# jazlab/moog.github.io

Measured on AMD Instinct MI355X. Metric: env steps/sec (whole node), 4096 envs x 32 sprites, 64x64 obs, higher is better.
Workload: dtype f64; 1 GPU; colliding_predators_32: 4096 envs/GPU x 32 sprites, K=10 substeps, 64x64 raster, random joystick actions, auto-reset on; phase=step + frames, envs_per_gpu=4096, total_envs=4096, sprites=32, parallelism=env-sharded x1, no collective, launch=step launch, then raster launch, on one stream, sub_batches=1, hw_queues=4, episodes=staggered (step_count offsets + 201 burn-in steps before the warm-up)

## Files before the change

### __graft_entry__.py

```python
import glob
import os
import time
import subprocess
import sys

REPO = os.path.dirname(os.path.abspath(__file__))
PKG = os.path.join(REPO, 'moog.github.io_amd')
CSRC = os.path.join(PKG, 'csrc')
LIB = os.path.join(PKG, 'lib', 'libmoog_hip.so')
HIPCC = os.environ.get('HIPCC', '/opt/rocm/bin/hipcc')
sys.path.insert(0, PKG)
from moog import _digest
HIP_FLAGS = _digest.HIP_FLAGS
_STEP_DEPS = ['moog_device.h', 'moog_kernels.h', 'moog_draw_record.h']
_RASTER_DEPS = ['moog_device.h', 'moog_raster.h', 'moog_raster_kernel.h', 'moog_raster_mask.h', 'moog_raster_mask_core.h', 'moog_draw_record.h']
UNITS = [('moog_engine.o', 'moog_engine.hip', [], _STEP_DEPS + _RASTER_DEPS),
         ('moog_raster.o', 'moog_raster.hip', [], _RASTER_DEPS),
         ('moog_reset_r0.o', 'moog_reset.hip', ['-DMOOG_RESET_FULL=0'], _STEP_DEPS),
         ('moog_reset_r1.o', 'moog_reset.hip', ['-DMOOG_RESET_FULL=1'], _STEP_DEPS)] + [
    ('moog_step_%s.o' % tag, 'moog_step_inst.hip',
     ['-DMOOG_STEP_DYN=%d' % dyn, '-DMOOG_STEP_WPS=%d' % wps, '-DMOOG_STEP_TAG=%s' % tag], _STEP_DEPS)
    for tag, dyn, wps in (('f3', 0, 3), ('f4', 0, 4), ('t3', 1, 3), ('t4', 1, 4), ('m3', 2, 3), ('m4', 2, 4))] + [
    ('moog_step_%sr.o' % tag, 'moog_step_inst.hip',
     ['-DMOOG_STEP_DYN=%d' % dyn, '-DMOOG_STEP_WPS=%d' % wps, '-DMOOG_STEP_TAG=%sr' % tag, '-DMOOG_STEP_REPEAT=1'], _STEP_DEPS)
    for tag, dyn, wps in (('f3', 0, 3), ('f4', 0, 4), ('t3', 1, 3), ('t4', 1, 4), ('m3', 2, 3), ('m4', 2, 4))]


SPEC_WORKLOADS = ['colliding_predators_32', 'falling_balls_64', 'functional_maze@128', 'chase_avoid_torus']


def _paths():
    for p in (PKG, os.path.join(REPO, 'tests')):
        if p not in sys.path:
            sys.path.insert(0, p)


def _stale(target, sources):
    if not os.path.exists(target):
        return True
    t = os.path.getmtime(target)
    return any(os.path.getmtime(s) > t for s in sources)


def build():
    hdr = os.path.join(REPO, 'include', 'moog_engine.h')
    os.makedirs(os.path.join(PKG, 'lib'), exist_ok=True)
    digest = _digest.source_digest()
    digest_file = os.path.join(PKG, 'lib', 'src_digest.txt')
    if not os.path.exists(digest_file) or open(digest_file).read().strip() != digest:
        with open(digest_file, 'w') as f:
            f.write(digest + '\n')
    flags_file = os.path.join(PKG, 'lib', 'hip_flags.txt')
    if not os.path.exists(flags_file) or open(flags_file).read().strip() != ' '.join(HIP_FLAGS):
        with open(flags_file, 'w') as f:
            f.write(' '.join(HIP_FLAGS) + '\n')
    for obj in glob.glob(os.path.join(PKG, 'lib', 'moog_*.o')):
        if os.path.basename(obj) not in [u[0] for u in UNITS]:
            os.remove(obj)
    objs, procs = [], []
    started = time.time()
    for obj_name, unit, extra, deps in UNITS:
        obj = os.path.join(PKG, 'lib', obj_name)
        objs.append(obj)
        own = [digest_file] if unit == 'moog_engine.hip' else []
        if unit == 'moog_engine.hip':
            extra = extra + [_digest.define_flag(digest)]
        if _stale(obj, [os.path.join(CSRC, unit), hdr, flags_file] + own + [os.path.join(CSRC, d) for d in sorted(set(deps))]):
            procs.append((obj, subprocess.Popen(
                [HIPCC] + HIP_FLAGS + extra + ['-c', os.path.join(CSRC, unit), '-o', obj])))
    for obj, p in procs:
        if p.wait() != 0:
            for _, q in procs:
                if q.poll() is None:
                    q.terminate()
            raise RuntimeError('hipcc failed: %s' % obj)
        os.utime(obj, (started, started))
    if _stale(LIB, objs):
        subprocess.check_call([HIPCC, '--offload-arch=gfx950', '-shared', '-fPIC'] + objs + ['-o', LIB])
    osrc = [os.path.join(REPO, 'oracle', 'moog_oracle.c'), hdr]
    if _stale(os.path.join(REPO, 'oracle', 'libmoog_oracle.so'), osrc):
        subprocess.check_call(['make', '-C', os.path.join(REPO, 'oracle'), '-B', 'libmoog_oracle.so'])
    _paths()
    import moog
    from moog import _engine
    _engine.load_library()
    from moog import _spec
    assert '%016x' % _engine.load_library().moog_source_digest() == digest, 'libmoog_hip.so does not carry the digest of its sources'
    _spec.main(SPEC_WORKLOADS)
    gone = _spec.remove_stale()
    if gone:
        print('removed %d specialised step kernels of another build: %s' % (len(gone), ' '.join(gone)))


def smoke():
    build()
    _paths()
    import numpy as np
    import torch
    import helpers
    from moog import environment
    from moog_demos import example_configs

    n = 16
    env = environment.BatchedEnvironment(num_envs=n, seed=3, **example_configs.load('colliding_predators'))
    o = helpers.OracleEnv(env.compiled, n_envs=n, seed=3)
    env.reset()
    o.reset()
    rs = np.random.RandomState(0)
    for _ in range(8):
        a = rs.uniform(-1, 1, size=(n, 2))
        ts = env.step(a)
        o.step(a)
    torch.cuda.synchronize()
    f, q = env.state_f64.cpu().numpy(), env.state_i32.cpu().numpy()
    assert np.array_equal(q, o.i32), 'integer state differs from the oracle'
    err = float(np.nanmax(np.abs(f - o.f64)))
    assert err <= 1e-9, 'float state differs from the oracle by %g' % err
    assert np.array_equal(ts.step_type.cpu().numpy(), o.step_type)
    o.f64[:], o.i32[:] = f, q
    assert np.array_equal(ts.observation['image'].cpu().numpy(), o.render()), 'frame mismatch'
    print('smoke ok: %d envs, max |state - oracle| = %.3g' % (n, err))


if __name__ == '__main__':
    build()
    print('build ok:', LIB)
```

### include/moog_engine.h

```cpp
#ifndef MOOG_ENGINE_H_
#define MOOG_ENGINE_H_

#include <stdint.h>

#ifdef __cplusplus
extern "C" {
#endif

#define MOOG_ABI_VERSION 31
#define MOOG_PROGRAM_VERSION 30
#define MOOG_MAX_ACTION_REPEAT 64

#define MOOG_MAX_LAYERS 16
#define MOOG_MAX_FORCES 16
#define MOOG_MAX_CORRECTIVE 4
#define MOOG_MAX_RULES 16
#define MOOG_MAX_TASKS 8
#define MOOG_MAX_OPS 256
#define MOOG_MAX_SHAPES 256
#define MOOG_MAX_SHAPE_VERTS 2048
#define MOOG_MAX_CAND 256
#define MOOG_MAX_DCODE 2048
#define MOOG_X_STACK 16
#define MOOG_MAX_SLOTS 256
// ... 307 lines not shown
  int32_t n_hdraws;
  int32_t rule_state2;
  double timeout_steps;

  moog_force_t forces[MOOG_MAX_FORCES];
  moog_corrective_t corrective[MOOG_MAX_CORRECTIVE];
  moog_rule_t rules[MOOG_MAX_RULES];
  moog_task_t tasks[MOOG_MAX_TASKS];
  moog_action_t action;
  int32_t n_actions;
  int32_t pad_actions_;
  moog_action_t more_actions[MOOG_MAX_MORE_ACTIONS];
  moog_render_t render;
  moog_maze_t maze;
  moog_genop_t ops[MOOG_MAX_OPS];
  moog_shape_t shapes[MOOG_MAX_SHAPES];
  double shape_verts[MOOG_MAX_SHAPE_VERTS][2];
  double cand[MOOG_MAX_CAND];
  int32_t n_dcode;
  int32_t xstack_depth;
  int32_t pad_x_;
  int32_t pad_y_;
  int32_t born_rule;
  moog_dinstr_t dcode[MOOG_MAX_DCODE];
  uint8_t slot_persist[MOOG_MAX_SLOTS];
} moog_program_t;

typedef struct {
  int32_t S, TOTV, T, R;
  int32_t f64_per_env, i32_per_env;
  int32_t o_pos;
  int32_t o_vel;
  int32_t o_angle;
  int32_t o_angvel;
  int32_t o_mass;
  int32_t o_color;
  int32_t o_inertia;
  int32_t o_maxr;
  int32_t o_action;
  int32_t o_task;
  int32_t o_rule;
  int32_t o_hdraw;
  int32_t o_rule2;
  int32_t o_scale;
  int32_t o_aspect;
  int32_t o_verts;
  int32_t o_flags;
  int32_t o_nverts;
  int32_t o_opacity;
  int32_t o_shape;
  int32_t o_tele;
  int32_t o_fmask;
  int32_t o_valias;
  int32_t o_step_count;
  int32_t o_reset_next;
  int32_t o_fault;
  int32_t o_rng;
  int32_t o_maze;
} moog_layout_t;

#if defined(__HIPCC__)
#define MOOG_HD __host__ __device__
#else
#define MOOG_HD
#endif
MOOG_HD static inline int32_t moog_align_(int32_t x, int32_t a) { return (x + a - 1) / a * a; }

MOOG_HD static inline void moog_layout(const moog_program_t* p, moog_layout_t* L) {
  int32_t S = p->n_slots, o = 0;
  L->S = S; L->TOTV = p->n_total_verts; L->T = p->n_tasks; L->R = p->n_rules;
  L->o_pos = o; o += 2 * S;
  L->o_vel = o; o += 2 * S;
  L->o_angle = o; o += S;
  L->o_angvel = o; o += S;
  L->o_mass = o; o += S;
  L->o_color = o; o += 3 * S;
  L->o_inertia = o; o += 2 * S;
  L->o_maxr = o; o += S;
  L->o_action = o; o += 2 * (p->n_actions > 1 ? p->n_actions : 1);
  L->o_task = o; o += p->n_tasks;
  L->o_rule = o; o += p->n_rules;
  if (p->n_hdraws > 0) { L->o_hdraw = o; o += p->n_hdraws; } else L->o_hdraw = -1;
  if (p->rule_state2) { L->o_rule2 = o; o += p->n_rules; } else L->o_rule2 = -1;
  if (p->sprite_factors) { L->o_scale = o; o += S; L->o_aspect = o; o += S; }
  else { L->o_scale = -1; L->o_aspect = -1; }
  o = moog_align_(o, 2);
  L->o_verts = o; o += 2 * p->n_total_verts;
  L->f64_per_env = moog_align_(o, 2);
  o = 0;
  L->o_flags = o; o += S;
  L->o_nverts = o; o += S;
  L->o_opacity = o; o += S;
  L->o_shape = o; o += S;
  L->o_tele = o; o += S;
  if (p->vel_alias) { L->o_valias = o; o += S; } else L->o_valias = -1;
  if (p->sprite_factors) { L->o_fmask = o; o += S; } else L->o_fmask = -1;
  L->o_step_count = o; o += 1;
  L->o_reset_next = o; o += 1;
  L->o_fault = o; o += 1;
  L->o_rng = o; o += 4;
  if (p->maze.random) { L->o_maze = o; o += MOOG_MAX_MAZE + MOOG_MAX_MAZE_POINTS; } else L->o_maze = -1;
  L->i32_per_env = moog_align_(o, 4);
}

typedef struct {
  double* f64;
  int32_t* i32;
} moog_state_view_t;

typedef struct {
  double* reward;
  double* discount;
  int32_t* step_type;
  uint8_t* image;
} moog_step_out_t;

typedef struct {
  const double* uniforms;
  int32_t per_env;
} moog_inject_t;

typedef struct moog_engine moog_engine_t;

enum { MOOG_K_STEP = 0, MOOG_K_RASTER = 1, MOOG_K_RESET = 2, MOOG_K_VIEWS = 3, MOOG_K_COUNT = 4 };

int moog_abi_version(void);
unsigned long long moog_source_digest(void);
const char* moog_last_error(void);
int64_t moog_program_sizeof(void);

int moog_engine_create(const moog_program_t* prog, int32_t n_envs, int32_t device_id,
                       uint64_t seed, int64_t env_index0, moog_engine_t** out);
int moog_engine_destroy(moog_engine_t* e);
int moog_engine_layout(const moog_engine_t* e, moog_layout_t* out);
int moog_engine_load_state(moog_engine_t* e, const moog_state_view_t* view);

int moog_engine_reset(moog_engine_t* e, const uint8_t* env_mask_dev,
                      const moog_inject_t* inject, const moog_step_out_t* out,
                      void* hip_stream);
int moog_engine_step(moog_engine_t* e, const void* actions_dev,
                     const moog_inject_t* inject, const moog_step_out_t* out,
                     void* hip_stream);
int moog_engine_set_action_dtype(moog_engine_t* e, int32_t float32);
int moog_engine_set_action_repeat(moog_engine_t* e, int32_t k, int32_t* count_dev);
int moog_engine_physics_only(moog_engine_t* e, const moog_inject_t* inject,
                             void* hip_stream);
int moog_engine_render(moog_engine_t* e, uint8_t* image_dev, void* hip_stream);

int moog_engine_add_view(moog_engine_t* e, const moog_render_t* render, int32_t* view);
int moog_engine_set_view_image(moog_engine_t* e, int32_t view, uint8_t* image_dev);
int moog_engine_view_raster_path(moog_engine_t* e, int32_t view, int32_t* path);

int moog_engine_set_schedule(moog_engine_t* e, int32_t* perm_dev, float* cost_dev);


int moog_engine_set_reset_pool(moog_engine_t* e, int32_t enabled);
int moog_engine_get_reset_pool(moog_engine_t* e, int32_t* enabled, int64_t* stats);

int moog_engine_layer_usage(moog_engine_t* e, int32_t* high_water, int32_t* dropped);

int moog_engine_set_timing(moog_engine_t* e, int32_t enabled);
int moog_engine_kernel_time(moog_engine_t* e, int32_t kernel_id, double* total_ms,
                            int64_t* launches);

int moog_engine_poll_faults(moog_engine_t* e, int32_t clear, int32_t* bits);

int moog_engine_static_prefix(moog_engine_t* e, int32_t* n_slots, uint8_t* image_dev, void* hip_stream);

int moog_engine_env_prefix(moog_engine_t* e, int32_t* n_slots);

int moog_engine_kernel_variant(moog_engine_t* e, int32_t* variant, int32_t* late_reset);

int moog_program_step_kernel(const moog_program_t* program, int32_t* variant, int32_t* wps, uint64_t* hash);
int moog_engine_step_kernel(moog_engine_t* e, int32_t* specialised);

enum { MOOG_RASTER_SPANS = 0, MOOG_RASTER_MASK = 1, MOOG_RASTER_MASK_COMPACT = 3 };
int moog_engine_raster_path(moog_engine_t* e, int32_t* path);

int moog_engine_read_draw_records(moog_engine_t* e, uint8_t* host_out, int64_t bytes, int64_t* stride, int32_t* in_step);

int moog_engine_set_color_override(moog_engine_t* e, const uint32_t* rgb_dev);

int moog_engine_set_debug(moog_engine_t* e, int32_t step_debug, int32_t raster_stop);

#define MOOG_WATCH_SECTIONS 32
int moog_engine_read_watch(moog_engine_t* e, int32_t* host_out, int32_t clear);

#ifdef __cplusplus
}
#endif
#endif
```

### moog.github.io_amd/csrc/moog_engine.hip

```cpp
#include <hip/hip_runtime.h>

#include <cmath>
#include <cstdio>
#include <cstring>
#include <string>
#include <vector>

#include "moog_kernels.h"

#include "moog_raster.h"
#include <dlfcn.h>
#include <unistd.h>

static thread_local std::string g_err;
static const char* const FRAMELESS_MSG = "this program draws no frames (no PILRenderer observer: render 0 x 0): pass no image";
static int fail(int code, const std::string& msg) { g_err = msg; return code; }
#define HIPCHK(x)                                                                        \
  do {                                                                                   \
    hipError_t err_ = (x);                                                               \
    if (err_ != hipSuccess)                                                              \
      return fail(MOOG_E_HIP, std::string(#x) + ": " + hipGetErrorString(err_));         \
  } while (0)

struct TimedKernel {
  std::vector<std::pair<hipEvent_t, hipEvent_t>> pending;
  double total_ms = 0;
  int64_t launches = 0;
  int64_t seq = 0;
};

struct RView {
  moog_render_t render{};
  const moog_program_t* P = nullptr;
  moog_program_t* d_own = nullptr;
  uint8_t* image = nullptr;
  RPlan raster_plan_{};
  RmSetup mask_setup{};
  uint8_t* draw = nullptr;
  RmDrawLayout draw_lay{};
  int raster_tile_w = 0, raster_band_h = 0, raster_tiles_x = 1, raster_bands = 1;
  int aa = 1, canvas_w = 0, canvas_h = 0, aa_chunk = 0;
  int pad_w = 0;
  uint8_t* pad_img = nullptr;
  int32_t* aa_tables = nullptr;
  RResize aa_resize{};
  int raster_chunk = 0, raster_words = 0, raster_iwords = 0, raster_hwords = 1, raster_xxcap = 4;
  size_t raster_lds = 0;
  int32_t* rows_seen = nullptr;
  int raster_rows_fixed = 0;
  int mask_free_cap = 0;
  int n_static = 0, nsv = 0, kept_n_static = 0;
  uint8_t* s_bg = nullptr;
};

struct moog_engine {
  moog_program_t prog;
  moog_layout_t L;
  moog_program_t* d_prog = nullptr;
  int16_t* d_vslot = nullptr;
  uint32_t* d_vinfo = nullptr;
  int32_t n_envs = 0;
  int device = 0;
  uint64_t seed = 0;
  int64_t env_index0 = 0;
  moog_state_view_t view{nullptr, nullptr};
  size_t step_lds = 0;
  int step_wps = 4;
  void* spec_handle = nullptr;
  void (*spec_launch)(int, size_t, hipStream_t, const KArgs*) = nullptr;
  int32_t xstack_off = 0;
  FOp* d_fops = nullptr;
  int32_t n_fops = 0;
  int32_t* watch = nullptr;
  int32_t watch_off = 0;
  bool dynamic_rules = false;
  bool maze_kernel = false;
  bool late_reset = false;
  uint8_t* late_mask = nullptr;
  RView views[MOOG_MAX_VIEWS];
  int n_views = 1;
  bool frameless = false;
  uint8_t* aa_canvas = nullptr;
  uint8_t* aa_tmp = nullptr;
  size_t aa_canvas_bytes = 0, aa_tmp_bytes = 0;
  int timing = 0;
  int32_t* perm = nullptr;
  hipStream_t sched_stream = nullptr;
  hipEvent_t ev_step_done = nullptr, ev_sched_done = nullptr;
  bool sched_pending = false;
  float* cost = nullptr;
  static constexpr int POOL_STREAMS = 8;
  int pool_streams = 2;
  bool pool_on = false, pool_ready = false;
  static constexpr int pool_depth = 2;
  int32_t* pool_state = nullptr;
  int32_t* pool_tag = nullptr;
  int32_t* pool_lock = nullptr;
  unsigned long long* pool_stats = nullptr;
  double* pool_f64[2] = {nullptr, nullptr};
  int32_t* pool_i32[2] = {nullptr, nullptr};
  hipStream_t pool_stream[POOL_STREAMS] = {};
  hipEvent_t ev_pool = nullptr;
  int64_t pool_fills = 0;
  int act_f32 = 0;
  int action_repeat = 1;
  int32_t* repeat_count = nullptr;
  int32_t* layer_hw = nullptr;
  TimedKernel timed[MOOG_K_COUNT];
  int32_t* fault_flag = nullptr;
  int step_dbg = 0, raster_stop = 0;
  double* s_f64 = nullptr;
  int32_t* s_i32 = nullptr;
  const uint32_t* rgb_override = nullptr;
  int kept_pe_ns = 0, kept_pe_nsv = 0;
  int pe_ns = 0, pe_nsv = 0;
  double* pe_f64 = nullptr;
  int32_t* pe_i32 = nullptr;
  uint8_t* pe_bg = nullptr;
  int32_t* pe_valid = nullptr;
  int32_t* pe_build = nullptr;
  int32_t* pe_min = nullptr;
};

static void free_engine(moog_engine* e) {
  if (e->d_prog) hipFree(e->d_prog);
  if (e->d_vslot) hipFree(e->d_vslot);
  if (e->d_vinfo) hipFree(e->d_vinfo);
  for (RView& v : e->views) {
    if (v.d_own) hipFree(v.d_own);
    if (v.draw) hipFree(v.draw);
    if (v.s_bg) hipFree(v.s_bg);
    if (v.pad_img) hipFree(v.pad_img);
    if (v.aa_tables) hipFree(v.aa_tables);
    if (v.rows_seen) hipHostFree(v.rows_seen);
  }
  if (e->s_f64) hipFree(e->s_f64);
  if (e->s_i32) hipFree(e->s_i32);
  if (e->aa_canvas) hipFree(e->aa_canvas);
  if (e->aa_tmp) hipFree(e->aa_tmp);
  if (e->fault_flag) hipHostFree(e->fault_flag);
  if (e->layer_hw) hipFree(e->layer_hw);
  for (int k = 0; k < moog_engine::POOL_STREAMS; ++k)
    if (e->pool_stream[k]) { hipStreamSynchronize(e->pool_stream[k]); hipStreamDestroy(e->pool_stream[k]); }
  if (e->ev_pool) hipEventDestroy(e->ev_pool);
  if (e->pe_f64) hipFree(e->pe_f64);
  if (e->pe_i32) hipFree(e->pe_i32);
  if (e->pe_bg) hipFree(e->pe_bg);
  if (e->pe_valid) hipFree(e->pe_valid);
  if (e->pe_build) hipFree(e->pe_build);
  if (e->pe_min) hipHostFree(e->pe_min);
  if (e->pool_state) hipFree(e->pool_state);
  if (e->pool_tag) hipFree(e->pool_tag);
  if (e->pool_lock) hipFree(e->pool_lock);
  if (e->late_mask) hipFree(e->late_mask);
  if (e->pool_stats) hipFree(e->pool_stats);
  for (int k = 0; k < 2; ++k) { if (e->pool_f64[k]) hipFree(e->pool_f64[k]); if (e->pool_i32[k]) hipFree(e->pool_i32[k]); }
  if (e->watch) hipFree(e->watch);
  if (e->d_fops) hipFree(e->d_fops);
  delete e;
}

static int static_prefix_slots(const moog_program_t* p, int polymod, int* nsv) {
  *nsv = 0;
  if (polymod != MOOG_POLYMOD_NONE) return 0;
  std::vector<char> ok((size_t)(p->n_slots > 0 ? p->n_slots : 1), 0);
  for (int oi = 0; oi < p->n_ops; ++oi) {
    const moog_genop_t& op = p->ops[oi];
    if (op.runtime || op.n_sampled != 0 || op.code_off >= 0 || op.count_min != op.count_max) continue;
    bool c = true;
    for (int k = 0; k < MOOG_NUM_FACTORS; ++k) c = c && op.factors[k].kind == MOOG_DIST_CONST;
    c = c && op.factors[MOOG_FAC_XVEL].a == 0 && op.factors[MOOG_FAC_YVEL].a == 0 && op.factors[MOOG_FAC_ANGVEL].a == 0;
    if (!c) continue;
    for (int sl = op.slot0; sl < op.slot0 + op.count_max && sl < p->n_slots; ++sl)
      if (sl >= 0 && !p->layer_dynamic[p->slot_layer[sl]]) ok[sl] = 1;
  }
  int ns = 0, nv = 0;
  while (ns < p->n_slots && ns < 32 && ok[ns] && p->slot_voff[ns] == nv) { nv += p->slot_vcap[ns]; ++ns; }
  *nsv = nv;
  return ns;
}

static int env_prefix_slots(const moog_program_t* p, int* nsv) {
  *nsv = 0;
  if (p->render.polymod != MOOG_POLYMOD_NONE) return 0;
  std::vector<char> ok((size_t)(p->n_slots > 0 ? p->n_slots : 1), 0);
  for (int oi = 0; oi < p->n_ops; ++oi) {
    const moog_genop_t& op = p->ops[oi];
    if (op.runtime || op.cell_sel == MOOG_CELL_STORE) continue;
    bool c = true;
    for (int k = MOOG_FAC_XVEL; k <= MOOG_FAC_ANGVEL; ++k)
      if (k == MOOG_FAC_XVEL || k == MOOG_FAC_YVEL || k == MOOG_FAC_ANGVEL) c = c && op.factors[k].kind == MOOG_DIST_CONST && op.factors[k].a == 0;
    if (!c) continue;
    for (int sl = op.slot0; sl < op.slot0 + op.count_max && sl < p->n_slots; ++sl)
      if (sl >= 0 && !p->layer_dynamic[p->slot_layer[sl]]) ok[sl] = 1;
  }
  for (int oi = 0; oi < p->n_ops; ++oi)
    if (p->ops[oi].cell_sel == MOOG_CELL_STORE && p->ops[oi].cell_arg >= 0 && p->ops[oi].cell_arg < p->n_slots) ok[p->ops[oi].cell_arg] = 0;
  int ns = 0, nv = 0;
  while (ns < p->n_slots && ok[ns] && p->slot_voff[ns] == nv) { nv += p->slot_vcap[ns]; ++ns; }
  *nsv = nv;
  return ns;
}

struct StepVariant { bool dynamic_rules = false, maze_kernel = false, late_reset = false; int wps = 4; size_t step_lds = 0; int32_t xstack_off = 0; };

static StepVariant step_variant_of(const moog_program_t* prog) {
  StepVariant v;
  moog_layout_t GL;
  moog_layout(prog, &GL);
  const moog_layout_t HL = hot_layout(GL).L;
  v.step_lds = (size_t)HL.f64_per_env * 8 + (size_t)HL.i32_per_env * 4 + (size_t)GL.S * 4 * 8 +
               (size_t)((GL.S + 3) & ~3) * 4 + CAND_CAP * 2 + 128 + 64 * 8 + 16;
  if (prog->xstack_depth > 0) {
    v.step_lds = (v.step_lds + 15) & ~(size_t)15;
    v.xstack_off = (int32_t)v.step_lds;
    v.step_lds += (size_t)prog->xstack_depth * 64 * 8;
  }
  for (int r = 0; r < prog->n_rules; ++r) {
    int k = prog->rules[r].kind;
    if (k == MOOG_RULE_VANISH_BY_FILTER || k == MOOG_RULE_CHANGE_LAYER || k == MOOG_RULE_CREATE_SPRITES ||
        k == MOOG_RULE_MODIFY_SPRITES || k == MOOG_RULE_MODIFY_ON_CONTACT || k == MOOG_RULE_DRAWS)
      v.dynamic_rules = true;
  }
  for (int t = 0; t < prog->n_tasks; ++t) {
    if (prog->tasks[t].kind == MOOG_TASK_CONTACT_REWARD && (prog->tasks[t].xcond >= 0 || prog->tasks[t].xreward >= 0))
      v.dynamic_rules = true;
    if (prog->tasks[t].kind == MOOG_TASK_RESET && (prog->tasks[t].cond >= MOOG_COND_ALL_EXPR || prog->tasks[t].xreward >= 0))
      v.dynamic_rules = true;
  }
  for (int r = 0; r < prog->n_rules; ++r)
    if ((prog->rules[r].kind == MOOG_RULE_CONDITIONAL || prog->rules[r].kind == MOOG_RULE_PHASE) &&
        prog->rules[r].cond >= MOOG_RCOND_CONTACT_COUNT)
      v.dynamic_rules = true;
  for (int l = 0; l < prog->n_layers; ++l) if (prog->layer_dynamic[l]) v.dynamic_rules = true;
  for (int f = 0; f < prog->n_forces; ++f)
    if (prog->forces[f].kind == MOOG_FORCE_DISTANCE_EXPR) v.dynamic_rules = true;
  for (int r = 0; r < prog->n_rules; ++r)
    if (prog->rules[r].kind == MOOG_RULE_FIXATION || (prog->rules[r].kind == MOOG_RULE_PHASE && prog->rules[r].op == 1))
      v.dynamic_rules = true;
  for (int k = 0; k < prog->n_dcode; ++k) {
    if (prog->dcode[k].op == MOOG_X_STORE && prog->dcode[k].a == MOOG_XA_ANGLE) v.maze_kernel = true;
    const int op = prog->dcode[k].op;
    if (op == MOOG_X_SLOT_ATTR || op == MOOG_X_HDRAW || op == MOOG_X_HDRAW_T || op == MOOG_X_STORE_VERT || op == MOOG_X_FACTOR)
      v.maze_kernel = true;
  }
  for (int o = 0; o < prog->n_ops; ++o) if (prog->ops[o].cell_sel != MOOG_CELL_NONE) v.maze_kernel = true;
  if (prog->n_hdraws > 0) v.maze_kernel = true;
  for (int o = 0; o < prog->n_ops; ++o)
    for (int k = 0; k < MOOG_NUM_FACTORS; ++k)
      if (prog->ops[o].factors[k].kind == MOOG_DIST_EXPR || prog->ops[o].factors[k].kind == MOOG_DIST_EXPR_SHAPE)
        v.maze_kernel = true;
  for (int f = 0; f < prog->n_forces; ++f)
    if (prog->forces[f].kind == MOOG_FORCE_MAZE_WALK || prog->forces[f].kind == MOOG_FORCE_MAZE_WALK_DET) v.maze_kernel = true;
  for (int c = 0; c < prog->n_corrective; ++c) if (prog->corrective[c].kind == MOOG_CORR_MAZE) v.maze_kernel = true;
  if (prog->maze.random) v.maze_kernel = true;
  if (v.maze_kernel) {
    bool stepping = false;
    for (int f = 0; f < prog->n_forces; ++f)
      stepping = stepping || prog->forces[f].kind == MOOG_FORCE_MAZE_WALK || prog->forces[f].kind == MOOG_FORCE_MAZE_WALK_DET;
    for (int c = 0; c < prog->n_corrective; ++c) stepping = stepping || prog->corrective[c].kind == MOOG_CORR_MAZE;
    for (int k = 0; k < prog->n_dcode; ++k) stepping = stepping || (prog->dcode[k].op == MOOG_X_STORE && prog->dcode[k].a == MOOG_XA_ANGLE);
    for (int o = 0; o < prog->n_ops; ++o) {
      const moog_genop_t& op = prog->ops[o];
      if (!op.runtime) continue;
      bool full = op.cell_sel != MOOG_CELL_NONE || op.code_off >= 0;
      for (int k = 0; k < MOOG_NUM_FACTORS; ++k)
        full = full || op.factors[k].kind == MOOG_DIST_EXPR || op.factors[k].kind == MOOG_DIST_EXPR_SHAPE;
      stepping = stepping || full;
    }
    const char* off = getenv("MOOG_NO_LATE_RESET");
    v.late_reset = !stepping && !(off && atoi(off));
    if (v.late_reset) v.dynamic_rules = true;
  }
  v.wps = (160 * 1024 / (v.step_lds ? v.step_lds : 1)) <= 14 ? 3 : 4;
  { const char* w = getenv("MOOG_STEP_WPS"); if (w && (atoi(w) == 3 || atoi(w) == 4)) v.wps = atoi(w); }
  return v;
}

static uint64_t program_hash(const moog_program_t* prog) {
  const unsigned char* b = reinterpret_cast<const unsigned char*>(prog);
  uint64_t h = 1469598103934665603ull;
  for (size_t i = 0; i < sizeof(moog_program_t); ++i) { h ^= b[i]; h *= 1099511628211ull; }
  return h;
}

static void load_spec_kernel(moog_engine* e, const moog_program_t* prog);

#ifndef MOOG_SRC_DIGEST
#define MOOG_SRC_DIGEST 0ull
#endif
#define MOOG_STR2(x) #x
#define MOOG_STR(x) MOOG_STR2(x)
extern "C" const char moog_src_digest_marker[] = "MOOG_SRC_DIGEST=" MOOG_STR(MOOG_SRC_DIGEST);

extern "C" {

int moog_abi_version(void) { return MOOG_ABI_VERSION; }
unsigned long long moog_source_digest(void) { return MOOG_SRC_DIGEST; }
const char* moog_last_error(void) { return g_err.c_str(); }
int64_t moog_program_sizeof(void) { return (int64_t)sizeof(moog_program_t); }

static int validate_render(const moog_program_t* p, const moog_render_t* r) {
  const int aa = r->aa > 1 ? r->aa : 1;
  const long long cw = (long long)aa * r->width, ch = (long long)aa * r->height;
  if (cw < 1 || cw > 8192 || ch < 1 || ch > 8192 || aa > 16)
    return fail(MOOG_E_UNSUPPORTED, "render size unsupported (1 <= anti_aliasing x width, height <= 8192, anti_aliasing <= 16)");
  if (r->cmap != MOOG_CMAP_IDENTITY && r->cmap != MOOG_CMAP_HSV) return fail(MOOG_E_INVALID, "render cmap out of range");
// ... 302 lines not shown
      v.mask_free_cap = (ms.ok && !v.raster_rows_fixed) ? mask_free_rows(e, v) : ms.cap_rows;
      if (ms.ok) {
        v.draw_lay = rm_draw_layout(ms.S, e->L.TOTV * ms.ncopy);
        if (hipMalloc(&v.draw, (size_t)e->n_envs * v.draw_lay.stride) != hipSuccess) {
          return fail(MOOG_E_NOMEM, "out of device memory (draw records)");
        }
      }
    }
  }
  if (hipHostMalloc(reinterpret_cast<void**>(&v.rows_seen), 2 * sizeof(int32_t), hipHostMallocMapped | hipHostMallocCoherent) == hipSuccess) { v.rows_seen[0] = 0; v.rows_seen[1] = 0; }
  else v.rows_seen = nullptr;
  return MOOG_OK;
}

int moog_engine_create(const moog_program_t* prog, int32_t n_envs, int32_t device_id, uint64_t seed,
                       int64_t env_index0, moog_engine_t** out) {
  if (!out) return fail(MOOG_E_INVALID, "null out");
  int rc = validate(prog);
  if (rc) return rc;
  if (n_envs <= 0) return fail(MOOG_E_INVALID, "n_envs <= 0");
  HIPCHK(hipSetDevice(device_id));
  moog_engine* e = new moog_engine();
  e->prog = *prog;
  e->frameless = prog->render.width == 0 && prog->render.height == 0;
  moog_layout(prog, &e->L);
  e->n_envs = n_envs;
  e->device = device_id;
  e->seed = seed;
  e->env_index0 = env_index0;
  hipError_t err = hipMalloc(&e->d_prog, sizeof(moog_program_t));
  if (err != hipSuccess) { free_engine(e); return fail(MOOG_E_NOMEM, "hipMalloc(program) failed"); }
  err = hipMemcpy(e->d_prog, prog, sizeof(moog_program_t), hipMemcpyHostToDevice);
  if (err != hipSuccess) { free_engine(e); return fail(MOOG_E_HIP, "hipMemcpy(program) failed"); }
  {
    std::vector<int16_t> vs((size_t)(prog->n_total_verts > 0 ? prog->n_total_verts : 1), 0);
    for (int sl = 0; sl < prog->n_slots; ++sl)
      for (int k = 0; k < prog->slot_vcap[sl]; ++k) vs[prog->slot_voff[sl] + k] = (int16_t)sl;
    err = hipMalloc(&e->d_vslot, vs.size() * sizeof(int16_t));
    if (err == hipSuccess)
      err = hipMemcpy(e->d_vslot, vs.data(), vs.size() * sizeof(int16_t), hipMemcpyHostToDevice);
    if (err != hipSuccess) { free_engine(e); return fail(MOOG_E_NOMEM, "vertex table"); }
    std::vector<uint32_t> vi(vs.size(), 0u);
    for (int sl = 0; sl < prog->n_slots; ++sl)
      for (int k = 0; k < prog->slot_vcap[sl]; ++k) vi[prog->slot_voff[sl] + k] = (uint32_t)sl | ((uint32_t)k << 8);
    err = hipMalloc(&e->d_vinfo, vi.size() * sizeof(uint32_t));
    if (err == hipSuccess)
      err = hipMemcpy(e->d_vinfo, vi.data(), vi.size() * sizeof(uint32_t), hipMemcpyHostToDevice);
    if (err != hipSuccess) { free_engine(e); return fail(MOOG_E_NOMEM, "vertex table"); }
  }
  {
    const std::vector<FOp> fops = moog_flatten_forces(prog);
    e->n_fops = (int32_t)fops.size();
    err = hipMalloc(&e->d_fops, (fops.size() + 1) * sizeof(FOp));
    if (err == hipSuccess && !fops.empty()) err = hipMemcpy(e->d_fops, fops.data(), fops.size() * sizeof(FOp), hipMemcpyHostToDevice);
    if (err != hipSuccess) { free_engine(e); return fail(MOOG_E_NOMEM, "force list"); }
  }
  {
    const StepVariant sv = step_variant_of(prog);
    e->step_lds = sv.step_lds; e->xstack_off = sv.xstack_off;
  }
  { const char* w = getenv("MOOG_WATCH");
    if (w && atoi(w) == 1) {
      e->step_lds = (e->step_lds + 15) & ~(size_t)15;
      e->watch_off = (int32_t)e->step_lds;
      e->step_lds += 16;
      if (hipMalloc(&e->watch, (size_t)n_envs * MOOG_WATCH_SECTIONS * sizeof(int32_t)) != hipSuccess ||
          hipMemset(e->watch, 0, (size_t)n_envs * MOOG_WATCH_SECTIONS * sizeof(int32_t)) != hipSuccess) {
        free_engine(e);
        return fail(MOOG_E_NOMEM, "hipMalloc(watch) failed");
      }
    } }
  if (e->step_lds > 160 * 1024) {
    free_engine(e);
    return fail(MOOG_E_UNSUPPORTED, "state record does not fit in 160 KB of LDS");
  }
  if (!e->frameless) {
    e->views[0].render = prog->render;
    e->views[0].P = e->d_prog;
    const int rc = setup_view(e, e->views[0], true);
    if (rc) { free_engine(e); return rc; }
  }
  {
    int (*const configure[12])(size_t) = {moog_configure_step_f3, moog_configure_step_f4, moog_configure_step_t3,
                                          moog_configure_step_t4, moog_configure_step_m3, moog_configure_step_m4,
                                          moog_configure_step_f3r, moog_configure_step_f4r, moog_configure_step_t3r,
                                          moog_configure_step_t4r, moog_configure_step_m3r, moog_configure_step_m4r};
    for (int v = 0; v < 12 && err == hipSuccess; ++v) err = (hipError_t)configure[v](e->step_lds);
  }
  {
    const StepVariant sv = step_variant_of(prog);
    e->dynamic_rules = sv.dynamic_rules; e->maze_kernel = sv.maze_kernel; e->late_reset = sv.late_reset; e->step_wps = sv.wps;
  }
  if (!e->watch) load_spec_kernel(e, prog);
  if (e->late_reset) {
    if (hipMalloc(&e->late_mask, (size_t)n_envs) != hipSuccess || hipMemset(e->late_mask, 0, (size_t)n_envs) != hipSuccess) {
      free_engine(e);
      return fail(MOOG_E_NOMEM, "hipMalloc(late reset mask) failed");
    }
  }
  if (err == hipSuccess)
    err = (hipError_t)moog_configure_reset_plain(e->step_lds);
    if (err == hipSuccess) err = (hipError_t)moog_configure_reset_full(e->step_lds);
  if (err == hipSuccess && !e->frameless)
    err = (hipError_t)moog_raster_configure(e->views[0].raster_lds);
  if (err == hipSuccess && e->views[0].mask_setup.ok) err = (hipError_t)moog_raster_configure_mask(64 * 1024);
  if (err != hipSuccess) {
    free_engine(e);
    return fail(MOOG_E_HIP, std::string("hipFuncSetAttribute: ") + hipGetErrorString(err));
  }
  { const char* ds = getenv("MOOG_STEP_DEBUG"); e->step_dbg = ds ? atoi(ds) : 0; }
  { const char* ds = getenv("MOOG_RASTER_STOP"); e->raster_stop = ds ? atoi(ds) : 0; }
  if (hipHostMalloc(reinterpret_cast<void**>(&e->fault_flag), sizeof(int32_t), hipHostMallocMapped | hipHostMallocCoherent) != hipSuccess) {
    free_engine(e);
    return fail(MOOG_E_NOMEM, "hipHostMalloc(fault flag) failed");
  }
  *e->fault_flag = 0;
  for (int l = 0; l < prog->n_layers; ++l)
    if (prog->layer_dynamic[l] && !e->layer_hw) {
      if (hipMalloc(&e->layer_hw, 2 * MOOG_MAX_LAYERS * sizeof(int32_t)) != hipSuccess ||
          hipMemset(e->layer_hw, 0, 2 * MOOG_MAX_LAYERS * sizeof(int32_t)) != hipSuccess) {
        free_engine(e);
        return fail(MOOG_E_NOMEM, "hipMalloc(layer usage) failed");
      }
    }
  int rc2 = MOOG_OK;
  if (!e->frameless) {
    RView& v = e->views[0];
    rc2 = build_static_prefix(e, v);
    if (rc2 == MOOG_OK) rc2 = setup_anti_aliasing(e, v);
    if (rc2 == MOOG_OK) rc2 = setup_env_prefix(e);
    if (rc2 == MOOG_OK && v.aa <= 1 && v.pad_w != v.canvas_w &&
        hipMalloc(&v.pad_img, (size_t)n_envs * v.canvas_h * v.pad_w * 3) != hipSuccess)
      rc2 = fail(MOOG_E_NOMEM, "hipMalloc(16-aligned frames) failed");
  }
  if (rc2) { free_engine(e); return rc2; }
  *out = e;
  return MOOG_OK;
}

static void drain(TimedKernel& t) {
  for (auto& pr : t.pending) {
    hipEventSynchronize(pr.second);
    float ms = 0;
    if (hipEventElapsedTime(&ms, pr.first, pr.second) == hipSuccess) { t.total_ms += ms; t.launches++; }
    hipEventDestroy(pr.first);
    hipEventDestroy(pr.second);
  }
  t.pending.clear();
}

int moog_engine_destroy(moog_engine_t* e) {
  if (!e) return MOOG_OK;
  for (int k = 0; k < MOOG_K_COUNT; ++k) drain(e->timed[k]);
  if (e->sched_stream) {
    hipStreamSynchronize(e->sched_stream);
    hipEventDestroy(e->ev_step_done); hipEventDestroy(e->ev_sched_done);
    hipStreamDestroy(e->sched_stream);
  }
  void* spec = e->spec_handle;
  free_engine(e);
  (void)spec;
  return MOOG_OK;
}

int moog_engine_layout(const moog_engine_t* e, moog_layout_t* out) {
  if (!e || !out) return fail(MOOG_E_INVALID, "null argument");
  *out = e->L;
  return MOOG_OK;
}

static int pool_drop(moog_engine* e, hipStream_t s);

int moog_engine_load_state(moog_engine_t* e, const moog_state_view_t* view) {
  if (!e || !view || !view->f64 || !view->i32) return fail(MOOG_E_INVALID, "null state view");
  if (((uintptr_t)view->f64 & 15) || ((uintptr_t)view->i32 & 15))
    return fail(MOOG_E_INVALID, "state buffers must be 16-byte aligned");
  e->view = *view;
  if (e->pool_on) {
    HIPCHK(hipSetDevice(e->device));
    const int rc = pool_drop(e, 0);
    if (rc) return rc;
    HIPCHK(hipStreamSynchronize(0));
  }
  return MOOG_OK;
}

static bool sampled(moog_engine* e, int id) {
  const int period = ((e->timing >> 8) & 255) + 1;
  return ((e->timing >> id) & 1) && (e->timed[id].seq++ % period) == 0;
}

struct Bracket {
  moog_engine* e; int id; hipStream_t s; hipEvent_t a = nullptr, b = nullptr;
  Bracket(moog_engine* e_, int id_, hipStream_t s_, int on = -1) : e(e_), id(id_), s(s_) {
    if (on < 0 ? sampled(e, id) : on != 0) { hipEventCreate(&a); hipEventCreate(&b); hipEventRecord(a, s); }
  }
  ~Bracket() {
    if (a) { hipEventRecord(b, s); e->timed[id].pending.emplace_back(a, b); }
  }
};

static KArgs make_args(moog_engine* e, const void* actions, const moog_inject_t* inj,
                       const moog_step_out_t* out, int mode, const uint8_t* mask) {
  KArgs a;
  a.P = e->d_prog; a.L = e->L; a.H = hot_layout(e->L); a.f64 = e->view.f64; a.i32 = e->view.i32;
  a.actions = actions;
  a.inj = (inj && inj->uniforms) ? inj->uniforms : nullptr;
  a.inj_n = (inj && inj->uniforms) ? inj->per_env : 0;
  a.n_envs = e->n_envs; a.seed = e->seed; a.env_index0 = e->env_index0;
  a.mask = mask;
  a.reward = out ? out->reward : nullptr;
  a.discount = out ? out->discount : nullptr;
  a.step_type = out ? out->step_type : nullptr;
  a.mode = mode;
  a.vslot = e->d_vslot;
  a.perm = (mode == MODE_STEP && e->perm) ? e->perm : nullptr;
  a.cost = (mode == MODE_STEP) ? e->cost : nullptr;
  a.dbg = e->step_dbg;
  a.fault_flag = e->fault_flag;
  a.layer_hw = e->layer_hw;
  a.act_f32 = e->act_f32;
  a.repeat = mode == MODE_STEP ? e->action_repeat : 1;
  a.repeat_count = mode == MODE_STEP ? e->repeat_count : nullptr;
  a.xstack_off = e->xstack_off;
  a.watch = (mode == MODE_STEP) ? e->watch : nullptr; a.watch_off = e->watch_off;
  a.fops = e->d_fops; a.n_fops = e->n_fops;
  const bool pool = e->pool_on && mode == MODE_STEP && !(inj && inj->uniforms);
  a.pool_state = pool ? e->pool_state : nullptr; a.pool_tag = e->pool_tag; a.pool_stats = e->pool_stats;
  a.pool_lock = e->pool_lock; a.pool_depth = e->pool_depth;
  for (int k = 0; k < 2; ++k) { a.pool_f64[k] = e->pool_f64[k]; a.pool_i32[k] = e->pool_i32[k]; }
  a.live_f64 = nullptr; a.live_i32 = nullptr;
  a.late_mask = (mode == MODE_STEP && e->late_reset) ? e->late_mask : nullptr;
  a.rank0 = 0;
  memset(&a.draw, 0, sizeof a.draw);
  a.draw_vinfo = e->d_vinfo;
  return a;
}

static void launch_step(moog_engine* e, hipStream_t s, const KArgs& a) {
  static const moog_step_launch_fn launch[12] = {moog_launch_step_f3, moog_launch_step_f4, moog_launch_step_t3,
                                                 moog_launch_step_t4, moog_launch_step_m3, moog_launch_step_m4,
                                                 moog_launch_step_f3r, moog_launch_step_f4r, moog_launch_step_t3r,
                                                 moog_launch_step_t4r, moog_launch_step_m3r, moog_launch_step_m4r};
  if (e->spec_launch) {
    e->spec_launch(e->n_envs, e->step_lds, s, &a);
    return;
  }
  const bool full = e->maze_kernel && !e->late_reset;
  launch[(a.repeat > 1 ? 6 : 0) + (full ? 4 : (e->dynamic_rules ? 2 : 0)) + (e->step_wps == 4 ? 1 : 0)](e->n_envs, e->step_lds, s, a);
}

static RmEmit emit_args(moog_engine* e, const RView& v) {
  RmEmit m;
  memset(&m, 0, sizeof m);
  const RmSetup& ms = v.mask_setup;
  if (!ms.ok || !v.draw) return m;
  m.out = v.draw; m.lay = v.draw_lay;
  m.S = ms.S; m.slots = ms.slots; m.ncopy = ms.ncopy; m.W = v.pad_w; m.H = v.canvas_h; m.scale_w = v.canvas_w;
  m.cmap = ms.cmap; m.first_person = ms.first_person; m.fp_slot0 = ms.fp_slot0; m.fp_nslots = ms.fp_nslots;
  m.n_static = (e->s_f64 && ms.ncopy == 1) ? v.n_static : 0;
  m.sref_v = e->s_f64 ? e->s_f64 + e->L.o_verts : nullptr;
  m.sref_col = e->s_f64 ? e->s_f64 + e->L.o_color : nullptr;
  m.sref_flags = e->s_i32 ? e->s_i32 + e->L.o_flags : nullptr;
  m.sref_nv = e->s_i32 ? e->s_i32 + e->L.o_nverts : nullptr;
  m.sref_opa = e->s_i32 ? e->s_i32 + e->L.o_opacity : nullptr;
  m.rgb_override = e->rgb_override;
  return m;
}
static bool step_emits_draw(moog_engine* e) {
  const RView& v = e->views[0];
  const bool scratch_fits = v.mask_setup.ncopy == 1 ||
      4u * (size_t)RM_EMIT_SCRATCH_WORDS(v.mask_setup.slots, v.mask_setup.S, v.mask_setup.ncopy) <= (size_t)CAND_CAP * 2 + 128 + 64 * 8;
  return v.mask_setup.ok && v.draw && e->pe_ns <= 0 && v.aa <= 1 && scratch_fits;
}

static RArgs raster_args(moog_engine* e, RView& v, uint8_t* image) {
  RArgs r;
  if (v.mask_setup.ok) mask_rows_grow(e, v);
  r.ms = v.mask_setup;
  r.rows_seen = (v.raster_rows_fixed || v.mask_setup.cap_rows >= v.mask_free_cap) ? nullptr : v.rows_seen;
  r.P = v.P; r.L = e->L; r.f64 = e->view.f64; r.i32 = e->view.i32; r.image = image;
  r.vinfo = e->d_vinfo; r.plan = v.raster_plan_;
  r.n_envs = e->n_envs; r.chunk = v.raster_chunk; r.words = v.raster_words;
  r.tile_w = v.raster_tile_w; r.band_h = v.raster_band_h; r.tiles_x = v.raster_tiles_x; r.bands = v.raster_bands;
  r.canvas_w = v.pad_w; r.scale_w = v.canvas_w; r.canvas_h = v.canvas_h; r.flip = v.aa > 1 ? 0 : 1;
  r.iwords = v.raster_iwords; r.hwords = v.raster_hwords; r.xxcap = v.raster_xxcap;
  r.debug_stop = e->raster_stop;
  r.n_static = v.n_static; r.nsv = v.nsv; r.build = 0;
  r.sref_v = e->s_f64 ? e->s_f64 + e->L.o_verts : nullptr;
  r.sref_col = e->s_f64 ? e->s_f64 + e->L.o_color : nullptr;
  r.sref_flags = e->s_i32 ? e->s_i32 + e->L.o_flags : nullptr;
  r.sref_nv = e->s_i32 ? e->s_i32 + e->L.o_nverts : nullptr;
  r.sref_opa = e->s_i32 ? e->s_i32 + e->L.o_opacity : nullptr;
  r.sbg = v.s_bg;
  r.sbg_env_stride = 0; r.env_build = nullptr; r.rgb_override = e->rgb_override;
  r.em = emit_args(e, v); r.draw_ready = 0; r.env0 = 0;
  return r;
}

static int use_env_prefix(moog_engine* e, RArgs& r, hipStream_t s) {
  if (e->pe_ns <= 0) return MOOG_OK;
  const int seen = __atomic_load_n(e->pe_min, __ATOMIC_RELAXED);
  if (seen < e->pe_ns) {
    e->pe_ns = seen < 8 ? 0 : seen;
    e->pe_nsv = e->pe_ns > 0 ? e->prog.slot_voff[e->pe_ns] : 0;
    __atomic_store_n(e->pe_min, INT32_MAX, __ATOMIC_RELAXED);
    if (e->pe_ns <= 0) return MOOG_OK;
    HIPCHK(hipMemsetAsync(e->pe_valid, 0, sizeof(int32_t) * (size_t)e->n_envs, s));
  }
  PCArgs c;
  c.P = e->d_prog; c.L = e->L; c.f64 = e->view.f64; c.i32 = e->view.i32; c.s_f64 = e->pe_f64; c.s_i32 = e->pe_i32;
  c.valid = e->pe_valid; c.build = e->pe_build; c.min_changed = e->pe_min; c.n_envs = e->n_envs; c.n_static = e->pe_ns;
  moog_prefix_check_launch(c, s);
  RArgs b = r;
  b.image = e->pe_bg; b.n_static = e->pe_ns; b.nsv = e->pe_nsv; b.build = 1; b.env_build = e->pe_build; b.debug_stop = 0;
  b.sbg = nullptr; b.sbg_env_stride = 0;
  moog_raster_launch(b, e->views[0].raster_lds, s);
  r.n_static = e->pe_ns; r.nsv = e->pe_nsv; r.sbg = e->pe_bg;
  r.sbg_env_stride = (size_t)e->views[0].canvas_h * e->views[0].pad_w * 3;
  return MOOG_OK;
}

static int launch_raster(moog_engine* e, RView& v, uint8_t* image, hipStream_t s, bool draw_ready = false) {
  RArgs r = raster_args(e, v, image);
  r.draw_ready = draw_ready ? 1 : 0;
  if (v.aa <= 1 && &v == &e->views[0]) { const int rc = use_env_prefix(e, r, s); if (rc) return rc; }
  if (v.aa <= 1 && v.pad_w != v.canvas_w) {
    r.image = v.pad_img;
    moog_raster_launch(r, v.raster_lds, s);
    moog_crop_launch(v.pad_img, image, (size_t)e->n_envs * v.canvas_h, v.pad_w * 3, v.canvas_w * 3, s);
  } else if (v.aa <= 1) {
    moog_raster_launch(r, v.raster_lds, s);
  } else {
    const size_t frame = (size_t)v.render.width * v.render.height * 3;
    for (int e0 = 0; e0 < e->n_envs; e0 += v.aa_chunk) {
      const int n = e->n_envs - e0 < v.aa_chunk ? e->n_envs - e0 : v.aa_chunk;
      RArgs c = r;
      c.f64 = r.f64 + (size_t)e0 * e->L.f64_per_env;
      c.i32 = r.i32 + (size_t)e0 * e->L.i32_per_env;
      c.image = e->aa_canvas;
      c.n_envs = n;
      c.env0 = e0; c.draw_ready = (e0 == 0 && n == e->n_envs) ? r.draw_ready : 0;
      moog_raster_launch(c, v.raster_lds, s);
      moog_resize_launch(v.aa_resize, e->aa_canvas, e->aa_tmp, image + (size_t)e0 * frame, n, s);
    }
  }
  HIPCHK(hipGetLastError());
  return MOOG_OK;
}

static bool derives_ahead(moog_engine* e, const RView& v) {
  if (!v.mask_setup.ok || !v.draw) return false;
  if (&v == &e->views[0] && e->pe_ns > 0) return false;
  return v.aa <= 1 || v.aa_chunk >= e->n_envs;
}

static int launch_frames(moog_engine* e, uint8_t* image, hipStream_t s, bool draw_ready = false, int timed = -1) {
  RView* extra[MOOG_MAX_VIEWS];
  int n_extra = 0;
  for (int k = 1; k < e->n_views; ++k) if (e->views[k].image) extra[n_extra++] = &e->views[k];
  if (n_extra == 0) {
    Bracket br(e, MOOG_K_RASTER, s, timed);
    return launch_raster(e, e->views[0], image, s, draw_ready);
  }
  RView& p = e->views[0];
  const bool join = !draw_ready && derives_ahead(e, p);
  {
    Bracket br(e, MOOG_K_VIEWS, s);
    RmEmit em[MOOG_MAX_VIEWS];
    bool ahead[MOOG_MAX_VIEWS] = {};
    int n_em = 0;
    if (join) em[n_em++] = emit_args(e, p);
    for (int k = 0; k < n_extra; ++k)
      if (derives_ahead(e, *extra[k])) { ahead[k] = true; em[n_em++] = emit_args(e, *extra[k]); }
    if (n_em > 0) moog_derive_launch(em, n_em, raster_args(e, p, image), s);
    for (int k = 0; k < n_extra; ++k) {
      const int rc = launch_raster(e, *extra[k], extra[k]->image, s, ahead[k]);
      if (rc) return rc;
    }
  }
  Bracket br(e, MOOG_K_RASTER, s, timed);
  return launch_raster(e, p, image, s, draw_ready || join);
}

static int pool_kick(moog_engine* e, hipStream_t s) {
  hipStream_t ps = e->pool_stream[e->pool_fills % e->pool_streams];
  HIPCHK(hipEventRecord(e->ev_pool, s));
  HIPCHK(hipStreamWaitEvent(ps, e->ev_pool, 0));
  KArgs a = make_args(e, nullptr, nullptr, nullptr, MODE_FILL, nullptr);
  a.live_f64 = e->view.f64; a.live_i32 = e->view.i32;
  a.f64 = e->pool_f64[1]; a.i32 = e->pool_i32[1];
  a.pool_state = e->pool_state;
  a.fault_flag = nullptr;
  a.dbg = 0;
  moog_launch_reset_full(e->n_envs * e->pool_depth, e->step_lds, ps, a);
  HIPCHK(hipGetLastError());
  ++e->pool_fills;
  return MOOG_OK;
}

static int late_reset_launch(moog_engine* e, const moog_inject_t* inject, const moog_step_out_t* out, hipStream_t s, const RmEmit* draw) {
  KArgs b = make_args(e, nullptr, inject, out, MODE_RESET_MASK, nullptr);
  if (draw) b.draw = *draw;
  b.late_mask = e->late_mask;
  b.pool_state = (e->pool_on && !(inject && inject->uniforms)) ? e->pool_state : nullptr;
  moog_launch_reset_full(e->n_envs, e->step_lds, s, b);
  HIPCHK(hipGetLastError());
  return MOOG_OK;
}

static int pool_drop(moog_engine* e, hipStream_t s) {
  for (int k = 0; k < e->pool_streams; ++k) HIPCHK(hipStreamSynchronize(e->pool_stream[k]));
  HIPCHK(hipMemsetAsync(e->pool_state, 0, sizeof(int32_t) * (size_t)e->n_envs * e->pool_depth, s));
  HIPCHK(hipMemsetAsync(e->pool_lock, 0, sizeof(int32_t) * (size_t)e->n_envs, s));
  return MOOG_OK;
}

static int ready(moog_engine* e) {
  if (!e) return fail(MOOG_E_INVALID, "null engine");
  if (!e->view.f64) return fail(MOOG_E_INVALID, "moog_engine_load_state has not been called");
  HIPCHK(hipSetDevice(e->device));
  return MOOG_OK;
}

int moog_engine_reset(moog_engine_t* e, const uint8_t* env_mask_dev, const moog_inject_t* inject,
                      const moog_step_out_t* out, void* hip_stream) {
  int rc = ready(e);
  if (rc) return rc;
  if (out && out->image && e->frameless) return fail(MOOG_E_INVALID, FRAMELESS_MSG);
  hipStream_t s = (hipStream_t)hip_stream;
  KArgs a = make_args(e, nullptr, inject, out, MODE_RESET_MASK, env_mask_dev);
  if (e->pool_on && (rc = pool_drop(e, s)) != MOOG_OK) return rc;
  {
    Bracket br(e, MOOG_K_RESET, s);
    (e->maze_kernel ? moog_launch_reset_full : moog_launch_reset_plain)(e->n_envs, e->step_lds, s, a);
  }
  HIPCHK(hipGetLastError());
  if (e->pool_on && !(inject && inject->uniforms) && (rc = pool_kick(e, s)) != MOOG_OK) return rc;
  if (out && out->image) return launch_frames(e, out->image, s);
  return MOOG_OK;
}

int moog_engine_step(moog_engine_t* e, const void* actions_dev, const moog_inject_t* inject,
                     const moog_step_out_t* out, void* hip_stream) {
  int rc = ready(e);
  if (rc) return rc;
  if (!actions_dev) return fail(MOOG_E_INVALID, "null actions");
  if (out && out->image && e->frameless) return fail(MOOG_E_INVALID, FRAMELESS_MSG);
  if (e->action_repeat > 1 && inject && inject->uniforms)
    return fail(MOOG_E_UNSUPPORTED, "injected uniforms are one call's stream: they cannot feed the several env-steps of an action repeat (moog_engine_set_action_repeat(e, 1, ...) first)");
  hipStream_t s = (hipStream_t)hip_stream;
  KArgs a = make_args(e, actions_dev, inject, out, MODE_STEP, nullptr);
  const bool emit = out && out->image && step_emits_draw(e);
  if (emit) a.draw = emit_args(e, e->views[0]);
  if (e->sched_pending) {
    HIPCHK(hipStreamWaitEvent(s, e->ev_sched_done, 0));
    e->sched_pending = false;
  }
  {
    Bracket br(e, MOOG_K_STEP, s);
    launch_step(e, s, a);
    if (e->late_reset && (rc = late_reset_launch(e, inject, out, s, emit ? &a.draw : nullptr)) != MOOG_OK) return rc;
  }
  HIPCHK(hipGetLastError());
  if (a.pool_state && (rc = pool_kick(e, s)) != MOOG_OK) return rc;
  if (e->perm && e->cost) {
    HIPCHK(hipEventRecord(e->ev_step_done, s));
    HIPCHK(hipStreamWaitEvent(e->sched_stream, e->ev_step_done, 0));
    moog_launch_sched(e->sched_stream, e->cost, e->perm, e->n_envs,
                      e->view.i32 + e->L.o_reset_next, e->L.i32_per_env);
    HIPCHK(hipEventRecord(e->ev_sched_done, e->sched_stream));
    e->sched_pending = true;
  }
  if (out && out->image) return launch_frames(e, out->image, s, emit);
  return MOOG_OK;
}

int moog_engine_physics_only(moog_engine_t* e, const moog_inject_t* inject, void* hip_stream) {
  int rc = ready(e);
  if (rc) return rc;
  hipStream_t s = (hipStream_t)hip_stream;
  KArgs a = make_args(e, nullptr, inject, nullptr, MODE_PHYSICS, nullptr);
  {
    Bracket br(e, MOOG_K_STEP, s);
    launch_step(e, s, a);
  }
  HIPCHK(hipGetLastError());
  return MOOG_OK;
}

int moog_engine_render(moog_engine_t* e, uint8_t* image_dev, void* hip_stream) {
  int rc = ready(e);
  if (rc) return rc;
  if (!image_dev) return fail(MOOG_E_INVALID, "null image");
  if (e->frameless) return fail(MOOG_E_INVALID, FRAMELESS_MSG);
  return launch_frames(e, image_dev, (hipStream_t)hip_stream);
}

int moog_engine_set_schedule(moog_engine_t* e, int32_t* perm_dev, float* cost_dev) {
  if (!e) return fail(MOOG_E_INVALID, "null engine");
  if (e->sched_pending) { hipEventSynchronize(e->ev_sched_done); e->sched_pending = false; }
  e->perm = perm_dev;
  e->cost = cost_dev;
  if (perm_dev && cost_dev) {
    HIPCHK(hipSetDevice(e->device));
    HIPCHK(hipMemset(cost_dev, 0, (size_t)e->n_envs * sizeof(float)));
  }
  if (perm_dev && cost_dev && !e->sched_stream) {
    HIPCHK(hipSetDevice(e->device));
    HIPCHK(hipStreamCreateWithFlags(&e->sched_stream, hipStreamNonBlocking));
    HIPCHK(hipEventCreateWithFlags(&e->ev_step_done, hipEventDisableTiming));
    HIPCHK(hipEventCreateWithFlags(&e->ev_sched_done, hipEventDisableTiming));
  }
  return MOOG_OK;
}

int moog_engine_set_reset_pool(moog_engine_t* e, int32_t enabled) {
  if (!e) return fail(MOOG_E_INVALID, "null engine");
  HIPCHK(hipSetDevice(e->device));
  if (!enabled) {
    if (e->pool_on) { const int rc = pool_drop(e, 0); if (rc) return rc; HIPCHK(hipStreamSynchronize(0)); }
    e->pool_on = false;
    return MOOG_OK;
  }
  if (!e->maze_kernel)
    return fail(MOOG_E_UNSUPPORTED, "the reset pool lives in the kernels that carry every component; this program runs the plain ones (its resets are cheap)");
  for (int o = 0; o < e->prog.n_ops; ++o)
    if (e->prog.ops[o].cell_sel == MOOG_CELL_PSTATE)
      return fail(MOOG_E_UNSUPPORTED, "the reset pool cannot serve a program whose initializer keeps a number across episodes (MOOG_CELL_PSTATE): its resets depend on how the previous episode went");
  {
    const char* ser = getenv("AMD_SERIALIZE_KERNEL");
    const char* blk = getenv("HIP_LAUNCH_BLOCKING");
    const char* hwq = getenv("GPU_MAX_HW_QUEUES");
    const char* cc = getenv("ROCPROF_COUNTER_COLLECTION");
    if ((ser && atoi(ser)) || (blk && atoi(blk)) || (hwq && atoi(hwq) == 1) || (cc && atoi(cc)))
      return fail(MOOG_E_UNSUPPORTED, "the reset pool needs kernels to run beside each other (AMD_SERIALIZE_KERNEL / HIP_LAUNCH_BLOCKING / GPU_MAX_HW_QUEUES=1 / counter collection serialise them)");
  }
  if (!e->pool_ready) {
    const size_t n = (size_t)e->n_envs * e->pool_depth;
    if (!e->pool_state) HIPCHK(hipMalloc(&e->pool_state, sizeof(int32_t) * n));
    if (!e->pool_tag) HIPCHK(hipMalloc(&e->pool_tag, sizeof(int32_t) * n));
    if (!e->pool_lock) HIPCHK(hipMalloc(&e->pool_lock, sizeof(int32_t) * (size_t)e->n_envs));
    if (!e->pool_stats) { HIPCHK(hipMalloc(&e->pool_stats, 4 * sizeof(unsigned long long))); HIPCHK(hipMemset(e->pool_stats, 0, 4 * sizeof(unsigned long long))); }
    for (int k = 0; k < 2; ++k) {
      if (!e->pool_f64[k]) HIPCHK(hipMalloc(&e->pool_f64[k], sizeof(double) * n * (size_t)e->L.f64_per_env));
      if (!e->pool_i32[k]) HIPCHK(hipMalloc(&e->pool_i32[k], sizeof(int32_t) * n * (size_t)e->L.i32_per_env));
    }
    {
      const char* hwq = getenv("GPU_MAX_HW_QUEUES");
      const int queues = (hwq && atoi(hwq) > 0) ? atoi(hwq) : 4;
      e->pool_streams = queues - 2 < 1 ? 1 : (queues - 2 > moog_engine::POOL_STREAMS ? moog_engine::POOL_STREAMS : queues - 2);
    }
    for (int k = 0; k < e->pool_streams; ++k)
      if (!e->pool_stream[k]) HIPCHK(hipStreamCreateWithFlags(&e->pool_stream[k], hipStreamNonBlocking));
    if (!e->ev_pool) HIPCHK(hipEventCreateWithFlags(&e->ev_pool, hipEventDisableTiming));
    e->pool_ready = true;
  }
  HIPCHK(hipMemset(e->pool_state, 0, sizeof(int32_t) * (size_t)e->n_envs * e->pool_depth));
  HIPCHK(hipMemset(e->pool_tag, 0, sizeof(int32_t) * (size_t)e->n_envs * e->pool_depth));
  HIPCHK(hipMemset(e->pool_lock, 0, sizeof(int32_t) * (size_t)e->n_envs));
  e->pool_on = true;
  return MOOG_OK;
}

int moog_engine_get_reset_pool(moog_engine_t* e, int32_t* enabled, int64_t* stats) {
  if (!e) return fail(MOOG_E_INVALID, "null engine");
  if (enabled) *enabled = e->pool_on ? 1 : 0;
  if (stats) {
    stats[0] = e->pool_fills;
    for (int k = 1; k < 5; ++k) stats[k] = 0;
    if (e->pool_stats) {
      unsigned long long h[4];
      HIPCHK(hipSetDevice(e->device));
      HIPCHK(hipDeviceSynchronize());
      HIPCHK(hipMemcpy(h, e->pool_stats, sizeof(h), hipMemcpyDeviceToHost));
      for (int k = 0; k < 4; ++k) stats[1 + k] = (int64_t)h[k];
    }
  }
  return MOOG_OK;
}

int moog_engine_set_action_dtype(moog_engine_t* e, int32_t float32) {
  if (!e) return fail(MOOG_E_INVALID, "null engine");
  e->act_f32 = float32 ? 1 : 0;
  return MOOG_OK;
}

int moog_engine_set_action_repeat(moog_engine_t* e, int32_t k, int32_t* count_dev) {
  if (!e) return fail(MOOG_E_INVALID, "null engine");
  if (k < 1 || k > MOOG_MAX_ACTION_REPEAT) return fail(MOOG_E_INVALID, "action repeat out of range (1 .. MOOG_MAX_ACTION_REPEAT)");
  e->action_repeat = k;
  e->repeat_count = count_dev;
  return MOOG_OK;
}

int moog_engine_layer_usage(moog_engine_t* e, int32_t* high_water, int32_t* dropped) {
  if (!e || !high_water || !dropped) return fail(MOOG_E_INVALID, "null argument");
  int32_t host[2 * MOOG_MAX_LAYERS] = {0};
  if (e->layer_hw) {
    HIPCHK(hipSetDevice(e->device));
    HIPCHK(hipMemcpy(host, e->layer_hw, sizeof(host), hipMemcpyDeviceToHost));
  }
  for (int l = 0; l < MOOG_MAX_LAYERS; ++l) { high_water[l] = host[l]; dropped[l] = host[MOOG_MAX_LAYERS + l]; }
  return MOOG_OK;
}

int moog_program_step_kernel(const moog_program_t* prog, int32_t* variant, int32_t* wps, uint64_t* hash) {
  if (!prog) return fail(MOOG_E_INVALID, "null program");
  const StepVariant v = step_variant_of(prog);
  if (variant) *variant = (v.maze_kernel && !v.late_reset) ? 2 : (v.dynamic_rules ? 1 : 0);
  if (wps) *wps = v.wps;
  if (hash) *hash = program_hash(prog);
  return MOOG_OK;
}

int moog_engine_step_kernel(moog_engine_t* e, int32_t* specialised) {
  if (!e || !specialised) return fail(MOOG_E_INVALID, "null argument");
  *specialised = e->spec_launch ? 1 : 0;
  return MOOG_OK;
}

int moog_engine_read_draw_records(moog_engine_t* e, uint8_t* host_out, int64_t bytes, int64_t* stride, int32_t* in_step) {
  if (!e) return fail(MOOG_E_INVALID, "null engine");
  const RView& v = e->views[0];
  if (!v.mask_setup.ok || !v.draw) return fail(MOOG_E_UNSUPPORTED, "this program's frames are not the mask rasteriser's: no draw records");
  if (stride) *stride = (int64_t)v.draw_lay.stride;
  if (in_step) *in_step = step_emits_draw(e) ? 1 : 0;
  if (!host_out) return MOOG_OK;
  const int64_t need = (int64_t)e->n_envs * (int64_t)v.draw_lay.stride;
  if (bytes < need) return fail(MOOG_E_INVALID, "host buffer too small for the draw records");
  HIPCHK(hipSetDevice(e->device));
  HIPCHK(hipDeviceSynchronize());
  HIPCHK(hipMemcpy(host_out, v.draw, (size_t)need, hipMemcpyDeviceToHost));
  return MOOG_OK;
}

int moog_engine_raster_path(moog_engine_t* e, int32_t* path) { return moog_engine_view_raster_path(e, 0, path); }

int moog_engine_view_raster_path(moog_engine_t* e, int32_t view, int32_t* path) {
  if (!e || !path) return fail(MOOG_E_INVALID, "null argument");
  if (e->frameless) return fail(MOOG_E_INVALID, FRAMELESS_MSG);
  if (view < 0 || view >= e->n_views) return fail(MOOG_E_INVALID, "no such view");
  const RmSetup& ms = e->views[view].mask_setup;
  const bool prefix = view == 0 && e->pe_ns > 0;
  *path = (ms.ok && !prefix) ? (ms.compact ? MOOG_RASTER_MASK_COMPACT : MOOG_RASTER_MASK) : MOOG_RASTER_SPANS;
  return MOOG_OK;
}

int moog_engine_add_view(moog_engine_t* e, const moog_render_t* render, int32_t* view) {
  if (!e || !render || !view) return fail(MOOG_E_INVALID, "null argument");
  if (e->frameless) return fail(MOOG_E_INVALID, "this program draws no frames (render 0 x 0): it takes no extra views");
  if (e->n_views >= MOOG_MAX_VIEWS) return fail(MOOG_E_UNSUPPORTED, "at most MOOG_MAX_VIEWS views per engine");
  int rc = validate_render(&e->prog, render);
  if (rc) return rc;
  HIPCHK(hipSetDevice(e->device));
  RView& v = e->views[e->n_views];
  v = RView();
  v.render = *render;
  moog_program_t* host = new moog_program_t(e->prog);
  host->render = *render;
  hipError_t err = hipMalloc(&v.d_own, sizeof(moog_program_t));
  if (err == hipSuccess) err = hipMemcpy(v.d_own, host, sizeof(moog_program_t), hipMemcpyHostToDevice);
  delete host;
  v.P = v.d_own;
  if (err == hipSuccess) rc = setup_view(e, v, false);
  else rc = fail(MOOG_E_NOMEM, "hipMalloc(view program) failed");
// ... 171 lines not shown
```

### moog.github.io_amd/csrc/moog_kernels.h

```cpp
#pragma once
#include "moog_device.h"
#include "moog_draw_record.h"

static __device__ __forceinline__ float moog_cost_ema(float now, float before) {
  return (before >= 0.f && before < 3.0e38f) ? 0.4f * before + 0.6f * now : now;
}

struct HotLayout {
  moog_layout_t L;
  int32_t f_cut0, f_cut1;
  int32_t i_cut0, i_cut1;
};

__host__ __device__ inline HotLayout hot_layout(const moog_layout_t& G) {
  HotLayout h;
  h.L = G;
  const int S = G.S;
  const bool f_ok = (G.o_color % 2 == 0) && ((3 * S) % 2 == 0);
  h.f_cut0 = G.o_color;
  h.f_cut1 = f_ok ? G.o_color + 3 * S : G.o_color;
  const int fc = h.f_cut1 - h.f_cut0;
  h.L.o_inertia -= fc; h.L.o_maxr -= fc; h.L.o_action -= fc; h.L.o_task -= fc; h.L.o_rule -= fc;
  if (G.o_hdraw >= 0) h.L.o_hdraw -= fc;
  if (G.o_rule2 >= 0) h.L.o_rule2 -= fc;
  if (G.o_scale >= 0) { h.L.o_scale -= fc; h.L.o_aspect -= fc; }
  h.L.o_verts -= fc; h.L.f64_per_env -= fc;
  const bool i_ok = (G.o_opacity % 4 == 0) && ((3 * S) % 4 == 0) && (G.o_shape == G.o_opacity + S) &&
                    (G.o_tele == G.o_shape + S);
  h.i_cut0 = G.o_opacity;
  h.i_cut1 = i_ok ? G.o_opacity + 3 * S : G.o_opacity;
  const int ic = h.i_cut1 - h.i_cut0;
  if (G.o_valias >= 0) h.L.o_valias -= ic;
  if (G.o_fmask >= 0) h.L.o_fmask -= ic;
  h.L.o_step_count -= ic; h.L.o_reset_next -= ic; h.L.o_fault -= ic; h.L.o_rng -= ic;
  if (G.o_maze >= 0) h.L.o_maze -= ic;
  h.L.i32_per_env -= ic;
  return h;
}

#ifdef MOOG_SPEC_PROGRAM_INC
__device__ __forceinline__ moog_layout_t moog_spec_hot_layout_fn() {
  moog_layout_t L;
  moog_layout(&MOOG_SPEC_PROGRAM, &L);
  return hot_layout(L).L;
}
#endif

__device__ inline void load_record(const Env& e, const HotLayout& h, const moog_layout_t& G,
                                   const double* gf, const int32_t* gq) {
  const double2* src = reinterpret_cast<const double2*>(gf);
  double2* dst = reinterpret_cast<double2*>(EF(e));
  const int fa = h.f_cut0 / 2, fb = h.f_cut1 / 2;
  for (int i = e.lane; i < G.f64_per_env / 2; i += 64) {
    if (i < fa) dst[i] = src[i];
    else if (i >= fb) dst[i - (fb - fa)] = src[i];
  }
  const int4* srci = reinterpret_cast<const int4*>(gq);
  int4* dsti = reinterpret_cast<int4*>(EQ(e));
  const int ia = h.i_cut0 / 4, ib = h.i_cut1 / 4;
  for (int i = e.lane; i < G.i32_per_env / 4; i += 64) {
    if (i < ia) dsti[i] = srci[i];
    else if (i >= ib) dsti[i - (ib - ia)] = srci[i];
  }
  for (int i = e.lane; i < EL(e).S; i += 64) EVOFF(e)[i] = EP(e)->slot_voff[i];
  wsync();
}

__device__ inline void store_record(const Env& e, const HotLayout& h, const moog_layout_t& G,
                                    double* gf, int32_t* gq, int32_t* fault_flag = nullptr) {
  wsync();
  if (fault_flag && e.lane == 0) {
    const int32_t fw = EQ(e)[EL(e).o_fault];
    if (fw) __hip_atomic_fetch_or(fault_flag, fw, __ATOMIC_RELAXED, __HIP_MEMORY_SCOPE_SYSTEM);
  }
  double2* dst = reinterpret_cast<double2*>(gf);
  const double2* src = reinterpret_cast<const double2*>(EF(e));
  const int fa = h.f_cut0 / 2, fb = h.f_cut1 / 2;
  int4* dsti = reinterpret_cast<int4*>(gq);
  const int4* srci = reinterpret_cast<const int4*>(EQ(e));
  const int ia = h.i_cut0 / 4, ib = h.i_cut1 / 4;
  for (int i = e.lane; i < G.f64_per_env / 2; i += 64) {
    if (i < fa) dst[i] = src[i];
    else if (i >= fb) dst[i] = src[i - (fb - fa)];
  }
  for (int i = e.lane; i < G.i32_per_env / 4; i += 64) {
    if (i < ia) dsti[i] = srci[i];
    else if (i >= ib) dsti[i] = srci[i - (ib - ia)];
  }
}

#include <vector>
inline std::vector<FOp> moog_flatten_forces(const moog_program_t* p) {
  std::vector<FOp> out;
  for (int fi = 0; fi < p->n_forces; ++fi) {
    const moog_force_t& F = p->forces[fi];
    for (int a = 0; a < F.n_a; ++a) {
      FOp op = {};
      op.fi = fi; op.kind = F.kind; op.symmetric = F.symmetric; op.i0 = F.i0; op.i1 = F.i1; op.p0 = F.p0; op.p1 = F.p1;
      op.a0 = p->layer_slot0[F.layers_a[a]]; op.a1 = op.a0 + p->layer_nslots[F.layers_a[a]];
      op.n_b = F.n_b;
      if (F.n_b == 0) { out.push_back(op); continue; }
      for (int b = 0; b < F.n_b; ++b) {
        op.b0 = p->layer_slot0[F.layers_b[b]]; op.b1 = op.b0 + p->layer_nslots[F.layers_b[b]];
        out.push_back(op);
      }
    }
  }
  return out;
}

struct KArgs {
  const moog_program_t* P;
  moog_layout_t L;
  HotLayout H;
  double* f64;
  int32_t* i32;
  const void* actions;
  const double* inj;
  int32_t inj_n;
  int32_t n_envs;
  uint64_t seed;
  int64_t env_index0;
  const uint8_t* mask;
  double* reward;
  double* discount;
  int32_t* step_type;
  int32_t mode;
  const int16_t* vslot;
  int32_t dbg;
  const int32_t* perm;
  float* cost;
  int32_t* fault_flag;
  int32_t* layer_hw;
  int32_t act_f32;
  int32_t xstack_off;
  const FOp* fops;
  int32_t n_fops;
  int32_t* watch;
  int32_t watch_off;
  int32_t* pool_state;
  int32_t* pool_tag;
  int32_t* pool_lock;
  int32_t pool_depth;
  double* pool_f64[2];
  int32_t* pool_i32[2];
  uint8_t* late_mask;
  unsigned long long* pool_stats;
  const double* live_f64;
  const int32_t* live_i32;
  int32_t rank0;
  const uint32_t* draw_vinfo;
  RmEmit draw;
  int32_t repeat;
  int32_t* repeat_count;
};

enum { MODE_STEP = 0, MODE_PHYSICS = 1, MODE_RESET_MASK = 2, MODE_FILL = 3 };

extern __shared__ __attribute__((aligned(16))) unsigned char moog_lds[];

__device__ inline void bind_env(Env& e, const KArgs& a, int env, unsigned char* lds = moog_lds, int lane = (int)threadIdx.x) {
  e.P = as_const_prog(a.P);
  e.fops = (PFOp)(unsigned long long)a.fops;
  e.n_fops = a.n_fops;
  e.L = a.H.L;
  const moog_layout_t& H = a.H.L;
  e.f = reinterpret_cast<double*>(lds);
  e.q = reinterpret_cast<int32_t*>(lds + (size_t)H.f64_per_env * 8);
  e.bb = reinterpret_cast<float*>(lds + (size_t)H.f64_per_env * 8 + (size_t)H.i32_per_env * 4);
  e.voff = reinterpret_cast<int32_t*>((e).bb + 8 * H.S);
  e.cand = reinterpret_cast<uint16_t*>((e).voff + ((H.S + 3) & ~3));
  e.lst = reinterpret_cast<uint8_t*>((e).cand + CAND_CAP);
  e.rowm = reinterpret_cast<unsigned long long*>((e).lst + 128);
  e.xstack = a.xstack_off > 0 ? reinterpret_cast<double*>(lds + a.xstack_off) : nullptr;
#ifdef MOOG_WATCH
  e.secw = a.watch ? reinterpret_cast<int32_t*>(__builtin_assume_aligned(lds + a.watch_off, 16)) : nullptr;
#endif
  if (a.H.f_cut1 > a.H.f_cut0) e.gcol = a.f64 + (size_t)env * a.L.f64_per_env + a.L.o_color;
  else e.gcol = EF(e) + H.o_color;
  if (a.H.i_cut1 > a.H.i_cut0) {
    e.gopa = a.i32 + (size_t)env * a.L.i32_per_env + a.L.o_opacity;
    e.gshape = a.i32 + (size_t)env * a.L.i32_per_env + a.L.o_shape;
    e.gtele = a.i32 + (size_t)env * a.L.i32_per_env + a.L.o_tele;
  } else {
    e.gopa = EQ(e) + H.o_opacity;
    e.gshape = EQ(e) + H.o_shape;
    e.gtele = EQ(e) + H.o_tele;
  }
  e.vslot = a.vslot;
  e.dbg = a.dbg;
  e.n_path = 0; e.n_resp = 0; e.n_disj = 0;
  e.layer_hw = a.layer_hw;
  e.cell_tab_n = 0; e.cell_nw = 0;
#ifdef MOOG_PROFILE
  for (int k = 0; k < 16; ++k) e.prof[k] = 0;
#endif
  e.inj = a.inj ? a.inj + (size_t)env * a.inj_n : nullptr;
  e.inj_n = a.inj_n;
  e.seed = a.seed;
  e.env_index = a.env_index0 + env;
  e.lane = lane;
}

struct RmSrcEnv {
  static constexpr bool kGlobalRecord = false;
  const Env* e; const uint32_t* vi;
  __device__ __forceinline__ int flags(int s) const { return EQ(*e)[EL(*e).o_flags + s]; }
  __device__ __forceinline__ int nv(int s) const { return EQ(*e)[EL(*e).o_nverts + s]; }
  __device__ __forceinline__ int opa(int s) const { return static_cast<const int32_t*>(e->gopa)[s]; }
  __device__ __forceinline__ int voff(int s) const { return EVOFF(*e)[s]; }
  __device__ __forceinline__ int vcap(int s) const { return EP(*e)->slot_vcap[s]; }
  __device__ __forceinline__ double col(int s, int c) const { return static_cast<const double*>(e->gcol)[3 * s + c]; }
  __device__ __forceinline__ uint32_t vinfo(int idx) const { return vi[idx]; }
  __device__ __forceinline__ const double* vbase() const { return &EF(*e)[EL(*e).o_verts]; }
  __device__ __forceinline__ const double* pos(int s) const { return &EF(*e)[EL(*e).o_pos + 2 * s]; }
};
__device__ __forceinline__ void emit_draw_record(const Env& e, const KArgs& a, int env) {
  if (!a.draw.out) return;
  const long long t_emit = (a.dbg & 256) ? clock64() : 0;
  wsync();
  RmSrcEnv src;
  src.e = &e; src.vi = a.draw_vinfo;
  RmEmitScratch sc;
  rm_emit_scratch(a.draw.ncopy > 1 ? reinterpret_cast<int32_t*>(ECAND(e)) : reinterpret_cast<int32_t*>(EBB(e)), a.draw.slots, a.draw.ncopy, &sc);
  long long clk[5];
  rm_emit(a.draw, src, env, e.lane, sc, EL(e).TOTV, (a.dbg & 256) ? clk : nullptr);
  if ((a.dbg & 256) && e.lane == 0 && a.step_type) {
    a.step_type[env] = (int32_t)(clock64() - t_emit);
    if (a.discount) a.discount[env] = (double)(clk[1] - clk[0]) + 65536.0 * (double)(clk[2] - clk[1]);
    if (a.reward) a.reward[env] = (double)(clk[3] - clk[2]) + 65536.0 * (double)(clk[4] - clk[3]);
  }
}

#if MOOG_WITH_MAZE
#define MOOG_WITH_POOL 1
#elif defined(MOOG_STEP_DYN)
#define MOOG_WITH_POOL (MOOG_STEP_DYN >= 1)
#else
#define MOOG_WITH_POOL 0
#endif
#if MOOG_WITH_POOL
__device__ inline bool pool_inputs_equal(const Env& e, const moog_layout_t& G, const double* af, const int32_t* aq,
                                         const double* bf, const int32_t* bq) {
  PProg P = EP(e);
  bool same = true;
  const bool born = P->born_rule > 0;
  if (born) {
    same = __double_as_longlong(af[G.o_rule + P->born_rule - 1]) == __double_as_longlong(bf[G.o_rule + P->born_rule - 1]);
    for (int s = e.lane; s < G.S; s += 64) {
      if (!P->slot_persist[s]) continue;
      #define PEQ_F(o, k) (__double_as_longlong(af[(o) + (k)]) == __double_as_longlong(bf[(o) + (k)]))
      #define PEQ_I(o) (aq[(o) + s] == bq[(o) + s])
      bool q = PEQ_F(G.o_pos, 2 * s) && PEQ_F(G.o_pos, 2 * s + 1) && PEQ_F(G.o_vel, 2 * s) && PEQ_F(G.o_vel, 2 * s + 1) &&
               PEQ_F(G.o_angle, s) && PEQ_F(G.o_angvel, s) && PEQ_F(G.o_mass, s) && PEQ_F(G.o_color, 3 * s) &&
               PEQ_F(G.o_color, 3 * s + 1) && PEQ_F(G.o_color, 3 * s + 2) && PEQ_F(G.o_inertia, 2 * s) &&
               PEQ_F(G.o_inertia, 2 * s + 1) && PEQ_F(G.o_maxr, s);
      if (G.o_scale >= 0) q = q && PEQ_F(G.o_scale, s) && PEQ_F(G.o_aspect, s);
      q = q && PEQ_I(G.o_flags) && PEQ_I(G.o_nverts) && PEQ_I(G.o_opacity) && PEQ_I(G.o_shape);
      if (G.o_valias >= 0) q = q && PEQ_I(G.o_valias);
      if (G.o_fmask >= 0) q = q && PEQ_I(G.o_fmask);
      int nv = aq[G.o_nverts + s];
      if (nv > P->slot_vcap[s]) nv = P->slot_vcap[s];
      const int v0 = G.o_verts + 2 * P->slot_voff[s];
      for (int k = 0; k < 2 * nv; ++k) q = q && PEQ_F(v0, k);
      #undef PEQ_F
      #undef PEQ_I
      same = same && q;
    }
  }
  return __all(same);
}

__device__ inline void pool_copy_record(const moog_layout_t& G, int lane, const double* sf, const int32_t* sq, double* df, int32_t* dq) {
  const double2* a = reinterpret_cast<const double2*>(sf);
  double2* b = reinterpret_cast<double2*>(df);
  for (int i = lane; i < G.f64_per_env / 2; i += 64) b[i] = a[i];
  const int4* c = reinterpret_cast<const int4*>(sq);
  int4* d = reinterpret_cast<int4*>(dq);
  for (int i = lane; i < G.i32_per_env / 4; i += 64) d[i] = c[i];
}

__device__ inline bool pool_adopt(Env& e, const KArgs& a, int env, double* gf, int32_t* gq, int* held) {
  *held = 0;
  if (!a.pool_state || e.inj) return false;
// ... 33 lines not shown
    return false;
  }
  __builtin_amdgcn_fence(__ATOMIC_ACQUIRE, "agent");
  const size_t rec = (size_t)pick * a.n_envs + env;
  const double* pre_f = a.pool_f64[0] + rec * a.L.f64_per_env; const int32_t* pre_q = a.pool_i32[0] + rec * a.L.i32_per_env;
  const double* post_f = a.pool_f64[1] + rec * a.L.f64_per_env; const int32_t* post_q = a.pool_i32[1] + rec * a.L.i32_per_env;
  const bool ok = pool_inputs_equal(e, a.L, pre_f, pre_q, gf, gq);
  wsync();
  if (!ok) {
    if (e.lane == 0) {
      __hip_atomic_store(&a.pool_state[rec], 0, __ATOMIC_RELAXED, __HIP_MEMORY_SCOPE_AGENT);
      atomicAdd(&a.pool_stats[1], 1ull); atomicAdd(&a.pool_stats[2], 1ull);
    }
    return false;
  }
  const int32_t fault = EQ(e)[EL(e).o_fault];
  const int r = e.lane < a.L.R ? e.lane : 0;
  const double keep = EF(e)[EL(e).o_rule + r];
  const double keep2 = EL(e).o_rule2 >= 0 ? EF(e)[EL(e).o_rule2 + r] : 0.0;
  wsync();
  load_record(e, a.H, a.L, post_f, post_q);
  if (a.H.f_cut1 > a.H.f_cut0)
    for (int i = a.H.f_cut0 + e.lane; i < a.H.f_cut1; i += 64) gf[i] = post_f[i];
  if (a.H.i_cut1 > a.H.i_cut0)
    for (int i = a.H.i_cut0 + e.lane; i < a.H.i_cut1; i += 64) gq[i] = post_q[i];
  if (e.lane < a.L.R && EP(e)->rules[e.lane].kind == MOOG_RULE_STATE_SLOT) {
    EF(e)[EL(e).o_rule + e.lane] = keep;
    if (EL(e).o_rule2 >= 0) EF(e)[EL(e).o_rule2 + e.lane] = keep2;
  }
  wave_global_fence();
  wsync();
  if (e.lane == 0) {
    EQ(e)[EL(e).o_fault] |= fault;
    __hip_atomic_store(&a.pool_state[rec], 0, __ATOMIC_RELAXED, __HIP_MEMORY_SCOPE_AGENT);
    atomicAdd(&a.pool_stats[0], 1ull);
    if (waited) atomicAdd(&a.pool_stats[3], 1ull);
  }
  wsync();
  return true;
}

__device__ inline void pool_release(const KArgs& a, int env, int lane) {
  __builtin_amdgcn_fence(__ATOMIC_RELEASE, "agent");
  if (lane == 0) __hip_atomic_store(&a.pool_lock[env], 0, __ATOMIC_RELAXED, __HIP_MEMORY_SCOPE_AGENT);
}
#else
__device__ __forceinline__ bool pool_adopt(Env&, const KArgs&, int, double*, int32_t*, int* held) { *held = 0; return false; }
__device__ __forceinline__ void pool_release(const KArgs&, int, int) {}
#endif

#ifdef MOOG_DEFINE_RESET_KERNELS
template <int VARIANT>
__global__ __launch_bounds__(64) void moog_reset_kernel(KArgs a) {
  int env = blockIdx.x;
#if MOOG_WITH_MAZE
  const int pool_d = a.mode == MODE_FILL ? env / a.n_envs : 0;
  if (a.mode == MODE_FILL) env -= pool_d * a.n_envs;
  const size_t rec = (size_t)pool_d * a.n_envs + env;
#else
  const size_t rec = (size_t)env;
#endif
  if (env >= a.n_envs) return;
  int32_t* gq = a.i32 + rec * a.L.i32_per_env;
  if (a.mask != nullptr && a.mask[env] == 0) return;
  if (a.late_mask != nullptr && a.mode != MODE_FILL && a.late_mask[env] == 0) return;
  double* gf = a.f64 + rec * a.L.f64_per_env;
#if MOOG_WITH_MAZE
  if (a.mode == MODE_FILL) {
    if (pool_d >= a.pool_depth) return;
    const int32_t* lq = a.live_i32 + (size_t)env * a.L.i32_per_env;
    int won = 0;
    if (threadIdx.x == 0 && __hip_atomic_load(&a.pool_lock[env], __ATOMIC_RELAXED, __HIP_MEMORY_SCOPE_AGENT) == 0) {
      bool lower_busy = true;
      for (int d = 0; d < pool_d; ++d)
        lower_busy = lower_busy && __hip_atomic_load(&a.pool_state[(size_t)d * a.n_envs + env], __ATOMIC_RELAXED, __HIP_MEMORY_SCOPE_AGENT) != 0;
      int expect = 0;
      won = lower_busy && __hip_atomic_compare_exchange_strong(&a.pool_state[rec], &expect, 3, __ATOMIC_RELAXED, __ATOMIC_RELAXED,
                                                               __HIP_MEMORY_SCOPE_AGENT) ? 1 : 0;
    }
    if (!__shfl(won, 0)) return;
    __builtin_amdgcn_fence(__ATOMIC_ACQUIRE, "agent");
    const double* lf = a.live_f64 + (size_t)env * a.L.f64_per_env;
    pool_copy_record(a.L, (int)threadIdx.x, lf, lq, a.pool_f64[0] + rec * a.L.f64_per_env, a.pool_i32[0] + rec * a.L.i32_per_env);
    pool_copy_record(a.L, (int)threadIdx.x, a.pool_f64[0] + rec * a.L.f64_per_env, a.pool_i32[0] + rec * a.L.i32_per_env, gf, gq);
    __builtin_amdgcn_fence(__ATOMIC_SEQ_CST, "workgroup");
    __builtin_amdgcn_wave_barrier();
    int go = 0;
    if (threadIdx.x == 0) {
      const unsigned ep_live = (unsigned)gq[a.L.o_rng + 1];
      unsigned target = ep_live + 1u;
      for (int round = 0; round < a.pool_depth; ++round)
        for (int d = 0; d < a.pool_depth; ++d) {
          if (d == pool_d) continue;
          const size_t o = (size_t)d * a.n_envs + env;
          int st = __hip_atomic_load(&a.pool_state[o], __ATOMIC_RELAXED, __HIP_MEMORY_SCOPE_AGENT);
          for (int spins = 0; st == 3 && d < pool_d && spins < 100000; ++spins) {
            __builtin_amdgcn_s_sleep(2);
            st = __hip_atomic_load(&a.pool_state[o], __ATOMIC_RELAXED, __HIP_MEMORY_SCOPE_AGENT);
          }
          if ((st == 1 || st == 2) &&
              (unsigned)__hip_atomic_load(&a.pool_tag[o], __ATOMIC_RELAXED, __HIP_MEMORY_SCOPE_AGENT) == target) ++target;
        }
      __hip_atomic_store(&a.pool_tag[rec], (int32_t)target, __ATOMIC_RELAXED, __HIP_MEMORY_SCOPE_AGENT);
      __hip_atomic_store(&a.pool_state[rec], 1, __ATOMIC_RELEASE, __HIP_MEMORY_SCOPE_AGENT);
      const bool stable = __hip_atomic_load(&a.pool_lock[env], __ATOMIC_RELAXED, __HIP_MEMORY_SCOPE_AGENT) == 0 &&
                          (unsigned)__hip_atomic_load(&lq[a.L.o_rng + 1], __ATOMIC_RELAXED, __HIP_MEMORY_SCOPE_AGENT) == ep_live;
      if (stable) { gq[a.L.o_rng + 1] = (int32_t)(target - 1u); go = 1; }
      else __hip_atomic_store(&a.pool_state[rec], 0, __ATOMIC_RELAXED, __HIP_MEMORY_SCOPE_AGENT);
    }
    if (!__shfl(go, 0)) return;
    __builtin_amdgcn_fence(__ATOMIC_SEQ_CST, "workgroup");
    __builtin_amdgcn_wave_barrier();
  }
#endif
  Env e;
  bind_env(e, a, env);
#if MOOG_WITH_MAZE
  if (a.mode == MODE_FILL) {
    if (a.H.f_cut1 > a.H.f_cut0) e.gcol = gf + a.L.o_color;
    if (a.H.i_cut1 > a.H.i_cut0) { e.gopa = gq + a.L.o_opacity; e.gshape = gq + a.L.o_shape; e.gtele = gq + a.L.o_tele; }
  }
#endif
  load_record(e, a.H, a.L, gf, gq);
  if (e.inj && e.lane == 0) EQ(e)[EL(e).o_rng + 2] = 0;
  wsync();
  env_reset<true>(e);
  wsync();
#if MOOG_WITH_MAZE
  if (a.mode == MODE_FILL) {
    if (e.lane == 0) EQ(e)[EL(e).o_reset_next] = 0;
    store_record(e, a.H, a.L, gf, gq, nullptr);
    __builtin_amdgcn_fence(__ATOMIC_RELEASE, "agent");
    if (e.lane == 0) __hip_atomic_store(&a.pool_state[rec], 2, __ATOMIC_RELEASE, __HIP_MEMORY_SCOPE_AGENT);
    return;
  }
#endif
  if (e.lane == 0) {
    EQ(e)[EL(e).o_reset_next] = 0;
    if (a.reward) a.reward[env] = __builtin_nan("");
    if (a.discount) a.discount[env] = __builtin_nan("");
    if (a.step_type) a.step_type[env] = 0;
  }
  emit_draw_record(e, a, env);
  store_record(e, a.H, a.L, gf, gq, a.fault_flag);
#if MOOG_WITH_MAZE
  if (a.late_mask != nullptr) {
    if (a.pool_state) pool_release(a, env, e.lane);
    if (e.lane == 0) a.late_mask[env] = 0;
  }
#endif
}

#if !MOOG_RESET_FULL
#define SCHED_BINS 1024
#define SCHED_THREADS 256
#define SCHED_KEEP 16
__device__ __forceinline__ int sched_wave_scan(int v) {
  v += __builtin_amdgcn_update_dpp(0, v, 0x111, 0xf, 0xf, false);
  v += __builtin_amdgcn_update_dpp(0, v, 0x112, 0xf, 0xf, false);
  v += __builtin_amdgcn_update_dpp(0, v, 0x114, 0xf, 0xf, false);
  v += __builtin_amdgcn_update_dpp(0, v, 0x118, 0xf, 0xf, false);
  v += __builtin_amdgcn_update_dpp(0, v, 0x142, 0xa, 0xf, false);
  v += __builtin_amdgcn_update_dpp(0, v, 0x143, 0xc, 0xf, false);
  return v;
}
__device__ __forceinline__ float sched_cost(const float* cost, int i) { const float c = cost[i]; return (c >= 0.f && c < 3.0e38f) ? c : 0.f; }
__global__ __launch_bounds__(SCHED_THREADS) void moog_sched_kernel(const float* cost, int32_t* perm, int n,
                                                                    const int32_t* reset_next, int stride) {
  __shared__ int hist[SCHED_BINS];
  __shared__ float red[SCHED_THREADS / 64];
  __shared__ int wsum[SCHED_THREADS / 64];
  const int t = threadIdx.x;
  float c[SCHED_KEEP];
  int rn[SCHED_KEEP];
  float m = 0.f;
#pragma unroll
  for (int q = 0; q < SCHED_KEEP; ++q) {
    const int i = t + SCHED_THREADS * q;
    c[q] = i < n ? sched_cost(cost, i) : 0.f;
    rn[q] = i < n ? reset_next[(size_t)i * stride] : 0;
    m = fmaxf(m, c[q]);
  }
  for (int i = t + SCHED_THREADS * SCHED_KEEP; i < n; i += SCHED_THREADS) m = fmaxf(m, sched_cost(cost, i));
  for (int o = 32; o > 0; o >>= 1) m = fmaxf(m, __shfl_xor(m, o));
  if ((t & 63) == 0) red[t >> 6] = m;
  for (int b = t; b < SCHED_BINS; b += SCHED_THREADS) hist[b] = 0;
  __syncthreads();
  m = red[0];
  for (int w = 1; w < SCHED_THREADS / 64; ++w) m = fmaxf(m, red[w]);
  const float scale = m > 0.f ? (float)(SCHED_BINS - 1) / m : 0.f;
  auto bin_of = [&](float cv, int r) {
    int b = SCHED_BINS - 1 - (int)(cv * scale);
    b = b < 0 ? 0 : (b > SCHED_BINS - 1 ? SCHED_BINS - 1 : b);
    return r == 1 ? 0 : b;
  };
  int bq[SCHED_KEEP];
#pragma unroll
  for (int q = 0; q < SCHED_KEEP; ++q) {
    bq[q] = bin_of(c[q], rn[q]);
    if (t + SCHED_THREADS * q < n) atomicAdd(&hist[bq[q]], 1);
  }
  for (int i = t + SCHED_THREADS * SCHED_KEEP; i < n; i += SCHED_THREADS) atomicAdd(&hist[bin_of(sched_cost(cost, i), reset_next[(size_t)i * stride])], 1);
  __syncthreads();
  constexpr int PER = SCHED_BINS / SCHED_THREADS;
  int own[PER], v = 0;
#pragma unroll
  for (int k = 0; k < PER; ++k) { own[k] = hist[PER * t + k]; v += own[k]; }
  const int inc = sched_wave_scan(v);
  if ((t & 63) == 63) wsum[t >> 6] = inc;
  __syncthreads();
  int before = inc - v;
  for (int w = 0; w < (t >> 6); ++w) before += wsum[w];
#pragma unroll
  for (int k = 0; k < PER; ++k) { hist[PER * t + k] = before; before += own[k]; }
  __syncthreads();
#pragma unroll
  for (int q = 0; q < SCHED_KEEP; ++q) {
    const int i = t + SCHED_THREADS * q;
    if (i < n) perm[atomicAdd(&hist[bq[q]], 1)] = i;
  }
  for (int i = t + SCHED_THREADS * SCHED_KEEP; i < n; i += SCHED_THREADS)
    perm[atomicAdd(&hist[bin_of(sched_cost(cost, i), reset_next[(size_t)i * stride])], 1)] = i;
}
#endif

#endif

__device__ __forceinline__ double uni_f64(double x) {
  const long long b = __double_as_longlong(x);
  const unsigned lo = (unsigned)uni((int)b), hi = (unsigned)uni((int)(b >> 32));
  return __longlong_as_double((long long)(((unsigned long long)hi << 32) | lo));
}

template <bool DYN, bool REPEAT>
__device__ __forceinline__ void step_env(const KArgs& a, const int env, unsigned char* lds, const int lane) {
  const long long t_sched = a.cost ? clock64() : 0;
  int32_t* gq = a.i32 + (size_t)env * a.L.i32_per_env;
  Env e;
  bind_env(e, a, env, lds, lane);
  const long long t_begin = (a.dbg & 128) ? clock64() : 0;
  double* gf = a.f64 + (size_t)env * a.L.f64_per_env;
  { PROF_T0; load_record(e, a.H, a.L, gf, gq); PROF_ADD(e, 9); }
  if (e.inj && e.lane == 0) EQ(e)[EL(e).o_rng + 2] = 0;
  wsync();
  if (a.mode == MODE_STEP && uni(EQ(e)[EL(e).o_reset_next]) == 1) {
    int held = 0;
    if (!(DYN && pool_adopt(e, a, env, gf, gq, &held))) {
      if (DYN && a.late_mask) {
        if (e.lane == 0) { a.late_mask[env] = 1; if (a.repeat_count) a.repeat_count[env] = 0; }
        return;
      }
      env_reset<DYN>(e);
    }
    wsync();
    if (e.lane == 0) {
      EQ(e)[EL(e).o_reset_next] = 0;
      if (a.reward) a.reward[env] = __builtin_nan("");
      if (a.discount) a.discount[env] = __builtin_nan("");
      if (a.step_type) a.step_type[env] = 0;
      if (a.repeat_count) a.repeat_count[env] = 0;
#ifdef MOOG_PROFILE
      if ((a.dbg & 128) && a.discount) {
        a.discount[env] = (double)(clock64() - t_begin);
        if (a.reward) a.reward[env] = (a.dbg >> 8) ? (double)e.prof[((a.dbg >> 8) & 31) - 1] : 0.0;
      }
#endif
    }
    emit_draw_record(e, a, env);
    store_record(e, a.H, a.L, gf, gq, a.fault_flag);
    if (DYN && held) pool_release(a, env, e.lane);
    if (a.cost && e.lane == 0) a.cost[env] = moog_cost_ema((float)(clock64() - t_sched), a.cost[env]);
    return;
  }
  PProg P = as_const_prog(a.P);
  const int K = uni(P->updates_per_env_step);
  const int reps = REPEAT ? a.repeat : 1;
  int done = 0, sr = 0;
  double rsum = 0;
  for (;;) {
    if constexpr (REPEAT) { e.cell_tab_n = 0; e.cell_nw = 0; }
    { PROF_T0; bbox_build_all(e); PROF_ADD(e, 9); }
    if (a.mode == MODE_PHYSICS) {
      for (int k = 0; k < K; ++k) apply_physics<DYN>(e);
      store_record(e, a.H, a.L, gf, gq, a.fault_flag);
      return;
    }
    {
    PROF_T0;
    SEC(e, SEC_RULES);
    const int n_rules = uni(P->n_rules);
    for (int r = 0; r < n_rules; ++r)
      if (P->rules[r].parent < 0) rule_step<DYN>(e, r);
    const bool af32 = a.act_f32 != 0;
    if (uni(P->n_actions) > 1) {
      const int na = uni(P->n_actions);
      for (int k = 0; k < na; ++k) {
        double x, y;
        if (af32) { const float* act = reinterpret_cast<const float*>(a.actions) + (size_t)2 * na * env; x = act[2 * k]; y = act[2 * k + 1]; }
        else { const double* act = reinterpret_cast<const double*>(a.actions) + (size_t)2 * na * env; x = act[2 * k]; y = act[2 * k + 1]; }
        action_step(e, k, x, y, (int)x, af32);
      }
    } else {
      double ax = 0, ay = 0;
      int ga = 4;
      if (P->action.kind == MOOG_ACTION_GRID) ga = reinterpret_cast<const int32_t*>(a.actions)[env];
      else if (af32) {
        ax = reinterpret_cast<const float*>(a.actions)[2 * env];
        ay = reinterpret_cast<const float*>(a.actions)[2 * env + 1];
      } else {
        ax = reinterpret_cast<const double*>(a.actions)[2 * env];
        ay = reinterpret_cast<const double*>(a.actions)[2 * env + 1];
      }
      action_step(e, 0, ax, ay, ga, af32);
    }
    PROF_ADD(e, 10);
    }
    { PROF_T0; for (int k = 0; k < K; ++k) apply_physics<DYN>(e); PROF_ADD(e, 6); }
    SEC(e, SEC_TASK);
    int sc = EQ(e)[EL(e).o_step_count] + 1;
    wsync();
    if (e.lane == 0) EQ(e)[EL(e).o_step_count] = sc;
    wsync();
    double rj;
    { PROF_T0; rj = task_reward<DYN>(e, sc, &sr); PROF_ADD(e, 11); }
    wsync();
    if (!REPEAT || reps <= 1) { rsum = rj; done = 1; break; }
    sr = uni(sr);
    rj = uni_f64(rj);
    rsum = done == 0 ? rj : uni_f64(rsum + rj);
    if (++done >= reps || sr) break;
  }
  if (e.lane == 0) {
    if (sr) EQ(e)[EL(e).o_reset_next] = 1;
    if (a.reward) a.reward[env] = rsum;
    if (a.discount) a.discount[env] = sr ? 0.0 : 1.0;
    if (a.step_type) a.step_type[env] = sr ? 2 : 1;
    if (a.repeat_count) a.repeat_count[env] = done;
  }
  SEC(e, SEC_STORE);
  emit_draw_record(e, a, env);
  store_record(e, a.H, a.L, gf, gq, a.fault_flag);
  if (a.cost && e.lane == 0) a.cost[env] = moog_cost_ema((float)(clock64() - t_sched), a.cost[env]);
  if ((a.dbg & 128) && e.lane == 0 && a.discount) {
    a.discount[env] = (double)(clock64() - t_begin);
    if (a.reward) a.reward[env] = (double)(e.n_path + 100000 * e.n_resp) + 1e10 * (double)e.n_disj;
#ifdef MOOG_PROFILE
    if (a.reward && (a.dbg >> 8)) a.reward[env] = (double)e.prof[((a.dbg >> 8) & 31) - 1];
#endif
  }
}

template <bool DYN, int WPS, int VARIANT, bool REPEAT>
#ifdef MOOG_WATCH
#define MOOG_STEP_THREADS 128
#else
#define MOOG_STEP_THREADS 64
#endif
__global__ __launch_bounds__(MOOG_STEP_THREADS, WPS) void moog_step_kernel(KArgs a) {
  int env = (int)blockIdx.x + a.rank0;
  if (env >= a.n_envs) return;
#ifdef MOOG_WATCH
  if (a.watch) {
    int32_t* w = reinterpret_cast<int32_t*>(__builtin_assume_aligned(moog_lds + a.watch_off, 16));
    if (threadIdx.x == 0) { w[0] = 0; w[1] = 0; }
    __syncthreads();
    if (threadIdx.x >= 64) {
      const int lane = (int)threadIdx.x - 64;
      int count = 0;
      while (__hip_atomic_load(&w[1], __ATOMIC_RELAXED, __HIP_MEMORY_SCOPE_WORKGROUP) == 0) {
        const int sec = __hip_atomic_load(&w[0], __ATOMIC_RELAXED, __HIP_MEMORY_SCOPE_WORKGROUP);
        if (lane == (sec & (MOOG_WATCH_SECTIONS - 1))) ++count;
        __builtin_amdgcn_s_sleep(3);
      }
      const int real = a.perm ? a.perm[env] : env;
      if (lane < MOOG_WATCH_SECTIONS) atomicAdd(&a.watch[(size_t)real * MOOG_WATCH_SECTIONS + lane], count);
      return;
    }
  } else if (threadIdx.x >= 64) return;
#endif
  if (a.perm) env = a.perm[env];
#ifdef MOOG_SPEC_PROGRAM_INC
  {
    moog_layout_t L;
    moog_layout(&MOOG_SPEC_PROGRAM, &L);
    a.L = L;
    a.H = hot_layout(L);
  }
#endif
  step_env<DYN, REPEAT>(a, env, moog_lds, (int)threadIdx.x);
#ifdef MOOG_WATCH
  if (a.watch && threadIdx.x == 0) { int32_t* w = reinterpret_cast<int32_t*>(__builtin_assume_aligned(moog_lds + a.watch_off, 16)); __hip_atomic_store(w + 1, 1, __ATOMIC_RELAXED, __HIP_MEMORY_SCOPE_WORKGROUP); }
#endif
}


typedef void (*moog_step_launch_fn)(int n_envs, size_t lds, hipStream_t s, const KArgs& a);
void moog_launch_step_f3(int n_envs, size_t lds, hipStream_t s, const KArgs& a);
void moog_launch_step_f4(int n_envs, size_t lds, hipStream_t s, const KArgs& a);
void moog_launch_step_t3(int n_envs, size_t lds, hipStream_t s, const KArgs& a);
void moog_launch_step_t4(int n_envs, size_t lds, hipStream_t s, const KArgs& a);
void moog_launch_step_m3(int n_envs, size_t lds, hipStream_t s, const KArgs& a);
void moog_launch_step_m4(int n_envs, size_t lds, hipStream_t s, const KArgs& a);
void moog_launch_step_f3r(int n_envs, size_t lds, hipStream_t s, const KArgs& a);
void moog_launch_step_f4r(int n_envs, size_t lds, hipStream_t s, const KArgs& a);
void moog_launch_step_t3r(int n_envs, size_t lds, hipStream_t s, const KArgs& a);
void moog_launch_step_t4r(int n_envs, size_t lds, hipStream_t s, const KArgs& a);
void moog_launch_step_m3r(int n_envs, size_t lds, hipStream_t s, const KArgs& a);
void moog_launch_step_m4r(int n_envs, size_t lds, hipStream_t s, const KArgs& a);
int moog_configure_step_f3(size_t lds);
int moog_configure_step_f4(size_t lds);
int moog_configure_step_t3(size_t lds);
int moog_configure_step_t4(size_t lds);
int moog_configure_step_m3(size_t lds);
int moog_configure_step_m4(size_t lds);
int moog_configure_step_f3r(size_t lds);
int moog_configure_step_f4r(size_t lds);
int moog_configure_step_t3r(size_t lds);
int moog_configure_step_t4r(size_t lds);
int moog_configure_step_m3r(size_t lds);
int moog_configure_step_m4r(size_t lds);
void moog_launch_reset_plain(int n_envs, size_t lds, hipStream_t s, const KArgs& a);
void moog_launch_reset_full(int n_envs, size_t lds, hipStream_t s, const KArgs& a);
int moog_configure_reset_plain(size_t lds);
int moog_configure_reset_full(size_t lds);
void moog_launch_sched(hipStream_t s, const float* cost, int32_t* perm, int n, const int32_t* reset_next, int stride);
```

### moog.github.io_amd/csrc/moog_raster.h

```cpp
#pragma once
#include <hip/hip_runtime.h>
#include <stdint.h>

#include "../../include/moog_engine.h"
#include "moog_raster_mask_core.h"

#define R_THREADS 256
#define R_SLOW 8
#define R_CAP 12
#define R_KEY_BIAS 32768
#define R_XLIM 16000.0f
#define R_NONE ((short)-32768)
#define R_CNT_MASK 0x1ffu
#define R_FIX_ONE 0x200u
#define R_GENERIC 0x20000u
#define R_ITEM_SHIFT 18

struct RPlan {
  unsigned o_pbase, o_edge, o_ivert, o_long, o_list, o_xx, o_item_y, o_item_rgba, o_rowbase, o_rowoff, o_head,
      o_rows, o_seg, o_queue, o_misc, total;
};

struct RmSetup {
  int32_t ok;
  int32_t S, slots, ncopy, big, compact, cap_rows, iwords, cmap, first_person, fp_slot0, fp_nslots;
  uint32_t bg;
  RmPlan plan;
  uint32_t lds;
};

struct RArgs {
  RmSetup ms;
  RmEmit em;
  int32_t draw_ready, env0;
  int32_t* rows_seen;
  const moog_program_t* P;
  moog_layout_t L;
  const double* f64;
  const int32_t* i32;
  uint8_t* image;
  const uint32_t* vinfo;
  int32_t n_envs;
  int32_t chunk;
  int32_t words;
  int32_t tile_w;
  int32_t band_h;
  int32_t tiles_x;
  int32_t bands;
  int32_t canvas_w, canvas_h;
  int32_t scale_w;
  int32_t flip;
  int32_t iwords;
  int32_t hwords;
  int32_t debug_stop;
  RPlan plan;
  int32_t xxcap;
  int32_t n_static;
  int32_t nsv;
  int32_t build;
  const double* sref_v;
  const double* sref_col;
  const int32_t* sref_flags;
  const int32_t* sref_nv;
  const int32_t* sref_opa;
  const uint8_t* sbg;
  size_t sbg_env_stride;
  const uint32_t* rgb_override;
  const int32_t* env_build;
};

struct REdge { short x0, y0, x1, y1; float dx; short vtop, vbot; };

struct RRow { unsigned short key[R_CAP]; unsigned hbits; unsigned cnt; };

__host__ __device__ inline size_t r_align(size_t x) { return (x + 15) & ~(size_t)15; }

__host__ __device__ inline void raster_plan(int S, int TOTV, int ncopy, int W, int H, int cap_rows,
                                            int iwords, int hwords, int xxcap, RPlan* p) {
  size_t o = 0;
  size_t nv = (size_t)TOTV * ncopy, items = (size_t)S * ncopy;
  p->o_edge = o; o = r_align(o + nv * sizeof(REdge));
  {
    size_t v1 = nv * 4 + 8, v2 = (size_t)H * (W / 16) * iwords * 4;
    p->o_ivert = o; p->o_seg = o; o = r_align(o + (v1 > v2 ? v1 : v2));
  }
  size_t l1 = nv * 4, l2 = (size_t)xxcap * R_SLOW * 4;
  p->o_long = o; p->o_xx = o; o = r_align(o + (l1 > l2 ? l1 : l2));
  p->o_list = o; o = r_align(o + nv * 4);
  p->o_pbase = o; o = r_align(o + (size_t)S * 4);
  p->o_item_y = o; o = r_align(o + items * 8);
  p->o_item_rgba = o; o = r_align(o + items * 4);
  p->o_rowbase = o; o = r_align(o + items * 4);
  p->o_rowoff = o; o = r_align(o + (items + 1) * 4);
  p->o_head = o; o = r_align(o + items * hwords * 4);
  p->o_rows = o; o = r_align(o + (size_t)cap_rows * sizeof(RRow));
  p->o_queue = o; o = r_align(o + (size_t)cap_rows * 4);
  p->o_misc = o; o = r_align(o + 64);
  p->total = o;
}

struct RResize { int32_t cw, ch, ow, oh, kh, kv; const int32_t* bh; const int32_t* bv; const int32_t* ch_coef; const int32_t* cv_coef;
                 int32_t hspan;
                 int32_t cstride, tstride;  };
void moog_crop_launch(const uint8_t* in, uint8_t* out, size_t rows, int in_stride, int row_bytes, hipStream_t stream);
void moog_resize_launch(const RResize& r, const uint8_t* canvas, uint8_t* tmp, uint8_t* out, int n, hipStream_t stream);
int moog_raster_configure_mask(size_t lds_bytes);
int moog_raster_configure(size_t lds_bytes);
void moog_raster_launch(const RArgs& a, size_t lds_bytes, hipStream_t stream);
void moog_derive_launch(const RmEmit* em, int n_em, const RArgs& a, hipStream_t stream);
struct PCArgs {
  const moog_program_t* P; moog_layout_t L;
  const double* f64; const int32_t* i32;
  double* s_f64; int32_t* s_i32;
  int32_t* valid; int32_t* build; int32_t* min_changed;
  int32_t n_envs, n_static;
};
void moog_prefix_check_launch(const PCArgs& a, hipStream_t stream);
```

### moog.github.io_amd/csrc/moog_raster.hip

```cpp
#include <mutex>

#include "moog_raster_kernel.h"
#include "moog_raster_mask.h"

template <int WORDS>
__global__ __launch_bounds__(R_THREADS, 6) void moog_raster_kernel(RArgs a) { raster_block<WORDS>(a, (int)blockIdx.x, -1); }

static std::mutex g_lds_mu;
static size_t g_span_lds = 0, g_mask_lds = 0;

int moog_raster_configure_mask(size_t lds_bytes) {
  std::lock_guard<std::mutex> lock(g_lds_mu);
  if (lds_bytes <= g_mask_lds) return (int)hipSuccess;
  const int err = moog_raster_mask_configure(lds_bytes);
  if (err == (int)hipSuccess) g_mask_lds = lds_bytes;
  return err;
}

int moog_raster_configure(size_t lds_bytes) {
  std::lock_guard<std::mutex> lock(g_lds_mu);
  if (lds_bytes <= g_span_lds) return (int)hipSuccess;
  hipError_t err = hipFuncSetAttribute(reinterpret_cast<const void*>(moog_raster_kernel<1>),
                                       hipFuncAttributeMaxDynamicSharedMemorySize, (int)lds_bytes);
  if (err == hipSuccess)
    err = hipFuncSetAttribute(reinterpret_cast<const void*>(moog_raster_kernel<2>),
                              hipFuncAttributeMaxDynamicSharedMemorySize, (int)lds_bytes);
  if (err == hipSuccess) g_span_lds = lds_bytes;
  return (int)err;
}

static RmArgs mask_args(const RArgs& r) {
  RmArgs a;
  memset(&a, 0, sizeof a);
  a.draw = r.em.out; a.lay = r.em.lay; a.image = r.image;
  a.n_envs = r.n_envs; a.S = r.ms.S; a.big = r.ms.big; a.compact = r.ms.compact; a.cap_rows = r.ms.cap_rows; a.W = r.canvas_w; a.H = r.canvas_h;
  a.flip = r.flip; a.iwords = r.ms.iwords; a.bg = r.ms.bg; a.debug_stop = r.debug_stop; a.threads = RM_THREADS;
  a.n_static = r.em.ncopy > 1 ? 0 : r.em.n_static;
  a.sbg = r.sbg; a.rows_seen = r.rows_seen;
  a.plan = r.ms.plan;
  return a;
}

void moog_derive_launch(const RmEmit* em, int n_em, const RArgs& a, hipStream_t stream) {
  RmDeriveArgs d;
  memset(&d, 0, sizeof d);
  for (int k = 0; k < n_em && k < MOOG_MAX_VIEWS; ++k) d.em[k] = em[k];
  d.n_em = n_em < MOOG_MAX_VIEWS ? n_em : MOOG_MAX_VIEWS;
  d.P = a.P; d.L = a.L; d.f64 = a.f64; d.i32 = a.i32; d.vinfo = a.vinfo; d.n_envs = a.n_envs; d.env0 = a.env0;
  moog_draw_derive_launch(d, stream);
}

void moog_raster_launch(const RArgs& a, size_t lds_bytes, hipStream_t stream) {
  if (a.ms.ok && !a.build && a.sbg_env_stride == 0 && !a.env_build) {
    if (!a.draw_ready) {
      moog_derive_launch(&a.em, 1, a, stream);
    }
    moog_raster_mask_launch(mask_args(a), a.ms.lds, stream);
    return;
  }
  const dim3 grid((unsigned)a.n_envs * (unsigned)(a.tiles_x * a.bands));
  if (a.words > 1) hipLaunchKernelGGL(moog_raster_kernel<2>, grid, dim3(R_THREADS), lds_bytes, stream, a);
  else hipLaunchKernelGGL(moog_raster_kernel<1>, grid, dim3(R_THREADS), lds_bytes, stream, a);
}

#define R_PRECISION_BITS (32 - 8 - 2)
__device__ __forceinline__ unsigned r_clip8(int v) {
  v >>= R_PRECISION_BITS;
  return (unsigned)(v < 0 ? 0 : (v > 255 ? 255 : v));
}

__global__ __launch_bounds__(256) void moog_resize_h_kernel(RResize r, const uint8_t* in, uint8_t* tmp, int n) {
  extern __shared__ uint8_t stage[];
  const size_t row = (size_t)blockIdx.y + (size_t)blockIdx.z * 65535u;
  if (row >= (size_t)n * r.ch) return;
  const int x0 = (int)blockIdx.x * 256, xx = x0 + (int)threadIdx.x;
  const int xl = (x0 + 255 < r.ow) ? x0 + 255 : r.ow - 1;
  const int b0 = (3 * r.bh[2 * x0]) & ~3, b1 = 3 * (r.bh[2 * xl] + r.bh[2 * xl + 1]);
  const uint8_t* rowp = in + row * (size_t)r.cstride * 3;
  const uint32_t* src = reinterpret_cast<const uint32_t*>(rowp + b0);
  uint32_t* dst = reinterpret_cast<uint32_t*>(stage);
  const int ndw = (b1 - b0 + 3) >> 2;
  const int row_dw = (r.cstride * 3 - b0) >> 2;
  for (int t = threadIdx.x; t < ndw; t += 256) dst[t] = t < row_dw ? src[t] : 0u;
  __syncthreads();
  if (xx >= r.ow) return;
  const int xmin = r.bh[2 * xx], xmax = r.bh[2 * xx + 1];
  const int32_t* k = r.ch_coef + (size_t)xx * r.kh;
  const uint8_t* p = stage + (3 * xmin - b0);
  int s0 = 1 << (R_PRECISION_BITS - 1), s1 = s0, s2 = s0;
  for (int x = 0; x < xmax; ++x) { const int kk = k[x]; s0 += p[3 * x] * kk; s1 += p[3 * x + 1] * kk; s2 += p[3 * x + 2] * kk; }
  uint8_t* o = tmp + (row * r.tstride + xx) * 3;
  o[0] = (uint8_t)r_clip8(s0); o[1] = (uint8_t)r_clip8(s1); o[2] = (uint8_t)r_clip8(s2);
}

__global__ __launch_bounds__(256) void moog_resize_v_kernel(RResize r, const uint8_t* tmp, uint8_t* out, int n) {
  const int d = (int)blockIdx.x * 256 + (int)threadIdx.x;
  const int row_dw = (r.tstride * 3) >> 2;
  if (d >= row_dw) return;
  const int yy = (int)blockIdx.y;
  const size_t env = blockIdx.z;
  const int ymin = r.bv[2 * yy], ymax = r.bv[2 * yy + 1];
  const int32_t* k = r.cv_coef + (size_t)yy * r.kv;
  const uint8_t* p = tmp + (env * r.ch + ymin) * (size_t)r.tstride * 3 + 4 * (size_t)d;
  int s0 = 1 << (R_PRECISION_BITS - 1), s1 = s0, s2 = s0, s3 = s0;
  for (int y = 0; y < ymax; ++y) {
    const int kk = k[y];
    const uint32_t w = *reinterpret_cast<const uint32_t*>(p + (size_t)y * r.tstride * 3);
    s0 += (int)(w & 255u) * kk; s1 += (int)((w >> 8) & 255u) * kk; s2 += (int)((w >> 16) & 255u) * kk; s3 += (int)(w >> 24) * kk;
  }
  uint8_t* o = out + (env * r.oh + (r.oh - 1 - yy)) * (size_t)r.ow * 3;
  const int b = 4 * d, nb = r.ow * 3;
  if (b < nb) o[b] = (uint8_t)r_clip8(s0);
  if (b + 1 < nb) o[b + 1] = (uint8_t)r_clip8(s1);
  if (b + 2 < nb) o[b + 2] = (uint8_t)r_clip8(s2);
  if (b + 3 < nb) o[b + 3] = (uint8_t)r_clip8(s3);
}

__global__ __launch_bounds__(256) void moog_crop_kernel(const uint8_t* in, uint8_t* out, size_t rows, int in_stride, int row_bytes) {
  const size_t row = (size_t)blockIdx.x * 4 + (threadIdx.x >> 6);
  if (row >= rows) return;
  const uint8_t* src = in + row * (size_t)in_stride;
  uint8_t* dst = out + row * (size_t)row_bytes;
  for (int b = threadIdx.x & 63; b < row_bytes; b += 64) dst[b] = src[b];
}

__global__ __launch_bounds__(64) void moog_prefix_check_kernel(PCArgs a) {
  const int env = blockIdx.x, lane = threadIdx.x;
  if (env >= a.n_envs) return;
  PProg P = as_const_prog(a.P);
  const moog_layout_t& L = a.L;
  const double* gf = a.f64 + (size_t)env * L.f64_per_env;
  const int32_t* gq = a.i32 + (size_t)env * L.i32_per_env;
  double* sf = a.s_f64 + (size_t)env * L.f64_per_env;
  int32_t* sq = a.s_i32 + (size_t)env * L.i32_per_env;
  const int had = a.valid[env];
  int first_bad = a.n_static;
  if (had) {
    for (int s = lane; s < a.n_static; s += 64) {
      const int fl = gq[L.o_flags + s], nv = gq[L.o_nverts + s];
      bool bad = ((fl ^ sq[L.o_flags + s]) & MOOG_F_ALIVE) != 0;
      if (fl & MOOG_F_ALIVE) {
        bad = bad || nv != sq[L.o_nverts + s] || gq[L.o_opacity + s] != sq[L.o_opacity + s];
        for (int k = 0; k < 3; ++k)
          bad = bad || __double_as_longlong(gf[L.o_color + 3 * s + k]) != __double_as_longlong(sf[L.o_color + 3 * s + k]);
        const int v0 = L.o_verts + 2 * P->slot_voff[s];
        const int n2 = 2 * (nv < P->slot_vcap[s] ? nv : P->slot_vcap[s]);
        for (int k = 0; k < n2; ++k) bad = bad || __double_as_longlong(gf[v0 + k]) != __double_as_longlong(sf[v0 + k]);
      }
      if (bad && s < first_bad) first_bad = s;
    }
    for (int o = 32; o > 0; o >>= 1) { const int other = __shfl_xor(first_bad, o); first_bad = other < first_bad ? other : first_bad; }
  }
  const bool rebuild = !had || first_bad < a.n_static;
  if (rebuild) {
    const double2* src = reinterpret_cast<const double2*>(gf);
    double2* dst = reinterpret_cast<double2*>(sf);
    for (int i = lane; i < L.f64_per_env / 2; i += 64) dst[i] = src[i];
    const int4* srci = reinterpret_cast<const int4*>(gq);
    int4* dsti = reinterpret_cast<int4*>(sq);
    for (int i = lane; i < L.i32_per_env / 4; i += 64) dsti[i] = srci[i];
  }
  if (lane == 0) {
    a.build[env] = rebuild ? 1 : 0;
    a.valid[env] = 1;
    if (had && first_bad < a.n_static && gq[L.o_step_count] != 0)
      __hip_atomic_fetch_min(a.min_changed, first_bad, __ATOMIC_RELAXED, __HIP_MEMORY_SCOPE_SYSTEM);
  }
}

void moog_prefix_check_launch(const PCArgs& a, hipStream_t stream) {
  hipLaunchKernelGGL(moog_prefix_check_kernel, dim3((unsigned)a.n_envs), dim3(64), 0, stream, a);
}

void moog_crop_launch(const uint8_t* in, uint8_t* out, size_t rows, int in_stride, int row_bytes, hipStream_t stream) {
  hipLaunchKernelGGL(moog_crop_kernel, dim3((unsigned)((rows + 3) / 4)), dim3(256), 0, stream, in, out, rows, in_stride, row_bytes);
}

void moog_resize_launch(const RResize& r, const uint8_t* canvas, uint8_t* tmp, uint8_t* out, int n, hipStream_t stream) {
  const unsigned bx = (unsigned)((r.ow + 255) / 256);
  const size_t rows = (size_t)n * r.ch;
  const unsigned gy = (unsigned)(rows < 65535u ? rows : 65535u), gz = (unsigned)((rows + 65534u) / 65535u);
  hipLaunchKernelGGL(moog_resize_h_kernel, dim3(bx, gy, gz), dim3(256), (size_t)r.hspan, stream, r, canvas, tmp, n);
  const unsigned bd = (unsigned)(((r.tstride * 3 >> 2) + 255) / 256);
  for (int e0 = 0; e0 < n; e0 += 65535) {
    const int m = n - e0 < 65535 ? n - e0 : 65535;
    hipLaunchKernelGGL(moog_resize_v_kernel, dim3(bd, (unsigned)r.oh, (unsigned)m), dim3(256), 0, stream, r,
                       tmp + (size_t)e0 * r.ch * r.tstride * 3, out + (size_t)e0 * r.oh * r.ow * 3, m);
  }
}
```

### moog.github.io_amd/csrc/moog_raster_kernel.h

```cpp
#ifndef MOOG_RASTER_KERNEL_H_
#define MOOG_RASTER_KERNEL_H_
#include "moog_device.h"
#include "moog_raster.h"

extern __shared__ __attribute__((aligned(16))) unsigned char moog_lds[];

__device__ __forceinline__ int pil_round_up(float f) {
  return (int)copysignf(floorf(fabsf(f) + 0.5f), f);
}
__device__ __forceinline__ int pil_round_down(float f) {
  return (int)copysignf(ceilf(fabsf(f) - 0.5f), f);
}
__device__ __forceinline__ int key_up(unsigned k) {
  int s = (int)k - R_KEY_BIAS;
  return s >= 0 ? (s + 1) >> 1 : s >> 1;
}
__device__ __forceinline__ int key_down(unsigned k) {
  int s = (int)k - R_KEY_BIAS;
  return s >= 0 ? s >> 1 : (s + 1) >> 1;
}

__device__ inline void hsv_to_rgb_u8(double h, double s, double v, unsigned& r8, unsigned& g8,
                                     unsigned& b8) {
  double r, g, b;
// ... 276 lines not shown
#pragma unroll
      for (int j = q % p; j <= N - 1 - q; j += 2 * q) {
#pragma unroll
        for (int i = 0; i < q; ++i) {
          if (i + j + q <= N - 1 && (i + j) / (2 * p) == (i + j + q) / (2 * p)) {
            unsigned lo = min(k[i + j], k[i + j + q]), hi = max(k[i + j], k[i + j + q]);
            k[i + j] = lo; k[i + j + q] = hi;
          }
        }
      }
    }
  }
}

template <int WORDS>
__device__ __forceinline__ void mask_or_range(RMask& m, int W, int xoff, int xs, int xe, bool pred) {
  xs -= xoff; xe -= xoff;
  const int a = xs < 0 ? 0 : xs, b = xe > W - 1 ? W - 1 : xe;
  pred = pred && (a <= b);
  {
    const int hi = b < 63 ? b : 63;
    unsigned long long bits = (~0ull << (a & 63)) & (~0ull >> ((63 - hi) & 63));
    m.w0 |= (pred && a < 64) ? bits : 0ull;
  }
  if (WORDS > 1) {
    const int lo = a > 64 ? a - 64 : 0, hi = b - 64;
    unsigned long long bits = (~0ull << (lo & 63)) & (~0ull >> ((63 - hi) & 63));
    m.w1 |= (pred && b >= 64) ? bits : 0ull;
  }
}

template <int WORDS>
__device__ __forceinline__ void draw_one_head(bool act, int hxmin, int hxmax, int& x_pos, RMask& m, int W, int xoff) {
  bool hv = act && (x_pos == -1 || x_pos >= hxmin);
  const int hs = x_pos > hxmin ? x_pos : hxmin;
  hv = hv && !(x_pos > hxmin && hxmax < hs);
  if (__any(hv)) mask_or_range<WORDS>(m, W, xoff, hs, hxmax, hv);
  x_pos = hv ? hxmax + 1 : x_pos;
}

template <int NP, int N, int WORDS>
__device__ __forceinline__ RMask span_loop(const unsigned (&k)[N], int cnt, bool head, int hxmin, int hxmax, int W, int xoff) {
  RMask m = {0ull, 0ull};
  int x_pos = (cnt == 0) ? -1 : 0;
  const bool anyhead = __any(head);
#pragma unroll
  for (int q = 0; q < NP; ++q) {
    if (q >= 1 && !__any(2 * q + 1 < cnt)) break;
    const int x_end = key_down(k[2 * q + 1]);
    bool act = (2 * q + 1 < cnt) && (x_end >= x_pos);
    if (anyhead) {
      draw_one_head<WORDS>(act && head, hxmin, hxmax, x_pos, m, W, xoff);
      act = act && (x_end >= x_pos);
    }
    const int x_start = key_up(k[2 * q]);
    const bool gt = x_pos > x_start;
    const int xs = gt ? x_pos : x_start;
    act = act && !(gt && x_end < xs);
    mask_or_range<WORDS>(m, W, xoff, xs, x_end, act);
    x_pos = act ? x_end + 1 : x_pos;
  }
  if (anyhead) draw_one_head<WORDS>(head, hxmin, hxmax, x_pos, m, W, xoff);
  return m;
}

template <int WORDS>
__device__ __forceinline__ void draw_pending_heads(const REdge* pe, unsigned& hb, int& x_pos, RMask& m, int W, int xoff) {
  unsigned bits = hb;
  while (bits) {
    const int k = __ffs((int)bits) - 1;
    bits &= bits - 1u;
    const unsigned xb = (unsigned)__float_as_int(pe[k].dx);
    const int xmin = (short)(xb & 0xffffu), xmax = (short)(xb >> 16);
    if (x_pos != -1 && x_pos < xmin) continue;
    hb &= ~(1u << k);
    const int hs = x_pos > xmin ? x_pos : xmin;
    const bool draw = !(x_pos > xmin && xmax < hs);
    mask_or_range<WORDS>(m, W, xoff, hs, xmax, draw);
    x_pos = draw ? xmax + 1 : x_pos;
  }
}

template <int NP, int N, int WORDS>
__device__ __forceinline__ RMask span_loop_pending(const unsigned (&k)[N], int cnt, const REdge* pe, unsigned hb, int W, int xoff) {
  RMask m = {0ull, 0ull};
  int x_pos = (cnt == 0) ? -1 : 0;
#pragma unroll
  for (int q = 0; q < NP; ++q) {
    if (q >= 1 && !__any(2 * q + 1 < cnt)) break;
    const int x_end = key_down(k[2 * q + 1]);
    bool act = (2 * q + 1 < cnt) && (x_end >= x_pos);
    if (act) draw_pending_heads<WORDS>(pe, hb, x_pos, m, W, xoff);
    act = act && (x_end >= x_pos);
    const int x_start = key_up(k[2 * q]);
    const bool gt = x_pos > x_start;
    const int xs = gt ? x_pos : x_start;
    act = act && !(gt && x_end < xs);
    mask_or_range<WORDS>(m, W, xoff, xs, x_end, act);
    x_pos = act ? x_end + 1 : x_pos;
  }
  draw_pending_heads<WORDS>(pe, hb, x_pos, m, W, xoff);
  return m;
}

template <int NP, int N>
__device__ __forceinline__ RMask span_loop_poly(const unsigned (&k)[N], int cnt, const RPoly& p, int y, int W, int xoff) {
  RMask m = {0ull, 0ull};
  int x_pos = (cnt == 0) ? -1 : 0;
#pragma unroll
  for (int q = 0; q < NP; ++q) {
    if (q >= 1 && !__any(2 * q + 1 < cnt)) break;
    if (2 * q + 1 < cnt) {
      int x_end = key_down(k[2 * q + 1]);
      if (x_end >= x_pos) {
        draw_horizontal(p, y, &x_pos, m, W, xoff);
        if (x_end >= x_pos) {
          int x_start = key_up(k[2 * q]);
          bool skip = false;
          if (x_pos > x_start) { x_start = x_pos; skip = (x_end < x_start); }
          if (!skip) {
            mask_fill(m, W, xoff, x_start, x_end);
            x_pos = x_end + 1;
          }
        }
      }
    }
  }
  draw_horizontal(p, y, &x_pos, m, W, xoff);
  return m;
}

__device__ __forceinline__ unsigned blend8(unsigned bg, unsigned fg, unsigned al) {
  unsigned t = bg * (255u - al) + fg * al + 128u;
  return ((t >> 8) + t) >> 8;
}

__device__ __noinline__ void r_next_pass(RRow* rows, int cap_rows, int* misc, int tid) {
  for (int i = tid; i < cap_rows; i += R_THREADS) {
    uint4* r = reinterpret_cast<uint4*>(rows + i);
    r[0] = make_uint4(~0u, ~0u, ~0u, ~0u);
    r[1] = make_uint4(~0u, ~0u, 0u, 0u);
  }
  if (tid == 0) { misc[1] = 0; misc[2] = 0; misc[3] = 0; misc[4] = 0; }
}

template <int WORDS>
__device__ __forceinline__ void raster_block(const RArgs& a, const int block, const int env_of_block) {
  const int tiles = a.tiles_x * a.bands;
  const int benv = a.tiles_x * a.bands == 1 ? block : block / tiles;
  if (benv >= a.n_envs) return;
  const int tile_id = block - benv * tiles;
  const int env = env_of_block >= 0 ? env_of_block : benv;
  if (a.build && a.env_build && a.env_build[env] == 0) return;
  const int band = tile_id / a.tiles_x;
  PProg P = as_const_prog(a.P);
  const int WF = a.canvas_w, H = a.canvas_h;
  const int W = a.tile_w;
  const int xoff = (tile_id - band * a.tiles_x) * a.tile_w;
  const int yb0 = band * a.band_h, yb1 = (yb0 + a.band_h < H) ? yb0 + a.band_h : H;
  const int S = P->n_slots, TOTV = a.L.TOTV;
  const bool torus = (P->render.polymod == MOOG_POLYMOD_TORUS);
  const int ncopy = torus ? 9 : 1;
  const int words = WORDS, iwords = a.iwords, hwords = a.hwords, cap_rows = a.chunk;
  const int nseg = W >> 4;
  const int items = S * ncopy;
  const double* gf = a.f64 + (size_t)env * a.L.f64_per_env;
  const int32_t* gq = a.i32 + (size_t)env * a.L.i32_per_env;
  const int tid = threadIdx.x, lane = tid & 63;
#ifdef MOOG_RASTER_PROFILE
  const bool clk = (a.debug_stop == 11);
  const long long T0 = clk ? clock64() : 0;
  long long T1 = 0, T2 = 0, T3 = 0, T4 = 0, T5 = 0, T6 = 0, TA = 0, TB = 0;
#define R_CLK(t) if (clk) t = clock64()
#else
#define R_CLK(t)
#endif

  const RPlan& pl = a.plan;
  REdge* edges = reinterpret_cast<REdge*>(moog_lds + pl.o_edge);
  short2* ivert = reinterpret_cast<short2*>(moog_lds + pl.o_ivert);
  unsigned* longlist = reinterpret_cast<unsigned*>(moog_lds + pl.o_long);
  unsigned* list = reinterpret_cast<unsigned*>(moog_lds + pl.o_list);
  float* xxs = reinterpret_cast<float*>(moog_lds + pl.o_xx);
  int* pbase = reinterpret_cast<int*>(moog_lds + pl.o_pbase);
  int* item_y = reinterpret_cast<int*>(moog_lds + pl.o_item_y);
  unsigned* item_rgba = reinterpret_cast<unsigned*>(moog_lds + pl.o_item_rgba);
  int* rowbase = reinterpret_cast<int*>(moog_lds + pl.o_rowbase);
  int* rowoff = reinterpret_cast<int*>(moog_lds + pl.o_rowoff);
  unsigned* headmask = reinterpret_cast<unsigned*>(moog_lds + pl.o_head);
  RRow* rows = reinterpret_cast<RRow*>(moog_lds + pl.o_rows);
  unsigned* segitems = reinterpret_cast<unsigned*>(moog_lds + pl.o_seg);
  unsigned short* queue = reinterpret_cast<unsigned short*>(moog_lds + pl.o_queue);
  int* misc = reinterpret_cast<int*>(moog_lds + pl.o_misc);

  unsigned vi_next = 0u;
  double2 v_next = make_double2(0.0, 0.0);
  const bool per_env = a.sbg_env_stride != 0;
  const int NS = (a.build || per_env) ? 0 : a.n_static;
  const int NSE = (per_env && !a.build) ? a.n_static : 0;
  const int S0 = NSE & ~63, V0 = NSE == 0 ? 0 : ((int)a.nsv / R_THREADS) * R_THREADS;
  const uint8_t* sbg = a.sbg + (size_t)env * a.sbg_env_stride;
  bool st_bad = false;
  if (V0 + tid < TOTV) {
    vi_next = a.vinfo[V0 + tid];
    v_next = *reinterpret_cast<const double2*>(gf + a.L.o_verts + 2 * (V0 + tid));
  }
  for (int i = tid; i < items; i += R_THREADS) { item_y[2 * i] = 0x7fffffff; item_y[2 * i + 1] = -0x7fffffff; }
  for (int i = tid; i < items * hwords; i += R_THREADS) headmask[i] = 0u;
  for (int i = tid; i < cap_rows; i += R_THREADS) {
    uint4* r = reinterpret_cast<uint4*>(rows + i);
    r[0] = make_uint4(~0u, ~0u, ~0u, ~0u);
    r[1] = make_uint4(~0u, ~0u, 0u, 0u);
  }
  if (tid < 8) misc[tid] = 0;
  for (int s = tid; s < S0; s += R_THREADS) {
    pbase[s] = P->slot_voff[s];
    for (int c = 0; c < ncopy; ++c) item_rgba[s * ncopy + c] = 0u;
  }
  for (int s = S0 + tid - (R_THREADS - 64); s >= S0 && s < S; s += 64) {
    const int flags = gq[a.L.o_flags + s];
    const int nvs = gq[a.L.o_nverts + s], opa = gq[a.L.o_opacity + s];
    const double* col = gf + a.L.o_color + 3 * s;
    const double c0 = col[0], c1 = col[1], c2 = col[2];
    const bool alive = (flags & MOOG_F_ALIVE) != 0 && !(a.build && s >= a.n_static) && s >= NSE;
    if (s < NS) {
      const double* rc = a.sref_col + 3 * s;
      st_bad = st_bad || ((flags ^ a.sref_flags[s]) & MOOG_F_ALIVE) != 0 || nvs != a.sref_nv[s] || opa != a.sref_opa[s] ||
               __double_as_longlong(c0) != __double_as_longlong(rc[0]) ||
               __double_as_longlong(c1) != __double_as_longlong(rc[1]) ||
               __double_as_longlong(c2) != __double_as_longlong(rc[2]);
    }
    bool in_tile = true;
    if (tiles > 1 && alive && !torus && P->render.polymod != MOOG_POLYMOD_FIRST_PERSON) {
      const double px = gf[a.L.o_pos + 2 * s], py = gf[a.L.o_pos + 2 * s + 1], rad = gf[a.L.o_maxr + s];
      const double x0 = (px - rad) * (double)a.scale_w - 2.0, x1 = (px + rad) * (double)a.scale_w + 2.0;
      const double y0 = (py - rad) * (double)H - 2.0, y1 = (py + rad) * (double)H + 2.0;
      if (x1 < (double)xoff || x0 > (double)(xoff + W) || y1 < (double)yb0 || y0 > (double)yb1) in_tile = false;
    }
    pbase[s] = P->slot_voff[s] | (((alive && in_tile) ? nvs : 0) << 20);
    unsigned rgba = 0u;
    if (alive) {
      unsigned r8, g8, b8;
      if (a.rgb_override) {
        const unsigned o = a.rgb_override[(size_t)env * S + s];
        r8 = o & 255u; g8 = (o >> 8) & 255u; b8 = (o >> 16) & 255u;
      } else if (P->render.cmap == MOOG_CMAP_HSV) hsv_to_rgb_u8(c0, c1, c2, r8, g8, b8);
      else { r8 = (unsigned)(int)c0 & 255u; g8 = (unsigned)(int)c1 & 255u; b8 = (unsigned)(int)c2 & 255u; }
      rgba = r8 | (g8 << 8) | (b8 << 16) | (((unsigned)opa & 255u) << 24);
    }
    for (int c = 0; c < ncopy; ++c) item_rgba[s * ncopy + c] = rgba;
  }
  const bool first_person = (P->render.polymod == MOOG_POLYMOD_FIRST_PERSON);
  double fpx = 0, fpy = 0;
  if (first_person) {
    int l = P->render.polymod_layer;
    for (int s = P->layer_slot0[l]; s < P->layer_slot0[l] + P->layer_nslots[l]; ++s)
      if (gq[a.L.o_flags + s] & MOOG_F_ALIVE) {
        fpx = 0.5 - gf[a.L.o_pos + 2 * s]; fpy = 0.5 - gf[a.L.o_pos + 2 * s + 1];
        break;
      }
  }
  __syncthreads();
  if (a.debug_stop == 1) return;

  unsigned vi_keep0 = 0u, vi_keep1 = 0u;
  for (int idx = V0 + tid; idx < TOTV; idx += R_THREADS) {
    const unsigned vi = vi_next;
    const double2 v = v_next;
    if (idx == V0 + tid) vi_keep0 = vi; else if (idx == V0 + tid + R_THREADS) vi_keep1 = vi;
    if (idx + R_THREADS < TOTV) {
      vi_next = a.vinfo[idx + R_THREADS];
      v_next = *reinterpret_cast<const double2*>(gf + a.L.o_verts + 2 * (idx + R_THREADS));
    }
    int s = vi & 0xffu, k = (vi >> 8) & 0xffu;
    if (k >= (pbase[s] >> 20)) continue;
    if (idx < a.nsv && NS > 0) {
      const double2 r = *reinterpret_cast<const double2*>(a.sref_v + 2 * idx);
      st_bad = st_bad || __double_as_longlong(v.x) != __double_as_longlong(r.x) ||
               __double_as_longlong(v.y) != __double_as_longlong(r.y);
    }
    for (int c = 0; c < ncopy; ++c) {
      double vx = v.x, vy = v.y;
      if (torus) { vx = vx + (double)(c / 3 - 1); vy = vy + (double)(c % 3 - 1); }
      if (first_person) { vx = vx + fpx; vy = vy + fpy; }
      int ix = pil_int((double)a.scale_w * vx), iy = pil_int((double)H * vy);
      short2 o; o.x = clamp16(ix); o.y = clamp16(iy);
      ivert[c * TOTV + idx] = o;
      int it = s * ncopy + c;
      atomicMin(&item_y[2 * it], (int)o.y);
      atomicMax(&item_y[2 * it + 1], (int)o.y);
    }
  }
  if (st_bad) misc[5] = 1;
  __syncthreads();
  if (a.debug_stop == 2) return;
  const int s_lo = per_env ? NSE : ((NS > 0 && misc[5] == 0) ? NS : 0);

  for (int c = 0; c < ncopy; ++c) {
    for (int base0 = V0; base0 < TOTV; base0 += R_THREADS) {
      int idx = base0 + tid;
      int kind = 0;
      unsigned vi = 0u;
      if (idx < TOTV) vi = base0 == V0 ? vi_keep0 : (base0 == V0 + R_THREADS ? vi_keep1 : a.vinfo[idx]);
      if (idx < TOTV) {
        int s = vi & 0xffu, k = (vi >> 8) & 0xffu;
        int nv = pbase[s] >> 20;
// ... 388 lines not shown
```

### moog.github.io_amd/csrc/moog_raster_mask.h

```cpp
#ifndef MOOG_RASTER_MASK_H_
#define MOOG_RASTER_MASK_H_
#include <hip/hip_runtime.h>

#include "moog_raster_mask_core.h"


extern __shared__ __attribute__((aligned(16))) unsigned char moog_lds[];

template <int WORDS, bool BIG, bool COMPACT>
__global__ __launch_bounds__(RM_THREADS, RM_WAVES_PER_SIMD) void moog_raster_mask_kernel(RmArgs a) {
  const RmCtx c = rm_ctx(a.plan, moog_lds);
  const int tid = (int)threadIdx.x, lane = tid & 63;
  const int env = (int)blockIdx.x;
  if (env >= a.n_envs) return;
  rm_load(a, c, env, tid, RM_THREADS);
  __syncthreads();
  if (a.debug_stop == 1 || a.debug_stop == 2) return;
  const int s_lo = __builtin_amdgcn_readfirstlane(rm_s_lo(a, c));
  const bool single = __builtin_amdgcn_readfirstlane(c.misc[6]) != 0;
  if (a.rows_seen && tid == 0 && c.rowoff[a.S] > a.cap_rows) {
    atomicMax(a.rows_seen, c.rowoff[a.S]);
    atomicAdd(a.rows_seen + 1, 1);
  }
  for (int base = 0;;) {
    const int end = __builtin_amdgcn_readfirstlane(rm_pass_end(a, c, base));
    const int total_rows = __builtin_amdgcn_readfirstlane(c.rowoff[end] - c.rowoff[base]);
    if (!single) {
      rm_p2_assign(a, c, base, end, s_lo, lane);
      __builtin_amdgcn_fence(__ATOMIC_ACQ_REL, "wavefront");
      __builtin_amdgcn_wave_barrier();
    }
    if (a.debug_stop == 3) return;
    rm_p3<WORDS, COMPACT>(a, c, base, end, s_lo, tid, RM_THREADS);
    __syncthreads();
    if (a.debug_stop == 4) return;
    if (a.cap_rows <= RM_SORT_ROUNDS * RM_THREADS) {
      RmSortKey sk;
      rm_p4a(c, total_rows, tid, RM_THREADS, sk);
      __syncthreads();
      rm_p4b(c, total_rows, tid, RM_THREADS, sk);
      __syncthreads();
    } else {
      rm_p4a_lds(c, total_rows, tid, RM_THREADS);
      __syncthreads();
      rm_p4b_lds(c, total_rows, tid, RM_THREADS);
      __syncthreads();
    }
    rm_p4<WORDS, COMPACT>(a, c, total_rows, tid, RM_THREADS, c.xx + (tid >> 6) * a.plan.xx_stride);
    if (BIG) rm_p4_big<WORDS, COMPACT>(a, c, tid, RM_THREADS, c.xx + (tid >> 6) * a.plan.xx_stride, reinterpret_cast<uint8_t*>(c.xx + (RM_THREADS / 64) * a.plan.xx_stride));
    __syncthreads();
    if (a.debug_stop == 5) return;
    rm_p5<WORDS>(a, c, env, base == 0, s_lo, tid, RM_THREADS);
    if (end >= a.S) break;
    base = end;
    __syncthreads();
    rm_next_pass(a, c, tid, RM_THREADS);
    __syncthreads();
  }
}

struct RmDeriveArgs { RmEmit em[MOOG_MAX_VIEWS]; const moog_program_t* P; moog_layout_t L; const double* f64; const int32_t* i32; const uint32_t* vinfo; int32_t n_envs; int32_t env0; int32_t n_em; };
__global__ __launch_bounds__(64) void moog_draw_derive_kernel(RmDeriveArgs d) {
  const int env = (int)blockIdx.x;
  if (env >= d.n_envs) return;
  RmSrcRecord src;
  src.P = d.P; src.L = &d.L; src.f = d.f64 + (size_t)env * d.L.f64_per_env; src.q = d.i32 + (size_t)env * d.L.i32_per_env; src.vi = d.vinfo;
#pragma unroll
  for (int k = 0; k < MOOG_MAX_VIEWS; ++k) {
    if (k >= d.n_em) break;
    if (k > 0) __syncthreads();
    RmEmit em = d.em[k];
    if (em.rgb_override) em.rgb_override += (size_t)d.env0 * em.slots;
    RmEmitScratch sc;
    rm_emit_scratch(reinterpret_cast<int32_t*>(moog_lds), em.slots, em.ncopy, &sc);
    rm_emit(em, src, env, (int)threadIdx.x, sc, d.L.TOTV);
  }
}

typedef void (*moog_raster_mask_fn)(RmArgs);
static inline moog_raster_mask_fn moog_raster_mask_pick(int words, bool big, bool compact) {
  static const moog_raster_mask_fn table[2][2][2] = {
      {{moog_raster_mask_kernel<1, false, false>, moog_raster_mask_kernel<1, false, true>},
       {moog_raster_mask_kernel<1, true, false>, moog_raster_mask_kernel<1, true, true>}},
      {{moog_raster_mask_kernel<2, false, false>, moog_raster_mask_kernel<2, false, true>},
       {moog_raster_mask_kernel<2, true, false>, moog_raster_mask_kernel<2, true, true>}}};
  return table[words - 1][big ? 1 : 0][compact ? 1 : 0];
}

static inline int moog_raster_mask_configure(size_t lds_bytes) {
  hipError_t err = hipSuccess;
  for (int k = 0; k < 8 && err == hipSuccess; ++k)
    err = hipFuncSetAttribute(reinterpret_cast<const void*>(moog_raster_mask_pick(1 + (k & 1), (k & 2) != 0, (k & 4) != 0)),
                              hipFuncAttributeMaxDynamicSharedMemorySize, (int)lds_bytes);
  return (int)err;
}

static inline void moog_raster_mask_launch(const RmArgs& a, size_t lds_bytes, hipStream_t stream) {
  hipLaunchKernelGGL(moog_raster_mask_pick(a.W > 64 ? 2 : 1, a.big != 0, a.compact != 0), dim3((unsigned)a.n_envs), dim3(RM_THREADS), lds_bytes, stream, a);
}

static inline void moog_draw_derive_launch(const RmDeriveArgs& d, hipStream_t stream) {
  size_t words = 0;
  for (int k = 0; k < d.n_em; ++k) {
    const size_t w = (size_t)RM_EMIT_SCRATCH_WORDS(d.em[k].slots, d.em[k].S, d.em[k].ncopy);
    if (w > words) words = w;
  }
  hipLaunchKernelGGL(moog_draw_derive_kernel, dim3((unsigned)d.n_envs), dim3(64), 4u * words, stream, d);
}

#endif
```

### moog.github.io_amd/csrc/moog_raster_mask_core.h

```cpp
#ifndef MOOG_RASTER_MASK_CORE_H_
#define MOOG_RASTER_MASK_CORE_H_
#include "moog_draw_record.h"

#define RM_THREADS 128
#define RM_WAVES_PER_SIMD 5
#define RM_SORT_ROUNDS_T (3 * RM_THREADS)
#define RM_XX (2 * RM_BIG_NV)

struct alignas(16) RmEdge { uint32_t w0, w1, w2, w3; };
struct alignas(16) RmRow { uint32_t act, heads, tipP, tipN; };
struct alignas(16) RmItem { int32_t rowbase; int32_t pb_nv; int32_t pymax; uint32_t rgba; };

struct alignas(16) RmU4 { uint32_t x, y, z, w; };

struct RmPlan { uint32_t o_edge, o_ivert, o_rows, o_rowitem, o_info, o_item_y, o_rowoff, o_seg, o_lut, o_xx, o_misc, o_spare, o_owner, o_skey, xx_stride, total; };

struct RmArgs {
  const uint8_t* draw;
  RmDrawLayout lay;
  uint8_t* image;
  int32_t n_envs;
  int32_t S;
  int32_t big;
  int32_t compact;
  int32_t cap_rows;
  int32_t W, H;
  int32_t flip;
  int32_t iwords;
  uint32_t bg;
  int32_t debug_stop;
  int32_t threads;
  int32_t n_static;
  const uint8_t* sbg;
  int32_t* rows_seen;
  RmPlan plan;
};

static inline uint32_t rm_align(uint32_t x) { return (x + 15u) & ~15u; }

static inline void rm_plan(int S, int TOTV, int W, int H, int cap_rows, int iwords, int waves, int big, RmPlan* p, int compact = 0) {
  uint32_t o = 0;
  p->o_edge = o; o = rm_align(o + (uint32_t)TOTV * (compact ? 4u : (uint32_t)sizeof(RmEdge)));
  p->o_ivert = o; o = rm_align(o + (uint32_t)TOTV * 4u);
  p->o_rows = o; o = rm_align(o + (uint32_t)cap_rows * sizeof(RmRow));
  p->o_rowitem = o; o = rm_align(o + (uint32_t)cap_rows * 2u);
  p->o_info = o; o = rm_align(o + (uint32_t)S * sizeof(RmItem));
  p->o_item_y = o; o = rm_align(o + (uint32_t)S * 8u);
  p->o_rowoff = o; o = rm_align(o + (uint32_t)(S + 1) * 4u);
  p->o_seg = o; o = rm_align(o + (uint32_t)H * (uint32_t)(W / 16) * (uint32_t)iwords * 4u);
  p->o_lut = o; o = rm_align(o + 16u * 16u);
  p->xx_stride = big ? (uint32_t)RM_XX : 2u * RM_MAX_NV;
  p->o_xx = o; o = rm_align(o + (uint32_t)waves * p->xx_stride * 4u + (big ? (uint32_t)waves * 64u * RM_MAX_NV : 0u));
  p->o_misc = o; o = rm_align(o + 64u);
  p->o_owner = o; o = rm_align(o + (uint32_t)TOTV);
  p->o_skey = o; o = rm_align(o + (cap_rows > RM_SORT_ROUNDS_T ? (uint32_t)cap_rows * 2u : 0u));
  {
    const uint32_t b1 = (uint32_t)waves * 64u * 4u, b2 = (uint32_t)cap_rows * 2u;
    p->o_spare = o; o = rm_align(o + (b1 > b2 ? b1 : b2));
  }
  p->total = o;
}

struct RmCtx {
  RmEdge* edges; uint32_t* ivert; RmRow* rows; uint16_t* rowitem;
  RmItem* info; int32_t* item_y; int32_t* rowoff;
  uint32_t* seg; uint32_t* lut; float* xx; uint32_t* spare; uint16_t* sorted; uint16_t* skey; uint8_t* owner; int32_t* misc;
};

RM_FN RmCtx rm_ctx(const RmPlan& pl, unsigned char* lds) {
  RmCtx c;
  c.edges = reinterpret_cast<RmEdge*>(lds + pl.o_edge);
  c.ivert = reinterpret_cast<uint32_t*>(lds + pl.o_ivert);
  c.rows = reinterpret_cast<RmRow*>(lds + pl.o_rows);
  c.rowitem = reinterpret_cast<uint16_t*>(lds + pl.o_rowitem);
  c.info = reinterpret_cast<RmItem*>(lds + pl.o_info);
  c.item_y = reinterpret_cast<int32_t*>(lds + pl.o_item_y);
  c.rowoff = reinterpret_cast<int32_t*>(lds + pl.o_rowoff);
  c.seg = reinterpret_cast<uint32_t*>(lds + pl.o_seg);
  c.lut = reinterpret_cast<uint32_t*>(lds + pl.o_lut);
  c.xx = reinterpret_cast<float*>(lds + pl.o_xx);
  c.misc = reinterpret_cast<int32_t*>(lds + pl.o_misc);
  c.spare = reinterpret_cast<uint32_t*>(lds + pl.o_spare);
  c.sorted = reinterpret_cast<uint16_t*>(lds + pl.o_spare);
  c.owner = reinterpret_cast<uint8_t*>(lds + pl.o_owner);
  c.skey = reinterpret_cast<uint16_t*>(lds + pl.o_skey);
  return c;
}

RM_FN int rm_ffs(uint32_t m) { return __builtin_ctz(m); }
RM_FN void rm_or(uint32_t* p, uint32_t v) {
#if RM_DEV
  atomicOr(p, v);
#else
  *p |= v;
#endif
}
RM_FN int rm_f2i(float f) {
  if (!(f > -2147483648.0f)) return (int)0x80000000;
  if (!(f < 2147483648.0f)) return 0x7fffffff;
  return (int)f;
}
RM_FN int rm_round_up(float f) { return rm_f2i(copysignf(floorf(fabsf(f) + 0.5f), f)); }
RM_FN int rm_round_down(float f) { return rm_f2i(copysignf(ceilf(fabsf(f) - 0.5f), f)); }
template <int WORDS> struct RmMask { uint64_t w[WORDS]; };
RM_FN uint64_t rm_low(int t) { return t <= 0 ? 0ull : (t >= 64 ? ~0ull : ((1ull << t) - 1ull)); }
RM_FN uint64_t rm_high(int t) { return t >= 64 ? 0ull : (~0ull << (t & 63)); }
RM_FN uint64_t rm_high1(int t) { return t <= 64 ? ~0ull : rm_high(t - 64); }
template <int WORDS> RM_FN void rm_clear(RmMask<WORDS>& m) { for (int i = 0; i < WORDS; ++i) m.w[i] = 0ull; }
template <int WORDS> RM_FN bool rm_bit(const RmMask<WORDS>& m, int p) { return (m.w[WORDS > 1 ? (p >> 6) : 0] >> (p & 63)) & 1ull; }
template <int WORDS> RM_FN void rm_or_range(RmMask<WORDS>& m, int a, int b) {
  if (a < 0) a = 0;
  if (b > 64 * WORDS - 1) b = 64 * WORDS - 1;
  if (a > b) return;
  m.w[0] |= rm_low(b + 1) & ~rm_low(a);
  if (WORDS > 1) m.w[1] |= rm_low(b + 1 - 64) & ~rm_low(a - 64);
}

RM_FN int rm_y0(const RmEdge& e) { return (int)(int16_t)(e.w2 & 0xffffu); }
RM_FN int rm_y1(const RmEdge& e) { return (int)(int32_t)e.w2 >> 16; }
RM_FN float rm_xat(const RmEdge& e, int y) { return (float)(y - rm_y0(e)) * rm_u2f(e.w1) + rm_u2f(e.w0); }

#define RM_NO_EDGE 0x7fff8000u
struct RmEdgesFull {
  const RmEdge* pe;
  RM_MEMBER RmEdge operator[](int k) const { return pe[k]; }
};
struct RmEdgesCompact {
  const uint32_t* pv; const uint32_t* dx; int nv;
  RM_MEMBER RmEdge operator[](int k) const {
    const uint32_t q0 = pv[k], q1 = pv[(k + 1 >= nv) ? 0 : k + 1], w = dx[k];
    const bool table = (q0 >> 16) != (q1 >> 16), head = !table && w != RM_NO_EDGE;
    RmEdge E;
    E.w0 = table ? rm_f2u((float)(int)(int16_t)(q0 & 0xffffu)) : (head ? w : 0u);
    E.w1 = table ? w : 0u;
    E.w2 = table ? ((q0 >> 16) | (q1 & 0xffff0000u)) : (head ? ((q0 >> 16) | (q0 & 0xffff0000u)) : 0u);
    E.w3 = head ? 1u : 0u;
    return E;
  }
};
template <bool COMPACT> struct RmEdgeTab;
template <> struct RmEdgeTab<false> {
  typedef RmEdgesFull View;
  template <class C> static RM_MEMBER View view(const C& c, int first, int nv) { (void)nv; View v; v.pe = c.edges + first; return v; }
  template <class C> static RM_MEMBER void put(const C& c, int idx, const RmEdge& E, bool table, bool head) { (void)table; (void)head; c.edges[idx] = E; }
};
template <> struct RmEdgeTab<true> {
  typedef RmEdgesCompact View;
  template <class C> static RM_MEMBER View view(const C& c, int first, int nv) { View v; v.pv = c.ivert + first; v.dx = reinterpret_cast<const uint32_t*>(c.edges) + first; v.nv = nv; return v; }
  template <class C> static RM_MEMBER void put(const C& c, int idx, const RmEdge& E, bool table, bool head) {
    reinterpret_cast<uint32_t*>(c.edges)[idx] = table ? E.w1 : (head ? E.w0 : RM_NO_EDGE);
  }
};

RM_FN int rm_build_edge(const uint32_t* pv, int k, int nv, RmEdge* out) {
  const int k2 = (k + 1 == nv) ? 0 : k + 1;
  const uint32_t q0 = pv[k], q1 = pv[k2];
  const int x0 = (int16_t)(q0 & 0xffffu), y0 = (int16_t)(q0 >> 16), x1 = (int16_t)(q1 & 0xffffu), y1 = (int16_t)(q1 >> 16);
  const bool closing = (k == nv - 1);
  if (y0 != y1) {
    out->w0 = rm_f2u((float)x0);
    out->w1 = rm_f2u(((float)(x1 - x0)) / (float)(y1 - y0));
    out->w2 = (q0 >> 16) | (q1 & 0xffff0000u);
    out->w3 = 0u;
    return 1;
  }
  if (closing && x0 == x1) return 0;
  if (k >= 1 && !closing) {
    const uint32_t qp = pv[k - 1];
    const int xp = (int16_t)(qp & 0xffffu), yp = (int16_t)(qp >> 16);
    if (yp == y0 && ((x1 > x0 && x0 > xp) || (x1 < x0 && x0 < xp))) return 0;
    if (xp == x0 && yp == y0 && x1 == x0) return 0;
  }
  int hx = x1;
  {
    int q = k + 1;
    int px = x0, cx = x1;
    while (q <= nv - 2) {
      const uint32_t qn = pv[q + 1];
      const int nx = (int16_t)(qn & 0xffffu), ny = (int16_t)(qn >> 16);
      const bool ab = (ny == y0) && ((nx > cx && cx > px) || (nx < cx && cx < px));
      if (!ab) break;
      hx = nx; px = cx; cx = nx; ++q;
    }
  }
  const int xmin = x0 < hx ? x0 : hx, xmax = x0 < hx ? hx : x0;
  out->w0 = (uint32_t)(uint16_t)xmin | ((uint32_t)(uint16_t)xmax << 16);
  out->w1 = 0u;
  out->w2 = (q0 >> 16) | (q0 & 0xffff0000u);
// ... 737 lines not shown
```

### moog.github.io_amd/csrc/moog_reset.hip

```cpp
#include <hip/hip_runtime.h>

#define MOOG_DEFINE_RESET_KERNELS
#define MOOG_WITH_MAZE MOOG_RESET_FULL
#include "moog_kernels.h"

#if MOOG_RESET_FULL
#define RESET_FN(name) name##_full
#else
#define RESET_FN(name) name##_plain
#endif

void RESET_FN(moog_launch_reset)(int n_envs, size_t lds, hipStream_t s, const KArgs& a) {
  hipLaunchKernelGGL(moog_reset_kernel<MOOG_RESET_FULL>, dim3(n_envs), dim3(64), lds, s, a);
}

int RESET_FN(moog_configure_reset)(size_t lds) {
  return (int)hipFuncSetAttribute(reinterpret_cast<const void*>(moog_reset_kernel<MOOG_RESET_FULL>),
                                  hipFuncAttributeMaxDynamicSharedMemorySize, (int)lds);
}

#if !MOOG_RESET_FULL
void moog_launch_sched(hipStream_t s, const float* cost, int32_t* perm, int n, const int32_t* reset_next, int stride) {
  hipLaunchKernelGGL(moog_sched_kernel, dim3(1), dim3(SCHED_THREADS), 0, s, cost, perm, n, reset_next, stride);
}
#endif
```

### moog.github.io_amd/moog/_engine.py

```python
import ctypes
import os

from . import _abi

_HERE = os.path.dirname(os.path.abspath(__file__))
LIB_PATH = os.path.normpath(os.path.join(_HERE, '..', 'lib', 'libmoog_hip.so'))

SYMBOLS = (
    'moog_abi_version', 'moog_source_digest', 'moog_last_error', 'moog_program_sizeof', 'moog_engine_create',
    'moog_engine_destroy', 'moog_engine_layout', 'moog_engine_load_state', 'moog_engine_reset',
    'moog_engine_step', 'moog_engine_physics_only', 'moog_engine_render',
    'moog_engine_set_timing', 'moog_engine_kernel_time', 'moog_engine_set_schedule',
    'moog_engine_set_debug', 'moog_engine_static_prefix', 'moog_engine_poll_faults',
    'moog_engine_layer_usage', 'moog_engine_set_action_dtype', 'moog_engine_set_action_repeat',
    'moog_engine_read_watch', 'moog_engine_set_reset_pool', 'moog_engine_get_reset_pool',
    'moog_engine_env_prefix', 'moog_engine_set_color_override',
    'moog_engine_kernel_variant', 'moog_engine_raster_path', 'moog_engine_read_draw_records', 'moog_program_step_kernel', 'moog_engine_step_kernel',
    'moog_engine_add_view', 'moog_engine_set_view_image', 'moog_engine_view_raster_path',
)

_LIB = None


class EngineError(RuntimeError):
    pass


def load_library(path=None):
    global _LIB
    if _LIB is not None and path is None:
        return _LIB
    path = path or os.environ.get('MOOG_HIP_LIB', LIB_PATH)
    import torch
    if not os.path.exists(path):
        raise EngineError(
            'HIP engine library not found at %s -- build it with '
            '`python __graft_entry__.py` (hipcc --offload-arch=gfx950); there is no CPU fallback'
            % path)
    lib = ctypes.CDLL(path)
    vp, i32, i64, u64 = ctypes.c_void_p, ctypes.c_int32, ctypes.c_int64, ctypes.c_uint64
    lib.moog_abi_version.restype = ctypes.c_int
    lib.moog_source_digest.restype = ctypes.c_uint64
    lib.moog_last_error.restype = ctypes.c_char_p
    lib.moog_program_sizeof.restype = i64
    lib.moog_engine_create.argtypes = [ctypes.POINTER(_abi.Program), i32, i32, u64, i64,
                                       ctypes.POINTER(vp)]
    lib.moog_engine_destroy.argtypes = [vp]
    lib.moog_engine_layout.argtypes = [vp, ctypes.POINTER(_abi.Layout)]
    lib.moog_engine_load_state.argtypes = [vp, ctypes.POINTER(_abi.StateView)]
    lib.moog_engine_reset.argtypes = [vp, vp, ctypes.POINTER(_abi.Inject),
                                      ctypes.POINTER(_abi.StepOut), vp]
    lib.moog_engine_step.argtypes = [vp, vp, ctypes.POINTER(_abi.Inject),
                                     ctypes.POINTER(_abi.StepOut), vp]
    lib.moog_engine_physics_only.argtypes = [vp, ctypes.POINTER(_abi.Inject), vp]
    lib.moog_engine_render.argtypes = [vp, vp, vp]
    lib.moog_engine_set_schedule.argtypes = [vp, vp, vp]
    lib.moog_engine_set_timing.argtypes = [vp, i32]
    lib.moog_engine_set_reset_pool.argtypes = [vp, i32]
    lib.moog_engine_env_prefix.argtypes = [vp, ctypes.POINTER(i32)]
    lib.moog_engine_set_color_override.argtypes = [vp, vp]
    lib.moog_engine_kernel_variant.argtypes = [vp, ctypes.POINTER(i32), ctypes.POINTER(i32)]
    lib.moog_engine_raster_path.argtypes = [vp, ctypes.POINTER(i32)]
    lib.moog_engine_add_view.argtypes = [vp, ctypes.POINTER(_abi.Render), ctypes.POINTER(i32)]
    lib.moog_engine_set_view_image.argtypes = [vp, i32, vp]
    lib.moog_engine_view_raster_path.argtypes = [vp, i32, ctypes.POINTER(i32)]
    lib.moog_engine_read_draw_records.argtypes = [vp, vp, i64, ctypes.POINTER(i64), ctypes.POINTER(i32)]
    lib.moog_program_step_kernel.argtypes = [ctypes.POINTER(_abi.Program), ctypes.POINTER(i32), ctypes.POINTER(i32), ctypes.POINTER(u64)]
    lib.moog_engine_step_kernel.argtypes = [vp, ctypes.POINTER(i32)]
    lib.moog_engine_get_reset_pool.argtypes = [vp, ctypes.POINTER(i32), ctypes.POINTER(i64)]
    lib.moog_engine_set_action_dtype.argtypes = [vp, i32]
    lib.moog_engine_set_action_repeat.argtypes = [vp, i32, vp]
    lib.moog_engine_layer_usage.argtypes = [vp, ctypes.POINTER(i32), ctypes.POINTER(i32)]
    lib.moog_engine_set_debug.argtypes = [vp, i32, i32]
    lib.moog_engine_static_prefix.argtypes = [vp, ctypes.POINTER(i32), vp, vp]
    lib.moog_engine_poll_faults.argtypes = [vp, i32, ctypes.POINTER(i32)]
    lib.moog_engine_kernel_time.argtypes = [vp, i32, ctypes.POINTER(ctypes.c_double),
                                            ctypes.POINTER(i64)]
    for name in SYMBOLS:
        fn = getattr(lib, name)
        if name not in ('moog_last_error', 'moog_program_sizeof', 'moog_abi_version', 'moog_source_digest'):
            fn.restype = ctypes.c_int
    if lib.moog_abi_version() != _abi.MOOG_ABI_VERSION:
        raise EngineError('ABI mismatch: library %d, header %d'
                          % (lib.moog_abi_version(), _abi.MOOG_ABI_VERSION))
    if lib.moog_program_sizeof() != ctypes.sizeof(_abi.Program):
        raise EngineError('moog_program_t size mismatch: library %d, python %d'
                          % (lib.moog_program_sizeof(), ctypes.sizeof(_abi.Program)))
    if path == os.environ.get('MOOG_HIP_LIB', LIB_PATH):
        _LIB = lib
    return lib


def check(lib, rc):
    if rc != 0:
        msg = lib.moog_last_error()
        raise EngineError('engine call failed (%d): %s' % (rc, msg.decode() if msg else '?'))
```

Baseline: 6.319 million env steps/sec.

## Fold cost-sorted schedule into step kernel with last-block prefix and raster scatter

Removes the separate single-block sort kernel that ran on a side stream with event synchronisation. Each env now bins its own cost into a global histogram during the step kernel. The last env to finish computes the prefix sum, and the scatter into the permutation happens inside the raster kernel, or in a small scatter kernel when no image is produced. This drops one serial single-block kernel and the cross-stream waits, at the cost of global atomics per env and a one-step-stale bin scale.

```diff
diff --git a/__graft_entry__.py b/__graft_entry__.py
--- a/__graft_entry__.py
+++ b/__graft_entry__.py
@@ -12,8 +12,8 @@
 sys.path.insert(0, PKG)
 from moog import _digest
 HIP_FLAGS = _digest.HIP_FLAGS
-_STEP_DEPS = ['moog_device.h', 'moog_kernels.h', 'moog_draw_record.h']
-_RASTER_DEPS = ['moog_device.h', 'moog_raster.h', 'moog_raster_kernel.h', 'moog_raster_mask.h', 'moog_raster_mask_core.h', 'moog_draw_record.h']
+_STEP_DEPS = ['moog_device.h', 'moog_kernels.h', 'moog_draw_record.h', 'moog_sched.h']
+_RASTER_DEPS = ['moog_device.h', 'moog_raster.h', 'moog_raster_kernel.h', 'moog_raster_mask.h', 'moog_raster_mask_core.h', 'moog_draw_record.h', 'moog_sched.h']
 UNITS = [('moog_engine.o', 'moog_engine.hip', [], _STEP_DEPS + _RASTER_DEPS),
          ('moog_raster.o', 'moog_raster.hip', [], _RASTER_DEPS),
          ('moog_reset_r0.o', 'moog_reset.hip', ['-DMOOG_RESET_FULL=0'], _STEP_DEPS),
diff --git a/include/moog_engine.h b/include/moog_engine.h
--- a/include/moog_engine.h
+++ b/include/moog_engine.h
@@ -483,6 +483,7 @@
 int moog_engine_view_raster_path(moog_engine_t* e, int32_t view, int32_t* path);
 
 int moog_engine_set_schedule(moog_engine_t* e, int32_t* perm_dev, float* cost_dev);
+int moog_engine_schedule_state(moog_engine_t* e, int32_t* hist_nonzero, int32_t* done);
 
 
 int moog_engine_set_reset_pool(moog_engine_t* e, int32_t enabled);
diff --git a/moog.github.io_amd/csrc/moog_engine.hip b/moog.github.io_amd/csrc/moog_engine.hip
--- a/moog.github.io_amd/csrc/moog_engine.hip
+++ b/moog.github.io_amd/csrc/moog_engine.hip
@@ -85,10 +85,9 @@
   size_t aa_canvas_bytes = 0, aa_tmp_bytes = 0;
   int timing = 0;
   int32_t* perm = nullptr;
-  hipStream_t sched_stream = nullptr;
-  hipEvent_t ev_step_done = nullptr, ev_sched_done = nullptr;
-  bool sched_pending = false;
   float* cost = nullptr;
+  int32_t* order_ws = nullptr;
+  int32_t* order_key = nullptr;
   static constexpr int POOL_STREAMS = 8;
   int pool_streams = 2;
   bool pool_on = false, pool_ready = false;
@@ -153,6 +152,8 @@
   if (e->pool_tag) hipFree(e->pool_tag);
   if (e->pool_lock) hipFree(e->pool_lock);
   if (e->late_mask) hipFree(e->late_mask);
+  if (e->order_ws) hipFree(e->order_ws);
+  if (e->order_key) hipFree(e->order_key);
   if (e->pool_stats) hipFree(e->pool_stats);
   for (int k = 0; k < 2; ++k) { if (e->pool_f64[k]) hipFree(e->pool_f64[k]); if (e->pool_i32[k]) hipFree(e->pool_i32[k]); }
   if (e->watch) hipFree(e->watch);
@@ -761,11 +762,6 @@
 int moog_engine_destroy(moog_engine_t* e) {
   if (!e) return MOOG_OK;
   for (int k = 0; k < MOOG_K_COUNT; ++k) drain(e->timed[k]);
-  if (e->sched_stream) {
-    hipStreamSynchronize(e->sched_stream);
-    hipEventDestroy(e->ev_step_done); hipEventDestroy(e->ev_sched_done);
-    hipStreamDestroy(e->sched_stream);
-  }
   void* spec = e->spec_handle;
   free_engine(e);
   (void)spec;
@@ -825,6 +821,9 @@
   a.vslot = e->d_vslot;
   a.perm = (mode == MODE_STEP && e->perm) ? e->perm : nullptr;
   a.cost = (mode == MODE_STEP) ? e->cost : nullptr;
+  const bool order = a.perm && a.cost && e->order_ws;
+  a.sched_ws = order ? e->order_ws : nullptr;
+  a.sched_key = order ? e->order_key : nullptr;
   a.dbg = e->step_dbg;
   a.fault_flag = e->fault_flag;
   a.layer_hw = e->layer_hw;
@@ -904,6 +903,7 @@
   r.sbg = v.s_bg;
   r.sbg_env_stride = 0; r.env_build = nullptr; r.rgb_override = e->rgb_override;
   r.em = emit_args(e, v); r.draw_ready = 0; r.env0 = 0;
+  memset(&r.sched, 0, sizeof r.sched);
   return r;
 }
 
@@ -930,10 +930,18 @@
   return MOOG_OK;
 }
 
-static int launch_raster(moog_engine* e, RView& v, uint8_t* image, hipStream_t s, bool draw_ready = false) {
+static SchedScatter order_scatter(moog_engine* e) {
+  SchedScatter sc;
+  sc.ws = e->order_ws; sc.key = e->order_key; sc.perm = e->perm; sc.n = e->n_envs;
+  return sc;
+}
+static bool order_in_raster(moog_engine* e, const moog_step_out_t* out) { return out && out->image && e->views[0].aa <= 1; }
+
+static int launch_raster(moog_engine* e, RView& v, uint8_t* image, hipStream_t s, bool draw_ready = false, bool order = false) {
   RArgs r = raster_args(e, v, image);
   r.draw_ready = draw_ready ? 1 : 0;
   if (v.aa <= 1 && &v == &e->views[0]) { const int rc = use_env_prefix(e, r, s); if (rc) return rc; }
+  if (order && v.aa <= 1) r.sched = order_scatter(e);
   if (v.aa <= 1 && v.pad_w != v.canvas_w) {
     r.image = v.pad_img;
     moog_raster_launch(r, v.raster_lds, s);
@@ -964,13 +972,13 @@
   return v.aa <= 1 || v.aa_chunk >= e->n_envs;
 }
 
-static int launch_frames(moog_engine* e, uint8_t* image, hipStream_t s, bool draw_ready = false, int timed = -1) {
+static int launch_frames(moog_engine* e, uint8_t* image, hipStream_t s, bool draw_ready = false, int timed = -1, bool order = false) {
   RView* extra[MOOG_MAX_VIEWS];
   int n_extra = 0;
   for (int k = 1; k < e->n_views; ++k) if (e->views[k].image) extra[n_extra++] = &e->views[k];
   if (n_extra == 0) {
     Bracket br(e, MOOG_K_RASTER, s, timed);
-    return launch_raster(e, e->views[0], image, s, draw_ready);
+    return launch_raster(e, e->views[0], image, s, draw_ready, order);
   }
   RView& p = e->views[0];
   const bool join = !draw_ready && derives_ahead(e, p);
@@ -989,7 +997,7 @@
     }
   }
   Bracket br(e, MOOG_K_RASTER, s, timed);
-  return launch_raster(e, p, image, s, draw_ready || join);
+  return launch_raster(e, p, image, s, draw_ready || join, order);
 }
 
 static int pool_kick(moog_engine* e, hipStream_t s) {
@@ -1062,10 +1070,6 @@
   KArgs a = make_args(e, actions_dev, inject, out, MODE_STEP, nullptr);
   const bool emit = out && out->image && step_emits_draw(e);
   if (emit) a.draw = emit_args(e, e->views[0]);
-  if (e->sched_pending) {
-    HIPCHK(hipStreamWaitEvent(s, e->ev_sched_done, 0));
-    e->sched_pending = false;
-  }
   {
     Bracket br(e, MOOG_K_STEP, s);
     launch_step(e, s, a);
@@ -1073,15 +1077,12 @@
   }
   HIPCHK(hipGetLastError());
   if (a.pool_state && (rc = pool_kick(e, s)) != MOOG_OK) return rc;
-  if (e->perm && e->cost) {
-    HIPCHK(hipEventRecord(e->ev_step_done, s));
-    HIPCHK(hipStreamWaitEvent(e->sched_stream, e->ev_step_done, 0));
-    moog_launch_sched(e->sched_stream, e->cost, e->perm, e->n_envs,
-                      e->view.i32 + e->L.o_reset_next, e->L.i32_per_env);
-    HIPCHK(hipEventRecord(e->ev_sched_done, e->sched_stream));
-    e->sched_pending = true;
-  }
-  if (out && out->image) return launch_frames(e, out->image, s, emit);
+  const bool order = a.sched_ws != nullptr, in_raster = order && order_in_raster(e, out);
+  if (order && !in_raster) {
+    moog_launch_sched_scatter(s, order_scatter(e));
+    HIPCHK(hipGetLastError());
+  }
+  if (out && out->image) return launch_frames(e, out->image, s, emit, -1, in_raster);
   return MOOG_OK;
 }
 
@@ -1108,19 +1109,29 @@
 
 int moog_engine_set_schedule(moog_engine_t* e, int32_t* perm_dev, float* cost_dev) {
   if (!e) return fail(MOOG_E_INVALID, "null engine");
-  if (e->sched_pending) { hipEventSynchronize(e->ev_sched_done); e->sched_pending = false; }
   e->perm = perm_dev;
   e->cost = cost_dev;
   if (perm_dev && cost_dev) {
     HIPCHK(hipSetDevice(e->device));
     HIPCHK(hipMemset(cost_dev, 0, (size_t)e->n_envs * sizeof(float)));
-  }
-  if (perm_dev && cost_dev && !e->sched_stream) {
-    HIPCHK(hipSetDevice(e->device));
-    HIPCHK(hipStreamCreateWithFlags(&e->sched_stream, hipStreamNonBlocking));
-    HIPCHK(hipEventCreateWithFlags(&e->ev_step_done, hipEventDisableTiming));
-    HIPCHK(hipEventCreateWithFlags(&e->ev_sched_done, hipEventDisableTiming));
-  }
+    if (!e->order_ws) HIPCHK(hipMalloc(&e->order_ws, sizeof(int32_t) * SCHED_W_WORDS));
+    if (!e->order_key) HIPCHK(hipMalloc(&e->order_key, sizeof(int32_t) * 2 * (size_t)e->n_envs));
+    HIPCHK(hipMemset(e->order_ws, 0, sizeof(int32_t) * SCHED_W_WORDS));
+    HIPCHK(hipMemset(e->order_key, 0, sizeof(int32_t) * 2 * (size_t)e->n_envs));
+  }
+  return MOOG_OK;
+}
+
+int moog_engine_schedule_state(moog_engine_t* e, int32_t* hist_nonzero, int32_t* done) {
+  if (!e || !hist_nonzero || !done) return fail(MOOG_E_INVALID, "null argument");
+  *hist_nonzero = 0; *done = 0;
+  if (!e->order_ws) return MOOG_OK;
+  HIPCHK(hipSetDevice(e->device));
+  HIPCHK(hipDeviceSynchronize());
+  std::vector<int32_t> w(SCHED_W_BASE);
+  HIPCHK(hipMemcpy(w.data(), e->order_ws, sizeof(int32_t) * SCHED_W_BASE, hipMemcpyDeviceToHost));
+  for (int b = 0; b < SCHED_BINS; ++b) *hist_nonzero += w[SCHED_W_HIST + b] != 0;
+  *done = w[SCHED_W_DONE];
   return MOOG_OK;
 }
 
diff --git a/moog.github.io_amd/csrc/moog_kernels.h b/moog.github.io_amd/csrc/moog_kernels.h
--- a/moog.github.io_amd/csrc/moog_kernels.h
+++ b/moog.github.io_amd/csrc/moog_kernels.h
@@ -1,6 +1,7 @@
 #pragma once
 #include "moog_device.h"
 #include "moog_draw_record.h"
+#include "moog_sched.h"
 
 static __device__ __forceinline__ float moog_cost_ema(float now, float before) {
   return (before >= 0.f && before < 3.0e38f) ? 0.4f * before + 0.6f * now : now;
@@ -130,6 +131,8 @@
   int32_t dbg;
   const int32_t* perm;
   float* cost;
+  int32_t* sched_ws;
+  int32_t* sched_key;
   int32_t* fault_flag;
   int32_t* layer_hw;
   int32_t act_f32;
@@ -469,75 +472,9 @@
 }
 
 #if !MOOG_RESET_FULL
-#define SCHED_BINS 1024
-#define SCHED_THREADS 256
-#define SCHED_KEEP 16
-__device__ __forceinline__ int sched_wave_scan(int v) {
-  v += __builtin_amdgcn_update_dpp(0, v, 0x111, 0xf, 0xf, false);
-  v += __builtin_amdgcn_update_dpp(0, v, 0x112, 0xf, 0xf, false);
-  v += __builtin_amdgcn_update_dpp(0, v, 0x114, 0xf, 0xf, false);
-  v += __builtin_amdgcn_update_dpp(0, v, 0x118, 0xf, 0xf, false);
-  v += __builtin_amdgcn_update_dpp(0, v, 0x142, 0xa, 0xf, false);
-  v += __builtin_amdgcn_update_dpp(0, v, 0x143, 0xc, 0xf, false);
-  return v;
-}
-__device__ __forceinline__ float sched_cost(const float* cost, int i) { const float c = cost[i]; return (c >= 0.f && c < 3.0e38f) ? c : 0.f; }
-__global__ __launch_bounds__(SCHED_THREADS) void moog_sched_kernel(const float* cost, int32_t* perm, int n,
-                                                                    const int32_t* reset_next, int stride) {
-  __shared__ int hist[SCHED_BINS];
-  __shared__ float red[SCHED_THREADS / 64];
-  __shared__ int wsum[SCHED_THREADS / 64];
-  const int t = threadIdx.x;
-  float c[SCHED_KEEP];
-  int rn[SCHED_KEEP];
-  float m = 0.f;
-#pragma unroll
-  for (int q = 0; q < SCHED_KEEP; ++q) {
-    const int i = t + SCHED_THREADS * q;
-    c[q] = i < n ? sched_cost(cost, i) : 0.f;
-    rn[q] = i < n ? reset_next[(size_t)i * stride] : 0;
-    m = fmaxf(m, c[q]);
-  }
-  for (int i = t + SCHED_THREADS * SCHED_KEEP; i < n; i += SCHED_THREADS) m = fmaxf(m, sched_cost(cost, i));
-  for (int o = 32; o > 0; o >>= 1) m = fmaxf(m, __shfl_xor(m, o));
-  if ((t & 63) == 0) red[t >> 6] = m;
-  for (int b = t; b < SCHED_BINS; b += SCHED_THREADS) hist[b] = 0;
-  __syncthreads();
-  m = red[0];
-  for (int w = 1; w < SCHED_THREADS / 64; ++w) m = fmaxf(m, red[w]);
-  const float scale = m > 0.f ? (float)(SCHED_BINS - 1) / m : 0.f;
-  auto bin_of = [&](float cv, int r) {
-    int b = SCHED_BINS - 1 - (int)(cv * scale);
-    b = b < 0 ? 0 : (b > SCHED_BINS - 1 ? SCHED_BINS - 1 : b);
-    return r == 1 ? 0 : b;
-  };
-  int bq[SCHED_KEEP];
-#pragma unroll
-  for (int q = 0; q < SCHED_KEEP; ++q) {
-    bq[q] = bin_of(c[q], rn[q]);
-    if (t + SCHED_THREADS * q < n) atomicAdd(&hist[bq[q]], 1);
-  }
-  for (int i = t + SCHED_THREADS * SCHED_KEEP; i < n; i += SCHED_THREADS) atomicAdd(&hist[bin_of(sched_cost(cost, i), reset_next[(size_t)i * stride])], 1);
-  __syncthreads();
-  constexpr int PER = SCHED_BINS / SCHED_THREADS;
-  int own[PER], v = 0;
-#pragma unroll
-  for (int k = 0; k < PER; ++k) { own[k] = hist[PER * t + k]; v += own[k]; }
-  const int inc = sched_wave_scan(v);
-  if ((t & 63) == 63) wsum[t >> 6] = inc;
-  __syncthreads();
-  int before = inc - v;
-  for (int w = 0; w < (t >> 6); ++w) before += wsum[w];
-#pragma unroll
-  for (int k = 0; k < PER; ++k) { hist[PER * t + k] = before; before += own[k]; }
-  __syncthreads();
-#pragma unroll
-  for (int q = 0; q < SCHED_KEEP; ++q) {
-    const int i = t + SCHED_THREADS * q;
-    if (i < n) perm[atomicAdd(&hist[bq[q]], 1)] = i;
-  }
-  for (int i = t + SCHED_THREADS * SCHED_KEEP; i < n; i += SCHED_THREADS)
-    perm[atomicAdd(&hist[bin_of(sched_cost(cost, i), reset_next[(size_t)i * stride])], 1)] = i;
+__global__ __launch_bounds__(64) void moog_sched_scatter_kernel(SchedScatter s) {
+  const int env = (int)blockIdx.x * 64 + (int)threadIdx.x;
+  if (env < s.n) sched_scatter(s, env);
 }
 #endif
 
@@ -565,6 +502,7 @@
     if (!(DYN && pool_adopt(e, a, env, gf, gq, &held))) {
       if (DYN && a.late_mask) {
         if (e.lane == 0) { a.late_mask[env] = 1; if (a.repeat_count) a.repeat_count[env] = 0; }
+        if (a.sched_ws) sched_fold(a.sched_ws, a.sched_key, a.n_envs, env, e.lane, e.lane == 0 ? a.cost[env] : 0.f, 0);
         return;
       }
       env_reset<DYN>(e);
@@ -586,7 +524,11 @@
     emit_draw_record(e, a, env);
     store_record(e, a.H, a.L, gf, gq, a.fault_flag);
     if (DYN && held) pool_release(a, env, e.lane);
-    if (a.cost && e.lane == 0) a.cost[env] = moog_cost_ema((float)(clock64() - t_sched), a.cost[env]);
+    if (a.cost) {
+      float c = 0.f;
+      if (e.lane == 0) a.cost[env] = c = moog_cost_ema((float)(clock64() - t_sched), a.cost[env]);
+      if (a.sched_ws) sched_fold(a.sched_ws, a.sched_key, a.n_envs, env, e.lane, c, 0);
+    }
     return;
   }
   PProg P = as_const_prog(a.P);
@@ -657,7 +599,12 @@
   SEC(e, SEC_STORE);
   emit_draw_record(e, a, env);
   store_record(e, a.H, a.L, gf, gq, a.fault_flag);
-  if (a.cost && e.lane == 0) a.cost[env] = moog_cost_ema((float)(clock64() - t_sched), a.cost[env]);
+  if (a.cost) {
+    float c = 0.f;
+    int rn = 0;
+    if (e.lane == 0) { a.cost[env] = c = moog_cost_ema((float)(clock64() - t_sched), a.cost[env]); rn = EQ(e)[EL(e).o_reset_next]; }
+    if (a.sched_ws) sched_fold(a.sched_ws, a.sched_key, a.n_envs, env, e.lane, c, rn);
+  }
   if ((a.dbg & 128) && e.lane == 0 && a.discount) {
     a.discount[env] = (double)(clock64() - t_begin);
     if (a.reward) a.reward[env] = (double)(e.n_path + 100000 * e.n_resp) + 1e10 * (double)e.n_disj;
@@ -740,4 +687,4 @@
 void moog_launch_reset_full(int n_envs, size_t lds, hipStream_t s, const KArgs& a);
 int moog_configure_reset_plain(size_t lds);
 int moog_configure_reset_full(size_t lds);
-void moog_launch_sched(hipStream_t s, const float* cost, int32_t* perm, int n, const int32_t* reset_next, int stride);
+void moog_launch_sched_scatter(hipStream_t s, const SchedScatter& a);
diff --git a/moog.github.io_amd/csrc/moog_raster.h b/moog.github.io_amd/csrc/moog_raster.h
--- a/moog.github.io_amd/csrc/moog_raster.h
+++ b/moog.github.io_amd/csrc/moog_raster.h
@@ -67,6 +67,7 @@
   size_t sbg_env_stride;
   const uint32_t* rgb_override;
   const int32_t* env_build;
+  SchedScatter sched;
 };
 
 struct REdge { short x0, y0, x1, y1; float dx; short vtop, vbot; };
diff --git a/moog.github.io_amd/csrc/moog_raster.hip b/moog.github.io_amd/csrc/moog_raster.hip
--- a/moog.github.io_amd/csrc/moog_raster.hip
+++ b/moog.github.io_amd/csrc/moog_raster.hip
@@ -38,6 +38,7 @@
   a.n_static = r.em.ncopy > 1 ? 0 : r.em.n_static;
   a.sbg = r.sbg; a.rows_seen = r.rows_seen;
   a.plan = r.ms.plan;
+  a.sched = r.sched;
   return a;
 }
 
diff --git a/moog.github.io_amd/csrc/moog_raster_kernel.h b/moog.github.io_amd/csrc/moog_raster_kernel.h
--- a/moog.github.io_amd/csrc/moog_raster_kernel.h
+++ b/moog.github.io_amd/csrc/moog_raster_kernel.h
@@ -452,6 +452,7 @@
   const int tile_id = block - benv * tiles;
   const int env = env_of_block >= 0 ? env_of_block : benv;
   if (a.build && a.env_build && a.env_build[env] == 0) return;
+  if (a.sched.perm && tile_id == 0 && threadIdx.x == 0) sched_scatter(a.sched, env);
   const int band = tile_id / a.tiles_x;
   PProg P = as_const_prog(a.P);
   const int WF = a.canvas_w, H = a.canvas_h;
diff --git a/moog.github.io_amd/csrc/moog_raster_mask.h b/moog.github.io_amd/csrc/moog_raster_mask.h
--- a/moog.github.io_amd/csrc/moog_raster_mask.h
+++ b/moog.github.io_amd/csrc/moog_raster_mask.h
@@ -13,6 +13,7 @@
   const int tid = (int)threadIdx.x, lane = tid & 63;
   const int env = (int)blockIdx.x;
   if (env >= a.n_envs) return;
+  if (a.sched.perm && tid == 0) sched_scatter(a.sched, env);
   rm_load(a, c, env, tid, RM_THREADS);
   __syncthreads();
   if (a.debug_stop == 1 || a.debug_stop == 2) return;
diff --git a/moog.github.io_amd/csrc/moog_raster_mask_core.h b/moog.github.io_amd/csrc/moog_raster_mask_core.h
--- a/moog.github.io_amd/csrc/moog_raster_mask_core.h
+++ b/moog.github.io_amd/csrc/moog_raster_mask_core.h
@@ -1,6 +1,7 @@
 #ifndef MOOG_RASTER_MASK_CORE_H_
 #define MOOG_RASTER_MASK_CORE_H_
 #include "moog_draw_record.h"
+#include "moog_sched.h"
 
 #define RM_THREADS 128
 #define RM_WAVES_PER_SIMD 5
@@ -34,6 +35,7 @@
   const uint8_t* sbg;
   int32_t* rows_seen;
   RmPlan plan;
+  SchedScatter sched;
 };
 
 static inline uint32_t rm_align(uint32_t x) { return (x + 15u) & ~15u; }
diff --git a/moog.github.io_amd/csrc/moog_reset.hip b/moog.github.io_amd/csrc/moog_reset.hip
--- a/moog.github.io_amd/csrc/moog_reset.hip
+++ b/moog.github.io_amd/csrc/moog_reset.hip
@@ -20,7 +20,7 @@
 }
 
 #if !MOOG_RESET_FULL
-void moog_launch_sched(hipStream_t s, const float* cost, int32_t* perm, int n, const int32_t* reset_next, int stride) {
-  hipLaunchKernelGGL(moog_sched_kernel, dim3(1), dim3(SCHED_THREADS), 0, s, cost, perm, n, reset_next, stride);
+void moog_launch_sched_scatter(hipStream_t s, const SchedScatter& a) {
+  hipLaunchKernelGGL(moog_sched_scatter_kernel, dim3((unsigned)((a.n + 63) / 64)), dim3(64), 0, s, a);
 }
 #endif
diff --git a/moog.github.io_amd/csrc/moog_sched.h b/moog.github.io_amd/csrc/moog_sched.h
--- /dev/null
+++ b/moog.github.io_amd/csrc/moog_sched.h
@@ -0,0 +1,81 @@
+#pragma once
+#include <stdint.h>
+
+#define SCHED_BINS 1024
+enum {
+  SCHED_W_HIST = 0,
+  SCHED_W_DONE = SCHED_BINS,
+  SCHED_W_MAX = SCHED_BINS + 1,
+  SCHED_W_SCALE = SCHED_BINS + 2,
+  SCHED_W_BASE = SCHED_BINS + 4,
+  SCHED_W_WORDS = 2 * SCHED_BINS + 4
+};
+
+struct SchedScatter {
+  const int32_t* ws;
+  const int32_t* key;
+  int32_t* perm;
+  int32_t n;
+};
+
+#ifdef __HIPCC__
+#include <hip/hip_runtime.h>
+
+__device__ __forceinline__ float sched_cost(float c) { return (c >= 0.f && c < 3.0e38f) ? c : 0.f; }
+__device__ __forceinline__ int sched_bin_of(float cv, float scale, int r) {
+  int b = SCHED_BINS - 1 - (int)(cv * scale);
+  b = b < 0 ? 0 : (b > SCHED_BINS - 1 ? SCHED_BINS - 1 : b);
+  return r == 1 ? 0 : b;
+}
+
+__device__ __forceinline__ int sched_wave_scan(int v) {
+  v += __builtin_amdgcn_update_dpp(0, v, 0x111, 0xf, 0xf, false);
+  v += __builtin_amdgcn_update_dpp(0, v, 0x112, 0xf, 0xf, false);
+  v += __builtin_amdgcn_update_dpp(0, v, 0x114, 0xf, 0xf, false);
+  v += __builtin_amdgcn_update_dpp(0, v, 0x118, 0xf, 0xf, false);
+  v += __builtin_amdgcn_update_dpp(0, v, 0x142, 0xa, 0xf, false);
+  v += __builtin_amdgcn_update_dpp(0, v, 0x143, 0xc, 0xf, false);
+  return v;
+}
+
+__device__ __forceinline__ void sched_fold(int32_t* ws, int32_t* key, int n, int env, int lane, float cost, int reset_next) {
+  int last = 0;
+  if (lane == 0) {
+    const float c = sched_cost(cost);
+    const int b = sched_bin_of(c, __int_as_float(ws[SCHED_W_SCALE]), reset_next);
+    const int ord = __hip_atomic_fetch_add(&ws[SCHED_W_HIST + b], 1, __ATOMIC_RELAXED, __HIP_MEMORY_SCOPE_AGENT);
+    __hip_atomic_fetch_max(&ws[SCHED_W_MAX], __float_as_int(c), __ATOMIC_RELAXED, __HIP_MEMORY_SCOPE_AGENT);
+    *reinterpret_cast<int2*>(key + 2 * (size_t)env) = make_int2(b, ord);
+    __builtin_amdgcn_fence(__ATOMIC_RELEASE, "agent");
+    last = __hip_atomic_fetch_add(&ws[SCHED_W_DONE], 1, __ATOMIC_RELAXED, __HIP_MEMORY_SCOPE_AGENT) == n - 1;
+  }
+  if (!__builtin_amdgcn_readfirstlane(last)) return;
+  __builtin_amdgcn_fence(__ATOMIC_ACQUIRE, "agent");
+  constexpr int PER = SCHED_BINS / 64;
+  int own[PER], v = 0;
+#pragma unroll
+  for (int k = 0; k < PER; ++k) {
+    own[k] = __hip_atomic_load(&ws[SCHED_W_HIST + PER * lane + k], __ATOMIC_RELAXED, __HIP_MEMORY_SCOPE_AGENT);
+    v += own[k];
+  }
+  int before = sched_wave_scan(v) - v;
+#pragma unroll
+  for (int k = 0; k < PER; ++k) {
+    ws[SCHED_W_BASE + PER * lane + k] = before;
+    before += own[k];
+    ws[SCHED_W_HIST + PER * lane + k] = 0;
+  }
+  if (lane == 0) {
+    const float m = __int_as_float(__hip_atomic_load(&ws[SCHED_W_MAX], __ATOMIC_RELAXED, __HIP_MEMORY_SCOPE_AGENT));
+    ws[SCHED_W_SCALE] = __float_as_int(m > 0.f ? (float)(SCHED_BINS - 1) / m : 0.f);
+    ws[SCHED_W_MAX] = 0;
+    ws[SCHED_W_DONE] = 0;
+  }
+}
+
+__device__ __forceinline__ void sched_scatter(const SchedScatter& s, int env) {
+  const int2 k = *reinterpret_cast<const int2*>(s.key + 2 * (size_t)env);
+  const unsigned p = (unsigned)(s.ws[SCHED_W_BASE + (k.x & (SCHED_BINS - 1))] + k.y);
+  if (p < (unsigned)s.n) s.perm[p] = env;
+}
+#endif
diff --git a/moog.github.io_amd/moog/_engine.py b/moog.github.io_amd/moog/_engine.py
--- a/moog.github.io_amd/moog/_engine.py
+++ b/moog.github.io_amd/moog/_engine.py
@@ -11,6 +11,7 @@
     'moog_engine_destroy', 'moog_engine_layout', 'moog_engine_load_state', 'moog_engine_reset',
     'moog_engine_step', 'moog_engine_physics_only', 'moog_engine_render',
     'moog_engine_set_timing', 'moog_engine_kernel_time', 'moog_engine_set_schedule',
+    'moog_engine_schedule_state',
     'moog_engine_set_debug', 'moog_engine_static_prefix', 'moog_engine_poll_faults',
     'moog_engine_layer_usage', 'moog_engine_set_action_dtype', 'moog_engine_set_action_repeat',
     'moog_engine_read_watch', 'moog_engine_set_reset_pool', 'moog_engine_get_reset_pool',
@@ -55,6 +56,7 @@
     lib.moog_engine_physics_only.argtypes = [vp, ctypes.POINTER(_abi.Inject), vp]
     lib.moog_engine_render.argtypes = [vp, vp, vp]
     lib.moog_engine_set_schedule.argtypes = [vp, vp, vp]
+    lib.moog_engine_schedule_state.argtypes = [vp, ctypes.POINTER(i32), ctypes.POINTER(i32)]
     lib.moog_engine_set_timing.argtypes = [vp, i32]
     lib.moog_engine_set_reset_pool.argtypes = [vp, i32]
     lib.moog_engine_env_prefix.argtypes = [vp, ctypes.POINTER(i32)]
```

Result: slower. 5.441 million env steps/sec (-13.9%).
